# ChrisHird/ZLIB

Hardware: AMD Instinct MI355X
Metric: GiB/s raw input compressed (deflate level 6) (higher is better)
Workload: dtype u8

## Files before the change

### include/zamd_gpu.h

```cpp
#ifndef ZAMD_GPU_H
#define ZAMD_GPU_H
#include <stddef.h>
#include <stdint.h>

#ifdef __cplusplus
extern "C" {
#endif

#define ZGPU_OK 0
#define ZGPU_ERRNO (-1)
#define ZGPU_STREAM_ERROR (-2)
#define ZGPU_DATA_ERROR (-3)
#define ZGPU_MEM_ERROR (-4)
#define ZGPU_BUF_ERROR (-5)

#define ZGPU_CHUNK_MAX 65536u

#define ZGPU_F_FINAL 1u
#define ZGPU_F_ZLIB_WRAP 2u
#define ZGPU_F_POS0 4u
#define ZGPU_F_POS0_ALL 8u
#define ZGPU_F_GZIP_WRAP 16u
#define ZGPU_F_CRC32 32u

// ... 213 lines not shown
                                   uint64_t *total, uint64_t *nfailed);

int zgpu_inflate_batch_verify_device(zgpu_engine *e, const void *d_in, uint64_t in_bytes, const uint64_t *d_in_offsets, uint64_t n, int wrap,
                                     uint32_t checks, zgpu_inflate_item *d_items, uint64_t *nfailed, void *hip_stream);
int zgpu_inflate_batch_verify_host(zgpu_engine *e, const void *in, uint64_t in_bytes, const uint64_t *in_offsets, uint64_t n, int wrap,
                                   uint32_t checks, zgpu_inflate_item *items, uint64_t *nfailed);

#define ZGPU_BATCH_JOB_DECODE 0
#define ZGPU_BATCH_JOB_SIZES 1
#define ZGPU_BATCH_JOB_VERIFY 2
#define ZGPU_BATCH_JOB_PACKED 3
typedef struct {
    uint64_t nfailed, nbad_offsets, total;
    uint32_t overflow, reserved;
} zgpu_inflate_batch_summary;
uint64_t zgpu_inflate_batch_workspace_bytes(int job, uint64_t n);
int zgpu_inflate_batch_enqueue(zgpu_engine *e, const void *d_in, uint64_t in_bytes, const uint64_t *d_in_offsets, uint64_t n, int wrap,
                               uint32_t checks, void *d_out, uint64_t out_cap, const uint64_t *d_out_offsets, zgpu_inflate_item *d_items,
                               zgpu_inflate_batch_summary *d_summary, void *d_ws, uint64_t ws_bytes, void *hip_stream);
int zgpu_inflate_batch_sizes_enqueue(zgpu_engine *e, const void *d_in, uint64_t in_bytes, const uint64_t *d_in_offsets, uint64_t n, int wrap,
                                     zgpu_inflate_item *d_items, zgpu_inflate_batch_summary *d_summary, void *d_ws, uint64_t ws_bytes,
                                     void *hip_stream);
int zgpu_inflate_batch_verify_enqueue(zgpu_engine *e, const void *d_in, uint64_t in_bytes, const uint64_t *d_in_offsets, uint64_t n, int wrap,
                                      uint32_t checks, zgpu_inflate_item *d_items, zgpu_inflate_batch_summary *d_summary, void *d_ws,
                                      uint64_t ws_bytes, void *hip_stream);
int zgpu_inflate_batch_packed_enqueue(zgpu_engine *e, const void *d_in, uint64_t in_bytes, const uint64_t *d_in_offsets, uint64_t n, int wrap,
                                      uint32_t checks, uint32_t align, void *d_out, uint64_t out_cap, uint64_t *d_out_offsets,
                                      zgpu_inflate_item *d_items, zgpu_inflate_batch_summary *d_summary, void *d_ws, uint64_t ws_bytes,
                                      void *hip_stream);

int zgpu_bgzf_index_device(zgpu_engine *e, const void *d_in, uint64_t in_bytes, uint64_t *d_in_offsets, uint64_t *d_out_offsets, uint64_t cap_blocks,
                           uint64_t *nblocks, uint64_t *out_bytes, uint32_t *ends_with_eof_block, void *hip_stream);
int zgpu_bgzf_inflate_device(zgpu_engine *e, const void *d_in, uint64_t in_bytes, void *d_out, uint64_t out_cap, zgpu_inflate_item *d_items,
                             zgpu_inflate_result *res, void *hip_stream);
int zgpu_bgzf_inflate_host(zgpu_engine *e, const void *in, uint64_t in_bytes, void *out, uint64_t out_cap, zgpu_inflate_item *items, zgpu_inflate_result *res);
int zgpu_bgzf_verify_device(zgpu_engine *e, const void *d_in, uint64_t in_bytes, zgpu_inflate_item *d_items, zgpu_inflate_result *res, void *hip_stream);
int zgpu_bgzf_verify_host(zgpu_engine *e, const void *in, uint64_t in_bytes, zgpu_inflate_item *items, zgpu_inflate_result *res);

int zgpu_gzip_inflate_device(zgpu_engine *e, const void *d_in, uint64_t in_bytes, void *d_out, uint64_t out_cap, uint64_t *d_in_offsets, uint64_t *d_out_offsets,
                             zgpu_inflate_item *d_items, uint64_t cap_members, uint64_t *nmembers, zgpu_inflate_result *res, void *hip_stream);
int zgpu_gzip_inflate_host(zgpu_engine *e, const void *in, uint64_t in_bytes, void *out, uint64_t out_cap, uint64_t *in_offsets, uint64_t *out_offsets,
                           zgpu_inflate_item *items, uint64_t cap_members, uint64_t *nmembers, zgpu_inflate_result *res);
uint64_t zgpu_gzip_members_count(int which);

int zgpu_adler32_device(zgpu_engine *e, const void *d_in, uint64_t in_bytes, uint32_t *adler_out, void *hip_stream);
int zgpu_crc32_device(zgpu_engine *e, const void *d_in, uint64_t in_bytes, uint32_t *crc_out, void *hip_stream);

typedef struct {
    uint32_t adler32, crc32;
} zgpu_check_item;
int zgpu_checksum_batch_device(zgpu_engine *e, const void *d_in, uint64_t in_bytes, const uint64_t *d_offsets, uint64_t n, uint32_t checks,
                               zgpu_check_item *d_items, void *hip_stream);
int zgpu_checksum_batch_host(zgpu_engine *e, const void *in, uint64_t in_bytes, const uint64_t *offsets, uint64_t n, uint32_t checks,
                             zgpu_check_item *items);

enum {
    ZGPU_STAGE_CHAIN = 0,
    ZGPU_STAGE_MATCH,
    ZGPU_STAGE_PARSE,
    ZGPU_STAGE_LZ_SERIAL,
    ZGPU_STAGE_HUFFMAN,
    ZGPU_STAGE_STITCH,
    ZGPU_STAGE_INFLATE,
    ZGPU_STAGE_COUNT
};
void zgpu_profile_enable(zgpu_engine *e, int on);
void zgpu_profile_reset(zgpu_engine *e);
int zgpu_profile_get(zgpu_engine *e, int stage, double *ms, uint64_t *launches);
const char *zgpu_stage_name(int stage);

enum {
    ZGPU_FAST_ROUNDS = 0,
    ZGPU_FAST_TILE_PARSES,
    ZGPU_FAST_SAME_ENTRY,
    ZGPU_FAST_STOPPED_EARLY,
    ZGPU_FAST_DIFFERENT_TOKEN,
    ZGPU_FAST_REACH_TO_END,
    ZGPU_FAST_WINDOWS_TO_DIFF,
    ZGPU_FAST_WINDOWS_OF_DIFF,
    ZGPU_FAST_COUNT_N
};
uint64_t zgpu_deflate_fast_count(zgpu_engine *e, int which);

int zgpu_corpus_fill_device(zgpu_engine *e, uint32_t kind, uint64_t seed, uint64_t first_chunk, uint64_t nchunks,
                            void *d_out, void *hip_stream);

#ifdef __cplusplus
}
#endif
#endif
```

### zlib_amd/csrc/zgpu_common.h

```cpp
#pragma once
#include <hip/hip_runtime.h>
#include <stdint.h>

namespace zgpu {

constexpr uint32_t kWSize = 32768, kWMask = kWSize - 1, kHashSize = 32768, kHashMask = kHashSize - 1;
constexpr uint32_t kMinMatch = 3, kMaxMatch = 258, kMinLookahead = kMaxMatch + kMinMatch + 1;
constexpr uint32_t kMaxDist = kWSize - kMinLookahead;
constexpr uint32_t kTooFar = 4096;
constexpr uint32_t kChunkMax = 65536;
constexpr uint32_t kSPad = 8, kSStride = kChunkMax + kSPad;
constexpr uint32_t kBlockTokens = 16383;
constexpr uint32_t kSerialTableEntries = 32768 + 32768;
constexpr uint32_t kGeoTableEntries = 65536 + 32768;
constexpr uint32_t kGeoNostoreWords = 18;
constexpr uint32_t kGeoSlotStride = 65536 + 8192 + 1024 + 64 + 5 * 32 * kGeoNostoreWords + 448;
constexpr uint32_t kMaxBlocks = 6;
constexpr uint32_t kFullFinalBlock = 1u << 31;
constexpr uint32_t kHandedOn = 0xFFFFFFFFu;
constexpr int kLCodes = 286, kDCodes = 30, kBLCodes = 19, kHeapSize = 2 * kLCodes + 1, kMaxBits = 15, kMaxBLBits = 7;
constexpr int kEndBlock = 256;
constexpr uint32_t kSlotStride = 65536 + 256;

struct LevelCfg { uint32_t good, lazy, nice, chain, slow, strategy; uint32_t w_bits, hash_bits; };
constexpr uint32_t kFiltered = 1, kHuffmanOnly = 2, kRle = 3, kFixed = 4;
inline LevelCfg level_cfg(int level)
{
    static const LevelCfg t[10] = {{0, 0, 0, 0, 0, 0},      {4, 4, 8, 4, 0, 0},      {4, 5, 16, 8, 0, 0},      {4, 6, 32, 32, 0, 0},
                                   {4, 4, 16, 16, 1, 0},    {8, 16, 32, 32, 1, 0},   {8, 16, 128, 128, 1, 0},  {8, 32, 128, 256, 1, 0},
                                   {32, 128, 258, 1024, 1, 0}, {32, 258, 258, 4096, 1, 0}};
    return t[level];
}

enum InfMsg : uint32_t {
    kMsgNone = 0, kMsgBlockType, kMsgStoredLen, kMsgTooMany, kMsgCodeLens, kMsgRepeat, kMsgLitLens, kMsgDists, kMsgLitCode, kMsgDistCode,
    kMsgTooFar, kMsgTruncated, kMsgOutput, kMsgTrailing, kMsgShort, kMsgTable,
    kMsgHeaderCheck, kMsgMethod, kMsgWindow, kMsgHeaderFlags, kMsgHeaderCrc, kMsgDataCheck, kMsgLengthCheck, kMsgBgzfChain, kMsgCount
};

constexpr uint32_t kWrapRaw = 0, kWrapZlib = 1, kWrapGzip = 2, kWrapAuto = 3;
struct BatchItemState {
    uint64_t in_lo, in_hi, body_lo, out_lo;
    uint64_t piece0;
    uint32_t kind;
    int32_t code;
    uint32_t msg, used;
    uint32_t out_bytes, npieces;
};
struct InfStatus { int32_t code; uint32_t msg; uint32_t out_bytes; uint32_t used; };
constexpr uint32_t kWholeStream = 0xFFFFFFFFu;
struct SpecEnd { uint64_t end_bit; uint32_t out_bytes, flags; };
struct SpecArgs {
    uint16_t *mid;
    uint64_t *page_owner;
    uint32_t *page_count;
    uint32_t page_cap;
    uint16_t *tails;
    SpecEnd *ends;
    const struct PieceRow *rows = nullptr;
    uint32_t *need = nullptr;
    const uint8_t *windows = nullptr;
    const uint64_t *ostart = nullptr;
    struct PieceCheck *checks = nullptr;
};
struct PieceCheck { uint64_t end_bit; uint32_t out_bytes, flags, adler_a, adler_b, crc, pad; };
struct PieceTarget { uint64_t lo_bit, hi_bit, limit; };
struct PieceRow {
    uint64_t start, stop;
    uint64_t in_end;
    uint32_t item;
    uint32_t first;
};
constexpr uint32_t kPieceNoItem = 0xFFFFFFFFu;
struct PieceItem {
    uint64_t body_lo, in_hi, out_lo, out_hi;
    uint64_t total;
    uint64_t end_bit;
    uint32_t k;
    uint32_t target0, slot0;
    uint32_t ntargets, piece_cap;
    uint32_t npieces;
    uint32_t clean;
    uint32_t bad;
};
struct PiecesList { unsigned long long *hdr; PieceItem *items; uint64_t min_bytes, max_long; };
constexpr uint32_t kHdrLong = 0, kHdrTargets = 1, kHdrSlots = 2, kHdrRoom = 3, kHdrClean = 4, kHdrFell = 5, kHdrGathered = 6;

struct FrameHead { uint8_t b[18]; uint8_t n, gzip, bgzf; };
constexpr uint32_t kBgzfBlockMax = 65280;

struct ChunkMeta {
    uint32_t ntok;
    uint32_t nostore;
    uint32_t out_bytes;
    uint32_t data_type;
    uint32_t adler_a, adler_b;
    uint32_t in_bytes;
    uint32_t crc;
};

struct TileRow {
// ... 335 lines not shown
```

### zlib_amd/csrc/zgpu_deflate.hip

```cpp
#include "zgpu_engine.h"
#include "zgpu_deflate_plan.h"
#include <cstdlib>
#include <atomic>
#include <thread>

namespace zgpu {

int ensure_deflate_ws(zgpu_engine *e, uint32_t batch, bool serial, uint64_t nchunks_total, bool geo)
{
    int rc;
    bool grew;
    if (geo) {
        if ((rc = e->geo_slots.reserve(e, (size_t)batch * kGeoSlotStride))) return rc;
        if ((rc = e->geo_tables.reserve(e, (size_t)batch * kGeoTableEntries, &grew))) return rc;
        if (grew) {
            ZGPU_HIP_CHECK(hipMemsetAsync(e->geo_tables, 0, e->geo_tables.cap * sizeof(uint4), e->stream));
            ZGPU_HIP_CHECK(hipStreamSynchronize(e->stream));
        }
        if ((rc = e->geo_nostore.reserve(e, (size_t)batch * kGeoNostoreWords))) return rc;
    }
    if ((rc = e->tokens.reserve(e, (size_t)batch * kChunkMax))) return rc;
    if ((rc = e->meta.reserve(e, (size_t)batch))) return rc;
    if ((rc = e->slots.reserve(e, (size_t)batch * kSlotStride))) return rc;
    if (serial && !geo) {
// ... 155 lines not shown
    launch_seg_limit(c.d_seg, c.nseg, c.in_bytes, kBgzfBlockMax, flag, c.st);
    ZGPU_HIP_CHECK(hipMemcpyAsync(&over, flag, 4, hipMemcpyDeviceToHost, c.st));
    ZGPU_HIP_CHECK(hipStreamSynchronize(c.st));
    if (over) return fail(e, ZGPU_STREAM_ERROR, "BGZF blocks: a segment is longer than 65280 bytes (or the table leaves the input)");
    return ZGPU_OK;
}

static int reserve_deflate(zgpu_engine *e, const DeflatePlan &pl, uint32_t *hand_piece)
{
    int rc = ensure_deflate_ws(e, pl.batch, pl.serial, pl.nchunks, pl.geo);
    if (rc) return rc;
    *hand_piece = pl.hand_piece;
    if (pl.hand_on) {
        if ((rc = ensure_deflate_ws(e, pl.hand_piece, false, pl.nchunks))) return rc;
        if (e->par_cap > pl.hand_piece) *hand_piece = e->par_cap < pl.batch ? e->par_cap : pl.batch;
        if ((rc = e->hand_list.reserve(e, (size_t)pl.batch + 1))) return rc;
    }
    return ZGPU_OK;
}

static ChunkGeom chunk_geom(const zgpu_engine *e, const DeflateCall &c, const DeflatePlan &pl)
{
    const zgpu_deflate_params *p = c.p;
    ChunkGeom g{};
    g.in = c.d_in; g.in_bytes = c.in_bytes; g.seg_off = c.d_seg; g.chunk_size = pl.chunk_size;
    g.final_chunk = (!c.d_seg && (p->flags & ZGPU_F_FINAL)) ? pl.nchunks - 1 : ~0ull;
    g.all_final = (c.d_seg && (p->flags & ZGPU_F_FINAL)) ? 1u : 0u;
    g.pos0_mode = (p->flags & ZGPU_F_POS0_ALL) ? 2u : (p->flags & ZGPU_F_POS0) ? 1u : 0u;
    g.skip0 = c.skip0;
    g.block_tokens = pl.block_tokens;
    g.slot_stride = pl.geo ? kGeoSlotStride : kSlotStride;
    g.nostore_bits = pl.geo ? e->geo_nostore : nullptr;
    g.prime = (p->prime >> 16) ? ((p->prime & 0xffff0000u) | (p->prime & ((1u << (p->prime >> 16)) - 1u))) : 0u;
    return g;
}

static int copy_batch_in(zgpu_engine *e, const DeflateCall &c, const BatchSteps &s, uint32_t chunk_size)
{
    const uint64_t c1 = s.c0 + s.nb();
    const uint64_t lo = s.c0 * chunk_size, hi = c1 * (uint64_t)chunk_size < c.in_bytes ? c1 * (uint64_t)chunk_size : c.in_bytes;
    const hipEvent_t ev = engine_copy_event(e, s.k);
    ZGPU_HIP_CHECK(hipMemcpyAsync(const_cast<uint8_t *>(c.d_in) + lo, c.h_src + lo, hi - lo, hipMemcpyHostToDevice, e->copy_stream));
    ZGPU_HIP_CHECK(hipEventRecord(ev, e->copy_stream));
    ZGPU_HIP_CHECK(hipStreamWaitEvent(c.st, ev, 0));
    return ZGPU_OK;
}

static int lz_batch(zgpu_engine *e, const ChunkGeom &g, const DeflatePlan &pl, uint32_t hand_piece, hipStream_t st, bool *adler_done)
{
    *adler_done = false;
    if (!pl.serial) {
        if (pl.impl == ZGPU_LZ_PARALLEL) launch_lz_parallel(g, pl.cfg, e->par_ws, e->tokens, e->meta, st, e);
        else *adler_done = launch_lz_sorted(g, pl.cfg, e->par_ws, e->tokens, e->meta, st, e, e->exact_sort, pl.impl);
        return ZGPU_OK;
    }
    StageTimer t(e, st, ZGPU_STAGE_LZ_SERIAL);
    if (++e->serial_tag == 0) {
        if (e->tables) ZGPU_HIP_CHECK(hipMemsetAsync(e->tables, 0, e->tables.cap * sizeof(uint4), st));
        if (e->geo_tables) ZGPU_HIP_CHECK(hipMemsetAsync(e->geo_tables, 0, e->geo_tables.cap * sizeof(uint4), st));
        e->serial_tag = 1;
    }
    if (pl.geo) launch_lz_serial(g, pl.cfg, e->geo_tables, e->tokens, e->meta, st, e->geo_nostore, false, e->serial_tag);
    else launch_lz_serial(g, pl.cfg, e->tables, e->tokens, e->meta, st, nullptr, pl.hand_on, e->serial_tag);
    if (pl.hand_on) {
        launch_collect_handed_on(e->meta, g.nchunks, e->hand_list + 1, e->hand_list, st);
        uint32_t handed = 0;
        ZGPU_HIP_CHECK(hipMemcpyAsync(&handed, e->hand_list, 4, hipMemcpyDeviceToHost, st));
        ZGPU_HIP_CHECK(hipStreamSynchronize(st));
        for (uint32_t at = 0; at < handed; at += hand_piece) {
            ChunkGeom gl = g; gl.nchunks = handed - at < hand_piece ? handed - at : hand_piece; gl.chunk_map = e->hand_list + 1 + at;
            launch_lz_sorted(gl, pl.cfg, e->par_ws, e->tokens, e->meta, st, e, e->exact_sort, ZGPU_LZ_FASTWIN);
        }
        e->handed_on += handed;
    }
    return ZGPU_OK;
}

static void blocks_batch(zgpu_engine *e, const DeflateCall &c, const DeflatePlan &pl, const ChunkGeom &g, const FrameHead &fh, uint64_t body_cap, bool adler_done)
{
    const hipStream_t st = c.st;
    uint8_t *const slots = pl.geo ? e->geo_slots : e->slots;
    {
        StageTimer t(e, st, ZGPU_STAGE_HUFFMAN);
        launch_huffman(g, e->tokens, e->meta, slots, st, pl.cfg.strategy == kFixed);
    }
    StageTimer t(e, st, ZGPU_STAGE_STITCH);
    if (!adler_done) launch_adler(g, e->meta, st);
    if (pl.with_crc) launch_crc(g, e->meta, st);
    if (pl.seg_wrap) launch_frame(slots, e->meta, e->offsets, c.d_seg, g.chunk0, g.nchunks, c.d_out, body_cap, g.slot_stride, e->run, pl.with_crc, fh, st);
    else {
        launch_scan(e->meta, g.nchunks, g.chunk0, e->offsets, e->run, body_cap, st, pl.with_crc);
        launch_stitch(slots, e->meta, e->offsets, g.chunk0, g.nchunks, c.d_out, body_cap, g.slot_stride, st);
    }
    if (c.d_items) launch_seg_items(e->meta, e->offsets, c.d_seg, g.chunk0, g.nchunks, pl.with_crc, c.d_items, st);
}

static int deflate_device(zgpu_engine *e, const DeflateCall &c)
{
    if (!e) return ZGPU_STREAM_ERROR;
    const zgpu_deflate_params *const p = c.p;
    const hipStream_t st = c.st;
    PlanCall pc;
    pc.args = p && c.res && (c.d_in || !c.in_bytes) && c.d_out;
    if (p) { pc.level = p->level; pc.strategy = p->strategy; pc.lz_impl = p->lz_impl; pc.chunk_size = p->chunk_size; pc.flags = p->flags; pc.prime = p->prime; }
    pc.in_bytes = c.in_bytes; pc.seg = c.d_seg != nullptr; pc.nseg = c.nseg; pc.skip0 = c.skip0; pc.host_in = c.h_src != nullptr;
    PlanEngine pe; pe.geo_w = e->geo_w; pe.geo_m = e->geo_m;
    DeflatePlan pl = plan_deflate_args(pc, pe);
    if (pl.rc) return fail(e, pl.rc, pl.msg);
    ZGPU_HIP_CHECK(hipSetDevice(e->device));
    int rc;
    if ((p->flags & ZGPU_F_BGZF_WRAP) && c.nseg && !c.seg_checked && (rc = check_bgzf_segments(e, c))) return rc;
    const LevelCfg lc = level_cfg_for(e, p->level, p->strategy);
    pl = plan_deflate(pc, plan_engine(e, &lc), read_deflate_knobs());
    if (pl.rc) return fail(e, pl.rc, pl.msg);
    uint32_t hand_piece = 0;
    if ((rc = reserve_deflate(e, pl, &hand_piece))) return rc;
    const FrameHead fh = frame_head(p->level, p->strategy, pl.wrap, pl.gz, pl.bgzf);
    ChunkGeom g = chunk_geom(e, c, pl);
    const uint64_t body_cap = pl.tail_bytes ? (c.out_cap >= pl.head_bytes + pl.tail_bytes ? c.out_cap - pl.tail_bytes : 0) : c.out_cap;
    RunState rs{}; rs.out_total = pl.head_bytes; rs.adler_a = 1; rs.adler_b = 0; rs.data_type = 2;
    ZGPU_HIP_CHECK(hipMemcpyAsync(e->run, &rs, sizeof rs, hipMemcpyHostToDevice, st));
    uint32_t sort_fault = 0;
    if (pl.check_sort) ZGPU_HIP_CHECK(hipMemsetAsync(lz_sorted_fault_word(e->par_ws), 0, 4, st));
    if (!pl.seg_wrap && pl.head_bytes && c.out_cap >= pl.head_bytes) ZGPU_HIP_CHECK(hipMemcpyAsync(c.d_out, fh.b, pl.head_bytes, hipMemcpyHostToDevice, st));
    const size_t nbatches = plan_nbatches(pl);
    BatchHomer home;
    if (c.h_dst && c.h_src && nbatches > 1 && nbatches <= BatchHomer::kMaxBatches && (rc = home.start(e, c, nbatches))) return rc;
    for (BatchSteps s(pl); s.more(); s.next()) {
        g.chunk0 = s.c0; g.nchunks = s.nb();
        if (c.h_src && c.in_bytes && (rc = copy_batch_in(e, c, s, pl.chunk_size))) return rc;
        bool adler_done;
        if ((rc = lz_batch(e, g, pl, hand_piece, st, &adler_done))) return rc;
        blocks_batch(e, c, pl, g, fh, body_cap, adler_done);
        if (home.on() && (rc = home.queued(s.k, st))) return rc;
        const hipError_t he = hipGetLastError();
        if (he != hipSuccess) return zgpu::fail_hip(e, he, "kernel launch", __FILE__, __LINE__);
    }
    if (home.on() && (rc = home.finish(c.h_copied))) return rc;
    ZGPU_HIP_CHECK(hipMemcpyAsync(&rs, e->run, sizeof rs, hipMemcpyDeviceToHost, st));
    if (pl.check_sort) ZGPU_HIP_CHECK(hipMemcpyAsync(&sort_fault, lz_sorted_fault_word(e->par_ws), 4, hipMemcpyDeviceToHost, st));
    ZGPU_HIP_CHECK(hipStreamSynchronize(st));
    collect_spans(e);
    if (sort_fault) {
        e->exact_sort = 1;
        return deflate_device(e, c);
    }
    if (rs.overflow || (pl.tail_bytes && c.out_cap < rs.out_total + pl.tail_bytes)) return fail(e, ZGPU_BUF_ERROR, "output capacity too small");
    const uint32_t adler = rs.adler_a | (rs.adler_b << 16);
    if ((pl.wrap || pl.gz) && !pl.seg_wrap && (rc = write_trailer(e, pl.gz, adler, rs.crc, c.in_bytes, c.d_out, &rs.out_total, st))) return rc;
    if (c.d_chunk_offsets) {
        ZGPU_HIP_CHECK(hipMemcpyAsync(c.d_chunk_offsets, e->offsets, (pl.nchunks + 1) * sizeof(uint64_t), hipMemcpyDeviceToDevice, st));
        ZGPU_HIP_CHECK(hipStreamSynchronize(st));
    }
    zgpu_deflate_result *const res = c.res;
    res->out_bytes = rs.out_total; res->nchunks = pl.nchunks; res->adler32 = adler; res->data_type = rs.data_type; res->ntokens = rs.ntokens;
    res->crc32 = pl.with_crc ? rs.crc : 0;
    return ZGPU_OK;
}

}

using namespace zgpu;

extern "C" {
#pragma GCC visibility push(default)

uint64_t zgpu_deflate_bound(uint64_t in_bytes, uint32_t chunk_size)
// ... 256 lines not shown
```

### zlib_amd/csrc/zgpu_deflate_batch.hip

```cpp
#include "zgpu_engine.h"
#include "zgpu_deflate_plan.h"
#include "zgpu_deflate_batch_plan.h"

namespace zgpu {

static_assert(kDwsTokenBytes == kChunkMax * sizeof(uint32_t) && kDwsSlotBytes == kSlotStride && kDwsMetaBytes == sizeof(ChunkMeta),
              "zgpu_deflate_batch_plan.h states what a round's item costs as numbers");
static_assert(sizeof(zgpu_deflate_batch_item) == 40 && sizeof(zgpu_deflate_batch_summary) == 40, "the records of include/zamd_gpu.h");
static_assert(kDwsStageBytes == kChunkMax && kDwsLoBytes == sizeof(uint64_t) && kDwsPreBytes == sizeof(uint64_t), "the staging buffer and its tables");
static_assert(kDwsCntBytes / 8 == 32, "dbatch_head_kernel clears the counters with lanes 0..31");
static_assert(kSlotStride % 4 == 0, "dbatch_place_kernel reads the slots as words");

constexpr uint32_t kItemServed = 0, kItemFailed = 1;

__global__ void __launch_bounds__(64) dbatch_head_kernel(unsigned long long *cnt, uint32_t *fault, zgpu_deflate_batch_summary *summary)
{
    const uint32_t tid = threadIdx.x;
    if (cnt && tid < kDwsCntBytes / 8) cnt[tid] = 0;
    if (fault && tid == 32) fault[0] = 0;
    if (summary && tid == 33) *summary = zgpu_deflate_batch_summary{};
}

__global__ void __launch_bounds__(1024) dbatch_check_kernel(const uint64_t *__restrict__ in_off, uint64_t n, uint64_t in_bytes, uint32_t limit, const uint64_t *__restrict__ out_off,
                                                            uint64_t out_cap, uint32_t packed, uint64_t c0, uint32_t nb, uint64_t *__restrict__ lo_out, uint64_t *__restrict__ t,
// ... 137 lines not shown
{
    const uint64_t k = (uint64_t)blockIdx.x * 256 + threadIdx.x;
    const bool raised = fault[0] != 0;
    if (raised && k < n) items[k].code = ZGPU_ERRNO;
    if (k == 0 && summary) {
        zgpu_deflate_batch_summary s{};
        s.nfailed = raised ? n : cnt[kDcntFailed]; s.nbad_offsets = cnt[kDcntBadOffsets]; s.ntoo_long = cnt[kDcntTooLong];
        s.total = packed ? cnt[kDcntTotal] : 0; s.overflow = packed && cnt[kDcntTotal] > out_cap ? 1u : 0u; s.sort_fault = raised ? 1u : 0u;
        *summary = s;
    }
}

struct DeflateBatchWs {
    unsigned long long *cnt; uint64_t *lo, *pre; uint32_t *state; uint8_t *stage; uint8_t *sorted; uint32_t *tokens; uint8_t *slots; ChunkMeta *meta;
    uint32_t round;
};

struct DeflateBatchCfg { LevelCfg cfg; int impl; bool with_crc; FrameHead fh; uint32_t tail, limit; };
static const char *batch_params(const zgpu_engine *e, const zgpu_deflate_params *p, DeflateBatchCfg *bc)
{
    constexpr uint32_t kServed = ZGPU_F_FINAL | ZGPU_F_ZLIB_WRAP | ZGPU_F_GZIP_WRAP | ZGPU_F_CRC32 | ZGPU_F_BGZF_WRAP;
    if (p->level < 1 || p->level > 9) return "deflate batch: level must be 1..9";
    if (!(p->flags & ZGPU_F_FINAL)) return "deflate batch: every item is a stream of its own, ZGPU_F_FINAL is required";
    if (p->flags & ~kServed) return "deflate batch: ZGPU_F_POS0 / ZGPU_F_POS0_ALL / ZGPU_F_CONTINUOUS are not served";
    const uint32_t wrappers = (p->flags & ZGPU_F_ZLIB_WRAP ? 1 : 0) + (p->flags & ZGPU_F_GZIP_WRAP ? 1 : 0) + (p->flags & ZGPU_F_BGZF_WRAP ? 1 : 0);
    if (wrappers > 1) return "deflate batch: one wrapper at a time";
    if (p->prime) return "deflate batch: prime is not served";
    if (p->lz_impl != ZGPU_LZ_AUTO) return "deflate batch: lz_impl must be ZGPU_LZ_AUTO";
    if (p->strategy < 0 || p->strategy > (int)kFixed) return "strategy must be 0..4";
    if (p->strategy == (int)kHuffmanOnly || p->strategy == (int)kRle) return "deflate batch: Z_HUFFMAN_ONLY and Z_RLE are not served (the blocking segment call serves them)";
    if (e->geo_w != 15 || e->geo_m != 8) return "deflate batch: the default geometry only (windowBits 15, memLevel 8)";
    bc->cfg = level_cfg_for(e, p->level, p->strategy);
    if (bc->cfg.slow) {
        if (const char *why = records_refuse(bc->cfg, ZGPU_LZ_WALK)) return why;
        bc->impl = ZGPU_LZ_WALK;
    } else {
        if (!lz_fastwin_serves(bc->cfg)) return "deflate batch: levels 1-3 with their own parameters only (ZGPU_LZ_FASTWIN does not serve this deflateTune row)";
        if (const char *why = fast_refuse(bc->cfg)) return why;
        bc->impl = ZGPU_LZ_FASTWIN;
    }
    const bool wrap = p->flags & ZGPU_F_ZLIB_WRAP, bgzf = p->flags & ZGPU_F_BGZF_WRAP, gz = (p->flags & ZGPU_F_GZIP_WRAP) || bgzf;
    bc->with_crc = gz || (p->flags & ZGPU_F_CRC32);
    bc->fh = frame_head(p->level, p->strategy, wrap, gz, bgzf);
    bc->tail = gz ? 8u : wrap ? 4u : 0u;
    bc->limit = bgzf ? kBgzfBlockMax : kChunkMax;
    return nullptr;
}

static int deflate_batch_enqueue(zgpu_engine *e, const void *d_in, uint64_t in_bytes, const uint64_t *d_in_off, uint64_t n, const zgpu_deflate_params *p, void *d_out, uint64_t out_cap,
                                 uint64_t *d_out_off, bool packed, zgpu_deflate_batch_item *d_items, zgpu_deflate_batch_summary *d_summary, void *d_ws, uint64_t ws_bytes,
                                 uint32_t batch_items, void *hip_stream)
{
    if (!e) return ZGPU_STREAM_ERROR;
    if (!p || n >= kDwsMaxItems || (n && (!d_in_off || !d_items || !d_out_off)) || (n && in_bytes && !d_in) || (n && out_cap && !d_out))
        return fail(e, ZGPU_STREAM_ERROR, "bad deflate batch arguments");
    DeflateBatchCfg bc{};
    if (const char *why = batch_params(e, p, &bc)) return fail(e, ZGPU_STREAM_ERROR, why);
    const hipStream_t st = hip_stream ? static_cast<hipStream_t>(hip_stream) : e->stream;
    DeflateBatchWs w{};
    if (n) {
        const DeflateWsPlan pl = deflate_batch_ws_plan(n, batch_items);
        if (!d_ws || (reinterpret_cast<uintptr_t>(d_ws) & (kDwsAlign - 1)) || pl.total == 0 || ws_bytes < pl.total)
            return fail(e, ZGPU_STREAM_ERROR, "deflate batch workspace: null, not 256-byte aligned or too small");
        uint8_t *b = static_cast<uint8_t *>(d_ws);
        w.cnt = reinterpret_cast<unsigned long long *>(b + pl.cnt.off); w.lo = reinterpret_cast<uint64_t *>(b + pl.lo.off); w.pre = reinterpret_cast<uint64_t *>(b + pl.pre.off); w.stage = b + pl.stage.off;
        w.state = reinterpret_cast<uint32_t *>(b + pl.state.off); w.sorted = b + pl.sorted.off; w.tokens = reinterpret_cast<uint32_t *>(b + pl.tokens.off);
        w.slots = b + pl.slots.off; w.meta = reinterpret_cast<ChunkMeta *>(b + pl.meta.off); w.round = (uint32_t)pl.round;
    }
    int cur = -1;
    ZGPU_HIP_CHECK(hipGetDevice(&cur));
    if (cur != e->device) ZGPU_HIP_CHECK(hipSetDevice(e->device));
    if (n == 0) {
        if (d_summary) hipLaunchKernelGGL(dbatch_head_kernel, dim3(1), dim3(64), 0, st, static_cast<unsigned long long *>(nullptr), static_cast<uint32_t *>(nullptr), d_summary);
        ZGPU_HIP_CHECK(hipGetLastError());
        return ZGPU_OK;
    }
    uint32_t *const fault = lz_sorted_fault_word(w.sorted);
    hipLaunchKernelGGL(dbatch_head_kernel, dim3(1), dim3(64), 0, st, w.cnt, fault, d_summary);
    const uint32_t ngrid = (uint32_t)((n + 255) / 256);
    ChunkGeom g{};
    g.in = w.stage; g.in_bytes = (uint64_t)w.round * kDwsStageBytes; g.chunk_size = kChunkMax;
    g.final_chunk = ~0ull; g.all_final = 1; g.block_tokens = kBlockTokens; g.slot_stride = kSlotStride;
    const uint32_t frame = bc.fh.n + bc.tail;
    for (uint64_t c0 = 0; c0 < n; c0 += w.round) {
        const uint32_t nb = (uint32_t)(n - c0 < w.round ? n - c0 : w.round);
        const uint64_t *const t = w.pre;
        g.seg_off = t; g.chunk0 = 0; g.nchunks = nb;
        hipLaunchKernelGGL(dbatch_check_kernel, dim3(1), dim3(1024), 0, st, d_in_off, n, in_bytes, bc.limit, d_out_off, out_cap, packed ? 1u : 0u, c0, nb, w.lo, w.pre, w.state, w.cnt);
        hipLaunchKernelGGL(dbatch_gather_kernel, dim3(nb), dim3(256), 0, st, static_cast<const uint8_t *>(d_in), w.lo, w.state, t, nb, w.stage);
        const bool adler_done = launch_lz_sorted(g, bc.cfg, w.sorted, w.tokens, w.meta, st, nullptr, e->exact_sort, bc.impl);
        launch_huffman(g, w.tokens, w.meta, w.slots, st, bc.cfg.strategy == kFixed);
        if (!adler_done) launch_adler(g, w.meta, st);
        if (bc.with_crc) launch_crc(g, w.meta, st);
        if (packed) hipLaunchKernelGGL(dbatch_scan_kernel, dim3(1), dim3(1024), 0, st, w.meta, w.state, c0, nb, frame, d_out_off, w.cnt);
        hipLaunchKernelGGL(dbatch_place_kernel, dim3(nb), dim3(256), 0, st, w.slots, w.meta, w.state, t, d_out_off, c0, nb, static_cast<uint8_t *>(d_out), out_cap,
                           packed ? 1u : 0u, bc.with_crc ? 1u : 0u, bc.fh, bc.tail, d_items, w.cnt);
    }
    hipLaunchKernelGGL(dbatch_finish_kernel, dim3(ngrid), dim3(256), 0, st, fault, n, packed ? 1u : 0u, out_cap, w.cnt, d_items, d_summary);
    ZGPU_HIP_CHECK(hipGetLastError());
    return ZGPU_OK;
}

}

using namespace zgpu;

extern "C" {
#pragma GCC visibility push(default)

uint64_t zgpu_deflate_batch_workspace_bytes(uint64_t n, uint32_t batch_items) { return deflate_batch_ws_bytes(n, batch_items); }

int zgpu_deflate_batch_enqueue(zgpu_engine *e, const void *d_in, uint64_t in_bytes, const uint64_t *d_in_offsets, uint64_t n, const zgpu_deflate_params *p, void *d_out,
                               uint64_t out_cap, const uint64_t *d_out_offsets, zgpu_deflate_batch_item *d_items, zgpu_deflate_batch_summary *d_summary, void *d_ws,
                               uint64_t ws_bytes, uint32_t batch_items, void *hip_stream)
{
    return deflate_batch_enqueue(e, d_in, in_bytes, d_in_offsets, n, p, d_out, out_cap, const_cast<uint64_t *>(d_out_offsets), false, d_items, d_summary, d_ws, ws_bytes, batch_items,
                                 hip_stream);
}

int zgpu_deflate_batch_packed_enqueue(zgpu_engine *e, const void *d_in, uint64_t in_bytes, const uint64_t *d_in_offsets, uint64_t n, const zgpu_deflate_params *p, void *d_out,
                                      uint64_t out_cap, uint64_t *d_out_offsets, zgpu_deflate_batch_item *d_items, zgpu_deflate_batch_summary *d_summary, void *d_ws,
                                      uint64_t ws_bytes, uint32_t batch_items, void *hip_stream)
{
    return deflate_batch_enqueue(e, d_in, in_bytes, d_in_offsets, n, p, d_out, out_cap, d_out_offsets, true, d_items, d_summary, d_ws, ws_bytes, batch_items, hip_stream);
}

int zgpu_engine_set_exact_sort(zgpu_engine *e, int on)
{
    if (!e) return ZGPU_STREAM_ERROR;
    e->exact_sort = on != 0;
    return ZGPU_OK;
}

#pragma GCC visibility pop
}
```

### zlib_amd/csrc/zgpu_engine.h

```cpp
#pragma once
#include "zgpu_common.h"
#include "../../include/zamd_gpu.h"
#include <vector>

namespace zgpu {

int fail_hip(zgpu_engine *e, hipError_t err, const char *what, const char *file, int line);
int fail(zgpu_engine *e, int code, const char *msg);

template <typename T> struct DevBuf {
    T *p = nullptr;
    size_t cap = 0;
    DevBuf() = default;
    DevBuf(const DevBuf &) = delete;
    DevBuf &operator=(const DevBuf &) = delete;
    ~DevBuf() { release(); }
    operator T *() const { return p; }
    void release() { if (p) hipFree(p); p = nullptr; cap = 0; }
    int reserve(zgpu_engine *e, size_t n, bool *grew = nullptr)
    {
        if (grew) *grew = false;
        if (n <= cap) return ZGPU_OK;
        release();
        const hipError_t err = hipMalloc(reinterpret_cast<void **>(&p), n * sizeof(T));
        if (err != hipSuccess) { p = nullptr; return fail_hip(e, err, "hipMalloc of an engine buffer", __FILE__, __LINE__); }
        cap = n;
        if (grew) *grew = true;
        return ZGPU_OK;
    }
};

struct Carve {
    size_t off = 0;
    size_t operator()(size_t bytes) { const size_t at = off; off = (off + bytes + 255) & ~(size_t)255; return at; }
};

}

namespace zgpu { struct StreamsRoundPart; struct StreamsRound; }
struct StageSpan { int stage; hipEvent_t a, b; };

struct zgpu_engine {
    template <typename T> using DevBuf = zgpu::DevBuf<T>;
    int device = 0;
    hipStream_t stream = nullptr;
    hipStream_t copy_stream = nullptr;
    std::vector<hipEvent_t> copy_ev;
    hipStream_t d2h_stream = nullptr;
    std::vector<hipEvent_t> done_ev;
    uint64_t *pin_tot = nullptr;
    char err[512] = {0};
    DevBuf<uint32_t> tokens;
    DevBuf<zgpu::ChunkMeta> meta;
    DevBuf<uint8_t> slots;
    uint32_t batch_cap() const { return (uint32_t)meta.cap; }
    DevBuf<uint4> tables;
    uint32_t serial_tag = 0;
    DevBuf<uint8_t> par_ws;
    uint32_t par_cap = 0;
    int tuned = 0; uint32_t tune[4] = {0, 0, 0, 0};
    int fast_prev0 = 0, before_buf = -1;
    int last_tok_match = -1;
    uint64_t handed_on = 0;
    DevBuf<uint32_t> hand_list;
    int geo_w = 15, geo_m = 8;
    DevBuf<uint8_t> geo_slots; DevBuf<uint4> geo_tables; DevBuf<uint32_t> geo_nostore;
    int exact_sort = 0;
    DevBuf<uint64_t> offsets;
    DevBuf<zgpu::RunState> run;
    DevBuf<uint8_t> stage_in, stage_out;
    DevBuf<uint8_t> inf_status;
    DevBuf<zgpu::ChunkMeta> inf_meta;
    DevBuf<uint64_t> inf_offs;
    DevBuf<uint8_t> inf_slots;
    DevBuf<uint8_t> inf_dict; uint32_t inf_dict_len = 0;
    uint32_t inf_checks = 3;
    DevBuf<uint16_t> ct_exits, ct_entry, ct_comp, ct_gentry;
    DevBuf<uint32_t> ct_tokoff, ct_T, ct_carry, ct_carry_in;
    DevBuf<zgpu::ContBlk> ct_blk; DevBuf<uint64_t> ct_pos; DevBuf<uint8_t> ct_slots; DevBuf<zgpu::ContState> ct_st;
    uint32_t ct_tiles() const { return ct_tokoff.cap ? (uint32_t)(ct_tokoff.cap - 1) : 0; }
    DevBuf<zgpu::ChunkMeta> ct_ckmeta;
    DevBuf<uint64_t> ct_excl;
    DevBuf<zgpu::TileRow> ds_rows; DevBuf<uint16_t> ds_entry; DevBuf<zgpu::ContState> ds_st; DevBuf<zgpu_check_item> ds_check; DevBuf<unsigned long long> ds_totals;
    DevBuf<uint32_t> ds_tokoff, ds_blk_item; DevBuf<zgpu::StreamsRoundPart> ds_parts; DevBuf<zgpu::StreamsRound> ds_rounds; DevBuf<uint64_t> ds_tile0;
    DevBuf<uint64_t> ds_in_off, ds_oo, ds_po; DevBuf<zgpu_deflate_batch_item> ds_items; DevBuf<uint8_t> ds_packed;
    DevBuf<uint16_t> cf_exit_a, cf_exit_b; DevBuf<uint32_t> cf_ins0, cf_ins1, cf_prev, cf_prev2, cf_hist, cf_count;
    DevBuf<uint8_t> cf_cur, cf_act_a, cf_act_b, cf_changed, cf_kept; DevBuf<uint32_t> cf_list_a, cf_list_b, cf_used; DevBuf<uint16_t> cf_entry_used;
    DevBuf<uint32_t> cf_dbg, cf_dstat;
    hipStream_t ct_stream = nullptr; hipEvent_t ct_ev_a[2] = {nullptr, nullptr}, ct_ev_b[2] = {nullptr, nullptr};
    uint64_t cf_rounds = 0, cf_tile_parses = 0;
    uint64_t cf_stat[6] = {};
    DevBuf<uint32_t> bz_cnt, bz_isize, bz_jump_a, bz_jump_b, bz_reach, bz_res;
    DevBuf<uint64_t> bz_base, bz_pos, bz_next, bz_in_off, bz_out_off;
    DevBuf<zgpu_inflate_item> bz_items;
    DevBuf<uint64_t> gz_in_end, gz_trial, gz_next; DevBuf<uint32_t> gz_guess;
    DevBuf<zgpu_inflate_item> gz_items;
    DevBuf<uint64_t> pk_hi; DevBuf<zgpu_inflate_item> pk_items;
    DevBuf<uint64_t> ck_piece0; DevBuf<uint32_t> ck_flag, ck_part;
    bool prof = false;
    double ms[ZGPU_STAGE_COUNT] = {0};
    uint64_t launches[ZGPU_STAGE_COUNT] = {0};
    std::vector<hipEvent_t> ev_pool;
    size_t ev_used = 0;
    std::vector<StageSpan> spans;

    zgpu_engine() = default;
    zgpu_engine(const zgpu_engine &) = delete;
    zgpu_engine &operator=(const zgpu_engine &) = delete;
    ~zgpu_engine();
};

namespace zgpu {

void collect_spans(zgpu_engine *e);
int ensure_stage(zgpu_engine *e, uint64_t in_bytes, uint64_t out_bytes);
hipEvent_t engine_copy_event(zgpu_engine *e, size_t i);
void prof_span_begin(zgpu_engine *e, hipStream_t st, hipEvent_t *a);
void prof_span_end(zgpu_engine *e, hipStream_t st, int stage, hipEvent_t a);
struct StageTimer {
    zgpu_engine *e; hipStream_t st; int stage; hipEvent_t a{};
    StageTimer(zgpu_engine *e_, hipStream_t st_, int stage_) : e(e_), st(st_), stage(stage_) { prof_span_begin(e, st, &a); }
    ~StageTimer() { prof_span_end(e, st, stage, a); }
};
uint32_t env_u32(const char *name, uint32_t dflt);
int checksum_pass(zgpu_engine *e, const uint8_t *d_bytes, uint64_t nbytes, uint32_t mask, uint32_t batch_cap, DevBuf<ChunkMeta> &meta, hipStream_t st, uint32_t *adler, uint32_t *crc);

int ensure_deflate_ws(zgpu_engine *e, uint32_t batch, bool serial, uint64_t nchunks_total, bool geo = false);
LevelCfg level_cfg_for(const zgpu_engine *e, int level, int strategy);
FrameHead frame_head(int level, int strategy, bool wrap, bool gz, bool bgzf = false);
int write_trailer(zgpu_engine *e, bool gz, uint32_t adler, uint32_t crc, uint64_t in_bytes, uint8_t *d_out, uint64_t *out_total, hipStream_t st);
struct PlanEngine;
PlanEngine plan_engine(const zgpu_engine *e, const LevelCfg *cfg);

const char *streams_refuse(const zgpu_engine *e, const zgpu_deflate_params *p);
void streams_list_geom(const uint8_t *d_in, uint64_t in_bytes, uint16_t *exits, uint16_t *entry, ChunkGeom *g, TileGeom *tg);

int deflate_cont_oneshot(zgpu_engine *e, const uint8_t *d_in, uint64_t in_bytes, const zgpu_deflate_params *p, uint8_t *d_out, uint64_t out_cap, zgpu_deflate_result *res, hipStream_t st);

void launch_lz_serial(const ChunkGeom &g, LevelCfg cfg, uint4 *tables, uint32_t *tokens, ChunkMeta *meta, hipStream_t st, uint32_t *nostore_bits, bool hand_on, uint32_t tag);

void launch_huffman(const ChunkGeom &g, const uint32_t *tokens, ChunkMeta *meta, uint8_t *slots, hipStream_t st, bool fixed_trees);
void launch_huffman_cont(const ChunkGeom &g, const uint32_t *compact_tokens, uint32_t nblk, ContBlk *blk, ContState *cst, uint8_t *slots, hipStream_t st, bool fixed_trees);
void launch_huffman_streams(const ChunkGeom &g, const uint32_t *batch_tokens, uint32_t nslots, ContBlk *blk, ContState *states, const uint32_t *blk_item, uint8_t *slots, hipStream_t st,
                            bool fixed_trees);

void launch_collect_handed_on(const ChunkMeta *meta, uint32_t n, uint32_t *list, uint32_t *count, hipStream_t st);
void launch_adler(const ChunkGeom &g, ChunkMeta *meta, hipStream_t st);
void launch_crc(const ChunkGeom &g, ChunkMeta *meta, hipStream_t st);
void launch_scan(const ChunkMeta *meta, uint32_t nchunks, uint64_t chunk0, uint64_t *offsets, void *run, uint64_t out_cap, hipStream_t st, bool with_crc = false);
void launch_frame(const uint8_t *slots, const ChunkMeta *meta, uint64_t *offsets, const uint64_t *seg_off, uint64_t chunk0, uint32_t nchunks, uint8_t *out,
                  uint64_t out_cap, uint32_t slot_stride, void *run, bool with_crc, const FrameHead &h, hipStream_t st);
void launch_stitch(const uint8_t *slots, const ChunkMeta *meta, const uint64_t *offsets, uint64_t chunk0, uint32_t nchunks, uint8_t *out,
                   uint64_t out_cap, uint32_t slot_stride, hipStream_t st);
void launch_bgzf_cut(uint64_t in_bytes, uint32_t block_size, uint64_t nseg, uint64_t *seg_off, hipStream_t st);
void launch_seg_limit(const uint64_t *seg_off, uint64_t nseg, uint64_t in_bytes, uint32_t limit, uint32_t *flag, hipStream_t st);
void launch_seg_items(const ChunkMeta *meta, const uint64_t *offsets, const uint64_t *seg_off, uint64_t chunk0, uint32_t nchunks, bool with_crc, zgpu_deflate_item *items, hipStream_t st);
void launch_corpus(uint32_t kind, uint64_t seed, uint64_t first_chunk, uint64_t nchunks, uint8_t *out, hipStream_t st);
void launch_batch_finish(const BatchItemState *items, uint64_t n, const ChunkMeta *meta, const uint8_t *in, uint32_t do_adler, uint32_t do_crc,
                         zgpu_inflate_item *out_items, unsigned long long *nfailed, hipStream_t st);

bool lz_parallel_available();
size_t lz_parallel_workspace_bytes(uint32_t batch_chunks);
void launch_lz_parallel(const ChunkGeom &g, LevelCfg cfg, void *workspace, uint32_t *tokens, ChunkMeta *meta, hipStream_t st, zgpu_engine *prof);
void launch_parse(const ChunkGeom &g, LevelCfg cfg, const uint2 *recs, uint32_t *tokens, ChunkMeta *meta, hipStream_t st);

void launch_parse2(const ChunkGeom &g, LevelCfg cfg, const uint2 *recs, uint32_t *tokens, ChunkMeta *meta, hipStream_t st);
void launch_parse_tile(const ChunkGeom &g, LevelCfg cfg, const uint32_t *gm, const uint32_t *gs, uint32_t *tokens, ChunkMeta *meta, const TileGeom &tg, hipStream_t st);

size_t lz_sorted_workspace_bytes(uint32_t batch_chunks);
uint32_t *lz_sorted_fault_word(void *workspace);
bool launch_lz_sorted(const ChunkGeom &g, LevelCfg cfg, void *workspace, uint32_t *tokens, ChunkMeta *meta, hipStream_t st, zgpu_engine *prof, int exact_sort,
                      int impl);
void launch_lz_tiles(const ChunkGeom &g, const TileGeom &tg, LevelCfg cfg, void *workspace, ChunkMeta *meta, uint16_t *comp, uint16_t *gentry, hipStream_t st, zgpu_engine *prof,
                     int exact_sort);
void launch_lz_tiles_parse(const ChunkGeom &g, const TileGeom &tg, LevelCfg cfg, void *workspace, uint32_t *tokens, ChunkMeta *meta, hipStream_t st, zgpu_engine *prof);
void launch_sort_tiles(const ChunkGeom &g, void *workspace, ChunkMeta *meta, hipStream_t st, zgpu_engine *prof, int exact_sort, const uint16_t **S_out, const uint32_t **ir_out);

bool lz_fastwin_serves(const LevelCfg &cfg);
void launch_lz_fastwin(const ChunkGeom &g, LevelCfg cfg, const uint16_t *S, const uint32_t *ir, uint32_t *tokens, ChunkMeta *meta, hipStream_t st);
void launch_lz_fastwin_tiles(const ChunkGeom &g, const TileGeom &tg, const FastTiles &ft, LevelCfg cfg, const uint16_t *S, const uint32_t *ir, uint32_t *tokens, ChunkMeta *meta, uint32_t ngrid,
                             hipStream_t st);
void launch_fast_init(uint8_t *cur, uint8_t *active, uint16_t *exit_cur, uint32_t n, hipStream_t st);
void launch_fast_flip_list(uint8_t *cur, uint16_t *exit_cur, const uint16_t *exit_new, const uint32_t *list, uint32_t n, hipStream_t st);
void launch_fast_flip(uint8_t *cur, const uint8_t *active, uint8_t *active_next, const uint8_t *changed, uint16_t *exit_cur, const uint16_t *exit_new, uint32_t n, uint32_t round,
                      uint32_t *count, uint32_t *list, const uint8_t *kept, hipStream_t st);
void launch_fast_finish(const uint8_t *cur, const uint16_t *exit_cur, const uint32_t *ins0, const uint32_t *ins1, uint32_t n, uint16_t *entry_after, uint32_t *prev_ins, uint32_t *prev_prev_ins,
                        const uint32_t *low, hipStream_t st);
void launch_fast_hist(const uint32_t *before, const uint32_t *last, uint32_t x0, uint32_t count, uint32_t *out, hipStream_t st);

uint32_t chain_groups(uint32_t ntiles);
uint64_t cont_special_pos(uint64_t n);
void launch_chain(const uint16_t *exits, uint32_t ntiles, uint16_t *comp, uint16_t *gentry, uint16_t *entry, hipStream_t st);
void launch_cont_tokens(const ChunkGeom &g, const TileGeom &tg, const uint32_t *tokens, const ChunkMeta *tmeta, ContState *st, uint32_t *tokoff, const uint32_t *carry, uint32_t *T,
                        ContBlk *blk, uint64_t seg_end, bool final_block, uint64_t sp, uint32_t nblk_cap, bool slow, hipStream_t s);
void launch_cont_stitch(const ContBlk *blk, ContState *st, uint64_t *pos, const uint8_t *slots, uint32_t slot_stride, const uint8_t *in, uint64_t abs0, uint8_t *out, uint64_t out_cap,
                        uint32_t nblk_cap, const uint32_t *T, uint32_t *carry, uint64_t seg_end, hipStream_t s);

struct ContBatch {
    const StreamsRoundPart *parts; const StreamsRound *round;
    const uint64_t *in_off, *oo, *tile0; uint64_t t0;
    const uint8_t *in; uint8_t *out; uint32_t flags, slow, nslots_max;
    ContState *st; const uint16_t *entry;
    const uint32_t *tokens; const ChunkMeta *tmeta;
    uint32_t *tokoff, *carry, *T; ContBlk *blk; uint64_t *pos; const uint8_t *slots; uint32_t *blk_item;
};
void launch_cont_batch_tokens(const ContBatch &q, uint32_t nparts_max, uint32_t ntiles_max, hipStream_t s);
void launch_cont_batch_stitch(const ContBatch &q, uint32_t nparts_max, hipStream_t s);

void launch_streams_head(const uint64_t *in_off, const uint64_t *oo, const uint32_t *state, uint64_t n, const FrameHead &fh, uint32_t flags, ContState *st, uint8_t *out, uint16_t *entry0,
                         unsigned long long *totals, hipStream_t s);
void launch_streams_entry(const TileRow *rows, uint32_t ntiles, uint16_t *entry, hipStream_t s);
void launch_streams_finish(const uint64_t *in_off, const uint64_t *oo, const uint32_t *state, uint64_t n, const FrameHead &fh, uint32_t flags, const ContState *st,
                           const zgpu_check_item *chk, bool want_crc, uint8_t *out, zgpu_deflate_batch_item *items, unsigned long long *totals, hipStream_t s);
void launch_streams_pack(const uint8_t *rooms, const uint64_t *oo, const uint64_t *po, uint64_t n, uint64_t total, uint8_t *packed, hipStream_t s);

void launch_senq_clear(unsigned long long *cnt, uint32_t *fault, zgpu_deflate_batch_summary *summary, hipStream_t s);
void launch_senq_scan(const uint64_t *in_off, const uint64_t *oo, uint64_t n, uint64_t in_bytes, uint64_t out_cap, uint32_t *state, uint64_t *tile0, uint64_t *piece0,
                      unsigned long long *cnt, hipStream_t s);
void launch_senq_rows(const uint64_t *in_off, const uint64_t *tile0, uint64_t n, uint64_t nrows, TileRow *rows, hipStream_t s);
void launch_senq_round(const uint64_t *tile0, uint64_t n, uint64_t t0, uint32_t batch, const TileRow *rows, StreamsRoundPart *parts, StreamsRound *round, uint16_t *exits, ChunkMeta *meta,
                       hipStream_t s);
void launch_senq_layout(const uint64_t *in_off, uint64_t n, uint64_t in_bytes, uint32_t flags, uint64_t *oo, hipStream_t s);
void launch_senq_summary(const uint32_t *fault, uint64_t n, const unsigned long long *cnt, zgpu_deflate_batch_item *items, zgpu_deflate_batch_summary *summary, hipStream_t s);

struct InfLaunch {
    const uint8_t *in; uint64_t in_bytes; const uint64_t *offsets; uint64_t chunk0; uint32_t nchunks;
    uint8_t *out; uint64_t out_cap; InfStatus *status;
    uint64_t last_chunk = ~0ull; uint32_t chunk_size = kWholeStream; ChunkMeta *meta = nullptr;
    const uint8_t *dict = nullptr; uint32_t dict_len = 0; uint32_t stream_mode = 1;
    uint32_t checks = 0;
};
enum InfKind { kInfChunks, kInfBatch, kInfSizes, kInfPieces, kInfVerify, kInfBatchFold, kInfPieceSizes, kInfPieceVerify };
constexpr int kInfNoRing = 0;
int inflate_ring_kb();
void launch_inflate_decode(InfKind kind, int ring_kb, const InfLaunch &a, const SpecArgs &sp, hipStream_t st);
int output_checksums(zgpu_engine *e, const uint8_t *d_out, uint64_t nbytes, uint64_t out_cap, zgpu_inflate_result *res, hipStream_t st);
int inflate_run(zgpu_engine *e, const uint8_t *d_in, uint64_t in_bytes, const uint64_t *d_offsets, uint64_t nchunks, uint32_t chunk_size, uint8_t *d_out, uint64_t out_cap,
                zgpu_inflate_result *res, hipStream_t st, uint32_t stream_mode = 0, const uint64_t *h_offsets = nullptr, bool open_end = false, uint8_t *h_dst = nullptr, uint64_t h_cap = 0);

void launch_spec_find_table(const uint8_t *d_in, uint64_t in_bytes, const PieceTarget *table, uint32_t ntargets, uint64_t *found, hipStream_t st);
void launch_spec_resolve_items(const SpecArgs &sp, uint32_t nslots, uint32_t nitems, const uint2 *ranges, const uint8_t *entry, uint8_t *windows, const uint64_t *out_start,
                               PieceItem *items, uint8_t *d_out, hipStream_t st);
void launch_spec_windows_items(uint16_t *tails, uint32_t nslots, uint32_t nitems, const uint2 *ranges, const uint8_t *entry, uint8_t *windows, hipStream_t st);

struct BatchPiecesKnobs { uint64_t min_bytes, round_bytes; };
BatchPiecesKnobs batch_pieces_knobs();
uint64_t batch_pieces_count(int which);
size_t batch_pieces_scratch_bytes(uint64_t max_long);
PieceItem *batch_pieces_items(uint8_t *scr);
int batch_pieces_run(zgpu_engine *e, const uint8_t *d_in, uint64_t in_bytes, uint8_t *d_out, uint64_t out_cap, uint64_t max_long, uint8_t *scr, unsigned long long *d_hdr,
                     const unsigned long long *hdr, BatchItemState *states, InfStatus *status, uint64_t round_bytes, int ring_kb, hipStream_t st);
struct BatchPiecesSizesKnobs { uint64_t min_bytes, round_slots; };
BatchPiecesSizesKnobs batch_pieces_sizes_knobs();
// ... 29 lines not shown
```

### zlib_amd/csrc/zgpu_engine.hip

```cpp
#include "zgpu_engine.h"
#include <cstdio>
#include <cstdlib>
#include <cstring>

namespace zgpu {

int fail_hip(zgpu_engine *e, hipError_t err, const char *what, const char *file, int line)
{
    if (e) snprintf(e->err, sizeof e->err, "HIP error %d (%s) at %s:%d: %s", (int)err, hipGetErrorString(err), file, line, what);
    if (err == hipErrorOutOfMemory) return ZGPU_MEM_ERROR;
    return ZGPU_ERRNO;
}

int fail(zgpu_engine *e, int code, const char *msg)
{
    if (e) snprintf(e->err, sizeof e->err, "%s", msg);
    return code;
}

static hipEvent_t next_event(zgpu_engine *e)
{
    if (e->ev_used == e->ev_pool.size()) { hipEvent_t ev; hipEventCreate(&ev); e->ev_pool.push_back(ev); }
    return e->ev_pool[e->ev_used++];
}

void prof_span_begin(zgpu_engine *e, hipStream_t st, hipEvent_t *a)
{
    if (e && e->prof) { *a = next_event(e); hipEventRecord(*a, st); }
}
void prof_span_end(zgpu_engine *e, hipStream_t st, int stage, hipEvent_t a)
{
    if (e && e->prof) { hipEvent_t b = next_event(e); hipEventRecord(b, st); e->spans.push_back({stage, a, b}); }
}

void collect_spans(zgpu_engine *e)
{
    for (auto &s : e->spans) { float ms = 0; if (hipEventElapsedTime(&ms, s.a, s.b) == hipSuccess) { e->ms[s.stage] += ms; e->launches[s.stage]++; } }
    e->spans.clear(); e->ev_used = 0;
}

uint32_t env_u32(const char *name, uint32_t dflt)
{
    const char *v = getenv(name);
    if (!v || !*v) return dflt;
    long x = strtol(v, nullptr, 10);
    return x > 0 ? (uint32_t)x : dflt;
}

int ensure_stage(zgpu_engine *e, uint64_t in_bytes, uint64_t out_bytes)
{
    int rc;
    if (in_bytes > e->stage_in.cap && (rc = e->stage_in.reserve(e, in_bytes + (in_bytes >> 3) + 4096))) return rc;
    if (out_bytes > e->stage_out.cap && (rc = e->stage_out.reserve(e, out_bytes + (out_bytes >> 3) + 4096))) return rc;
    return ZGPU_OK;
}

int checksum_pass(zgpu_engine *e, const uint8_t *d_bytes, uint64_t nbytes, uint32_t mask, uint32_t batch_cap, DevBuf<ChunkMeta> &meta, hipStream_t st, uint32_t *adler, uint32_t *crc)
{
    const uint64_t npieces = nbytes ? (nbytes + kChunkMax - 1) / kChunkMax : 1;
    const uint32_t batch = (uint32_t)(npieces < batch_cap ? npieces : batch_cap);
    if (meta.reserve(e, batch) || e->inf_offs.reserve(e, npieces + 1)) return ZGPU_MEM_ERROR;
    RunState rs{}; rs.adler_a = 1;
    ZGPU_HIP_CHECK(hipMemcpyAsync(e->run, &rs, sizeof rs, hipMemcpyHostToDevice, st));
    for (uint64_t c0 = 0; c0 < npieces; c0 += batch) {
        const uint32_t nb = (uint32_t)(npieces - c0 < batch ? npieces - c0 : batch);
        ZGPU_HIP_CHECK(hipMemsetAsync(meta, 0, (size_t)nb * sizeof(ChunkMeta), st));
        ChunkGeom g{}; g.in = d_bytes; g.in_bytes = nbytes; g.chunk_size = kChunkMax; g.chunk0 = c0; g.nchunks = nb; g.final_chunk = ~0ull;
        if (mask & 1u) launch_adler(g, meta, st);
        if (mask & 2u) launch_crc(g, meta, st);
        launch_scan(meta, nb, c0, e->inf_offs, e->run, ~0ull, st, (mask & 2u) != 0);
    }
    ZGPU_HIP_CHECK(hipMemcpyAsync(&rs, e->run, sizeof rs, hipMemcpyDeviceToHost, st));
    ZGPU_HIP_CHECK(hipStreamSynchronize(st));
    *adler = (mask & 1u) ? rs.adler_a | (rs.adler_b << 16) : 1u;
    *crc = (mask & 2u) ? rs.crc : 0u;
    return ZGPU_OK;
}

hipEvent_t engine_copy_event(zgpu_engine *e, size_t i)
{
    while (e->copy_ev.size() <= i) { hipEvent_t ev; if (hipEventCreateWithFlags(&ev, hipEventDisableTiming) != hipSuccess) return nullptr; e->copy_ev.push_back(ev); }
    return e->copy_ev[i];
}

}

zgpu_engine::~zgpu_engine()
{
    hipSetDevice(device);
    if (stream) hipStreamSynchronize(stream);
    for (auto ev : ev_pool) hipEventDestroy(ev);
    for (auto ev : copy_ev) hipEventDestroy(ev);
    for (auto ev : done_ev) hipEventDestroy(ev);
    if (ct_stream) hipStreamDestroy(ct_stream);
    for (int i = 0; i < 2; i++) { if (ct_ev_a[i]) hipEventDestroy(ct_ev_a[i]); if (ct_ev_b[i]) hipEventDestroy(ct_ev_b[i]); }
    if (d2h_stream) hipStreamDestroy(d2h_stream);
    if (pin_tot) hipHostFree(pin_tot);
    if (copy_stream) hipStreamDestroy(copy_stream);
    if (stream) hipStreamDestroy(stream);
}

using namespace zgpu;

extern "C" {
#pragma GCC visibility push(default)

int zgpu_device_count(void)
{
    int n = 0;
    if (hipGetDeviceCount(&n) != hipSuccess) return 0;
    return n;
}

const char *zgpu_version(void) { return "zamd-gpu 0.1 (gfx950; zlib 1.2.3 bit-exact, 64 KiB independent chunks)"; }

int zgpu_engine_create(int device, zgpu_engine **out)
{
    if (!out) return ZGPU_STREAM_ERROR;
    *out = nullptr;
    int n = zgpu_device_count();
    if (device < 0 || device >= n) return ZGPU_ERRNO;
    zgpu_engine *e = new zgpu_engine();
    e->device = device;
    if (hipSetDevice(device) != hipSuccess || hipStreamCreateWithFlags(&e->stream, hipStreamNonBlocking) != hipSuccess || hipStreamCreateWithFlags(&e->copy_stream, hipStreamNonBlocking) != hipSuccess ||
        e->run.reserve(e, 1) != ZGPU_OK) {
        delete e;
        return ZGPU_ERRNO;
    }
    *out = e;
    return ZGPU_OK;
}

void zgpu_engine_destroy(zgpu_engine *e)
{
    if (e) delete e;
}

const char *zgpu_engine_error(const zgpu_engine *e) { return e ? e->err : "no engine"; }
uint64_t zgpu_debug_handed_on(const zgpu_engine *e) { return e ? e->handed_on : 0; }
int zgpu_debug_sort_fallback(const zgpu_engine *e) { return e ? e->exact_sort : 0; }

int zgpu_adler32_device(zgpu_engine *e, const void *d_in, uint64_t in_bytes, uint32_t *adler_out, void *hip_stream)
{
    if (!e || !adler_out || (!d_in && in_bytes)) return fail(e, ZGPU_STREAM_ERROR, "null argument");
    ZGPU_HIP_CHECK(hipSetDevice(e->device));
    hipStream_t st = hip_stream ? static_cast<hipStream_t>(hip_stream) : e->stream;
    int rc = ensure_deflate_ws(e, 1, false, 1);
    if (rc) return rc;
    uint32_t crc;
    return checksum_pass(e, static_cast<const uint8_t *>(d_in), in_bytes, 1u, 65536, e->inf_meta, st, adler_out, &crc);
}

int zgpu_crc32_device(zgpu_engine *e, const void *d_in, uint64_t in_bytes, uint32_t *crc_out, void *hip_stream)
{
    if (!e || !crc_out || (!d_in && in_bytes)) return fail(e, ZGPU_STREAM_ERROR, "null argument");
    ZGPU_HIP_CHECK(hipSetDevice(e->device));
    hipStream_t st = hip_stream ? static_cast<hipStream_t>(hip_stream) : e->stream;
    int rc = ensure_deflate_ws(e, 1, false, 1);
    if (rc) return rc;
    uint32_t adler;
    return checksum_pass(e, static_cast<const uint8_t *>(d_in), in_bytes, 2u, 65536, e->inf_meta, st, &adler, crc_out);
}

void zgpu_profile_enable(zgpu_engine *e, int on) { if (e) e->prof = on != 0; }
void zgpu_profile_reset(zgpu_engine *e) { if (e) { memset(e->ms, 0, sizeof e->ms); memset(e->launches, 0, sizeof e->launches); } }
int zgpu_profile_get(zgpu_engine *e, int stage, double *ms, uint64_t *launches)
{
    if (!e || stage < 0 || stage >= ZGPU_STAGE_COUNT) return ZGPU_STREAM_ERROR;
    if (ms) *ms = e->ms[stage];
    if (launches) *launches = e->launches[stage];
    return ZGPU_OK;
}
const char *zgpu_stage_name(int stage)
{
    static const char *names[ZGPU_STAGE_COUNT] = {"chain", "match", "parse", "lz_serial", "huffman", "stitch", "inflate"};
    return stage >= 0 && stage < ZGPU_STAGE_COUNT ? names[stage] : "?";
}

uint64_t zgpu_deflate_fast_count(zgpu_engine *e, int which)
{
    if (!e || which < 0 || which >= ZGPU_FAST_COUNT_N) return 0;
    return which == ZGPU_FAST_ROUNDS ? e->cf_rounds : which == ZGPU_FAST_TILE_PARSES ? e->cf_tile_parses : e->cf_stat[which - ZGPU_FAST_SAME_ENTRY];
}

int zgpu_corpus_fill_device(zgpu_engine *e, uint32_t kind, uint64_t seed, uint64_t first_chunk, uint64_t nchunks, void *d_out, void *hip_stream)
{
    if (!e || !d_out) return fail(e, ZGPU_STREAM_ERROR, "null argument");
    ZGPU_HIP_CHECK(hipSetDevice(e->device));
    hipStream_t st = hip_stream ? static_cast<hipStream_t>(hip_stream) : e->stream;
    launch_corpus(kind, seed, first_chunk, nchunks, static_cast<uint8_t *>(d_out), st);
    ZGPU_HIP_CHECK(hipGetLastError());
    ZGPU_HIP_CHECK(hipStreamSynchronize(st));
    return ZGPU_OK;
}

#pragma GCC visibility pop
}
```

### zlib_amd/csrc/zgpu_huffman.hip

```cpp
#include "zgpu_common.h"
#include "zgpu_engine.h"

namespace zgpu {

#ifndef ZGPU_HUFF_THREADS
#define ZGPU_HUFF_THREADS 128
#endif
constexpr int kThreads = ZGPU_HUFF_THREADS;
constexpr uint32_t kEmitPer = 4, kEmitRound = kThreads * kEmitPer;

template <int kNodes>
struct TreeWorkT {
    static constexpr int kCap = kNodes;
    uint16_t freq[kNodes];
    uint16_t dad[kNodes];
    uint16_t len[kNodes];
    __attribute__((aligned(16))) uint32_t heap[kNodes + 5];
    uint16_t bl_count[kMaxBits + 1];
    uint16_t next_code[kMaxBits + 1];
};
using TreeWork = TreeWorkT<kHeapSize>;
using TreeWorkD = TreeWorkT<2 * kDCodes + 1>;
__device__ inline uint32_t heap_entry(uint32_t freq, uint32_t depth, uint32_t node) { return (freq << 16) | (depth << 10) | node; }

struct BitWriter {
    uint32_t *words;
    uint32_t wi;
    uint64_t acc;
    uint32_t nacc;
    __device__ void begin(uint32_t *base, uint64_t bitpos, uint32_t carry) { words = base; wi = (uint32_t)(bitpos >> 5); nacc = (uint32_t)(bitpos & 31); acc = carry; }
    __device__ uint64_t pos() const { return ((uint64_t)wi << 5) + nacc; }
    __device__ void put(uint32_t v, uint32_t nb)
    {
        acc |= (uint64_t)v << nacc; nacc += nb;
        if (nacc >= 32) { words[wi] = (uint32_t)acc; wi++; acc >>= 32; nacc -= 32; }
    }
    __device__ void put64(uint64_t v, uint32_t nb)
    {
        if (nb > 32) { put((uint32_t)v, 32); put((uint32_t)(v >> 32), nb - 32); } else put((uint32_t)v, nb);
    }
    __device__ void align_byte() { uint32_t k = (8 - (nacc & 7)) & 7; if (k) put(0, k); }
    __device__ uint32_t carry() const { return (uint32_t)acc; }
    __device__ void store_tail() { if (nacc) words[wi] = (uint32_t)acc; }
};

template <class TW>
__device__ inline void sift_down(TW &t, int heap_len, int k)
{
    const uint32_t v = t.heap[k];
    int j = k << 1;
    while (j <= heap_len) {
        const uint2 ch = *reinterpret_cast<const uint2 *>(&t.heap[j]);
        const uint4 gc = *reinterpret_cast<const uint4 *>(&t.heap[2 * j]);
        uint32_t c = ch.x; int j1 = j;
        if (j < heap_len && (ch.y >> 10) <= (ch.x >> 10)) { c = ch.y; j1 = j + 1; }
        if ((v >> 10) <= (c >> 10)) break;
        t.heap[k] = c; k = j1;
        const int j2 = j1 << 1;
        if (j2 > heap_len) break;
        const uint32_t g0 = j1 == j ? gc.x : gc.z, g1 = j1 == j ? gc.y : gc.w;
        uint32_t c2 = g0; int j3 = j2;
        if (j2 < heap_len && (g1 >> 10) <= (g0 >> 10)) { c2 = g1; j3 = j2 + 1; }
        if ((v >> 10) <= (c2 >> 10)) break;
        t.heap[k] = c2; k = j3; j = j3 << 1;
    }
    t.heap[k] = v;
}

__device__ inline uint32_t extra_bits_of(int kind, int n)
{
    if (kind == 0) { const int k = n - 257; return (k < 8 || k == 28) ? 0u : (uint32_t)((k >> 2) - 1); }
    if (kind == 1) return n < 4 ? 0u : (uint32_t)((n >> 1) - 1);
    return n == 16 ? 2u : n == 17 ? 3u : n == 18 ? 7u : 0u;
}
__device__ inline uint32_t static_len_of(int kind, int n) { return kind == 0 ? (n < 144 ? 8u : n < 256 ? 9u : n < 280 ? 7u : 8u) : 5u; }

template <class TW>
__device__ int build_tree(TW &t, int elems, int kind, int max_length,
                          uint16_t *out_code, uint8_t *out_len, uint32_t &opt_len, uint32_t &static_len)
{
    const bool has_static = kind != 2;
    int heap_len = 0, heap_max = TW::kCap, max_code = -1, n, m, node;
    for (n = 0; n < elems; n++) {
        if (t.freq[n] != 0) t.heap[++heap_len] = heap_entry(t.freq[n], 0, (uint32_t)(max_code = n));
// ... 215 lines not shown
        count = 0; prevlen = curlen;
        if (nextlen == 0) { max_count = 138; min_count = 3; }
        else if (curlen == nextlen) { max_count = 6; min_count = 3; }
        else { max_count = 7; min_count = 4; }
    }
}

template <int MODE>
__device__ __forceinline__ uint32_t run_items(uint32_t L, uint32_t N, uint32_t *blf, const uint16_t *blcode, const uint8_t *bllen, uint32_t *obuf, uint32_t at)
{
    uint32_t bits = 0, rem = N;
    bool first = true;
    auto item = [&](uint32_t sym, uint32_t xv, uint32_t xb) {
        if (MODE == 0) atomicAdd(&blf[sym], 1u);
        else {
            const uint32_t cl = bllen[sym], nb = cl + xb;
            if (MODE == 2) {
                const uint32_t v = (uint32_t)blcode[sym] | (xv << cl), w = at >> 5, sh = at & 31;
                atomicOr(&obuf[w], v << sh);
                if (sh + nb > 32) atomicOr(&obuf[w + 1], v >> (32 - sh));
                at += nb;
            }
            bits += nb;
        }
    };
    while (rem) {
        if (L == 0) {
            const uint32_t take = rem < 138 ? rem : 138;
            if (take < 3) { for (uint32_t k = 0; k < take; k++) item(0, 0, 0); }
            else if (take <= 10) item(17, take - 3, 3);
            else item(18, take - 11, 7);
            rem -= take;
        } else {
            const uint32_t maxc = first ? 7 : 6, minc = first ? 4 : 3, take = rem < maxc ? rem : maxc;
            if (take < minc) { for (uint32_t k = 0; k < take; k++) item(L, 0, 0); }
            else if (first) { item(L, 0, 0); item(16, take - 4, 2); }
            else item(16, take - 3, 2);
            rem -= take; first = false;
        }
    }
    return bits;
}

__device__ __forceinline__ uint32_t find_runs(const uint8_t *len, int max_code, uint16_t *spos, uint32_t lane)
{
    uint32_t nruns = 0;
    for (int g = 0; g * 64 <= max_code; g++) {
        const int n = g * 64 + (int)lane;
        const bool valid = n <= max_code;
        const uint32_t cur = valid ? len[n] : 0u, prv = (valid && n > 0) ? len[n - 1] : 0u;
        const bool st = valid && (n == 0 || cur != prv);
        const uint64_t m = __ballot(st);
        if (st) spos[nruns + __builtin_amdgcn_mbcnt_hi((uint32_t)(m >> 32), __builtin_amdgcn_mbcnt_lo((uint32_t)m, 0u))] = (uint16_t)n;
        nruns += (uint32_t)__builtin_popcountll(m);
    }
    if (lane == 0) spos[nruns] = (uint16_t)(max_code + 1);
    __builtin_amdgcn_wave_barrier(); asm volatile("s_waitcnt lgkmcnt(0)" ::: "memory");
    return nruns;
}

template <int MODE>
__device__ __forceinline__ uint32_t walk_lengths_wave(const uint8_t *len, int max_code, uint16_t *spos, uint32_t *blf, const uint16_t *blcode, const uint8_t *bllen,
                                                      uint32_t *obuf, uint32_t at0, uint32_t lane)
{
    const uint32_t nruns = find_runs(len, max_code, spos, lane);
    uint32_t done = 0;
    for (uint32_t r0 = 0; r0 < nruns; r0 += 64) {
        const uint32_t r = r0 + lane;
        uint32_t L = 0, N = 0;
        if (r < nruns) { const uint32_t p = spos[r]; N = (uint32_t)spos[r + 1] - p; L = len[p]; }
        if (MODE == 0) run_items<0>(L, N, blf, blcode, bllen, obuf, 0);
        else {
            const uint32_t mybits = run_items<1>(L, N, blf, blcode, bllen, obuf, 0);
            uint32_t x = mybits;
            for (int o = 1; o < 64; o <<= 1) { const uint32_t y = __shfl_up(x, o); if ((int)lane >= o) x += y; }
            run_items<2>(L, N, blf, blcode, bllen, obuf, at0 + done + x - mybits);
            done += __shfl(x, 63);
        }
    }
    __builtin_amdgcn_wave_barrier(); asm volatile("s_waitcnt lgkmcnt(0)" ::: "memory");
    return done;
}

__device__ inline void len_code_of(uint32_t lc, uint32_t &code, uint32_t &extra)
{
    const uint32_t e = (31u - (uint32_t)__clz((int)(lc | 8u))) - 2u;
    const bool small = lc < 8, top = lc == 255;
    code = small ? lc : top ? 28u : 4u * e + 4u + ((lc >> e) & 3u);
    extra = (small || top) ? 0u : e;
}
__device__ inline void dist_code_bits(uint32_t d, uint32_t &code, uint32_t &extra)
{
    const uint32_t msb = 31u - (uint32_t)__clz((int)(d | 2u));
    const bool small = d < 4;
    code = small ? d : 2u * msb + ((d >> (msb - 1u)) & 1u);
    extra = small ? 0u : msb - 1u;
}

__device__ inline void token_bits(uint32_t t, const uint16_t *lcode, const uint8_t *llen, const uint16_t *dcode, const uint8_t *dlen,
                                  uint64_t &bits, uint32_t &nb)
{
    uint32_t dist = t >> 8, lc = t & 255;
    if (dist == 0) { bits = lcode[lc]; nb = llen[lc]; return; }
    uint32_t c, xl, dc, xd;
    len_code_of(lc, c, xl);
    const uint32_t s = 257 + c;
    bits = lcode[s]; nb = llen[s];
    bits |= (uint64_t)(lc & ((1u << xl) - 1u)) << nb; nb += xl;
    dist--;
    dist_code_bits(dist, dc, xd);
    bits |= (uint64_t)dcode[dc] << nb; nb += dlen[dc];
    bits |= (uint64_t)(dist & ((1u << xd) - 1u)) << nb; nb += xd;
}

__device__ inline uint32_t block_reduce_add(uint32_t v, uint32_t *tmp)
{
    for (int o = 32; o > 0; o >>= 1) v += __shfl_down(v, o);
    __syncthreads();
    if ((threadIdx.x & 63) == 0) tmp[threadIdx.x >> 6] = v;
    __syncthreads();
    uint32_t s = 0;
    for (int w = 0; w < kThreads / 64; w++) s += tmp[w];
    return s;
}

__device__ inline uint32_t block_exclusive_scan(uint32_t v, uint32_t *tmp, uint32_t *total)
{
    uint32_t lane = threadIdx.x & 63, wave = threadIdx.x >> 6, x = v;
    for (int o = 1; o < 64; o <<= 1) { uint32_t y = __shfl_up(x, o); if (lane >= (uint32_t)o) x += y; }
    __syncthreads();
    if (lane == 63) tmp[wave] = x;
    __syncthreads();
    uint32_t base = 0;
    for (uint32_t w = 0; w < wave; w++) base += tmp[w];
    uint32_t s = 0;
    for (int w = 0; w < kThreads / 64; w++) s += tmp[w];
    *total = s;
    return base + x - v;
}

#ifdef ZGPU_HUF_TIME
__device__ unsigned long long huf_time[8];
extern "C" __attribute__((visibility("default"))) void zgpu_debug_huf_time(unsigned long long *out, int reset)
{
    unsigned long long z[8] = {};
    (void)hipMemcpyFromSymbol(out, HIP_SYMBOL(huf_time), sizeof z);
    if (reset) (void)hipMemcpyToSymbol(HIP_SYMBOL(huf_time), z, sizeof z);
}
#define HUF_T(i) do { if (tid == 0) { const unsigned long long t_ = wall_clock64(); t_acc[i] += t_ - t_prev; t_prev = t_; } } while (0)
#define HUF_T0() unsigned long long t_prev = wall_clock64(), t_acc[8] = {}
#define HUF_TEND() do { if (tid == 0) for (int i_ = 0; i_ < 8; i_++) atomicAdd(&huf_time[i_], t_acc[i_]); } while (0)
#else
#define HUF_T(i) do { } while (0)
#define HUF_T0() do { } while (0)
#define HUF_TEND() do { } while (0)
#endif

#ifndef ZGPU_HUF_WAVES
#define ZGPU_HUF_WAVES 8
#endif
template <bool CONT, bool MULTI = false>
__global__ void __launch_bounds__(kThreads, ZGPU_HUF_WAVES) huffman_kernel(ChunkGeom g, const uint32_t *__restrict__ tokens, ChunkMeta *meta, uint8_t *slots, uint32_t fixed_trees,
                                                                            ContBlk *blk, ContState *cst, const uint32_t *__restrict__ blk_item)
{
    static_assert(CONT || !MULTI, "many streams' blocks are continuous streams' blocks");
    __shared__ __attribute__((aligned(16))) TreeWork work0;
    __shared__ TreeWorkD work1;
    __shared__ uint32_t hist[kLCodes + kDCodes + 2];
    __shared__ uint16_t lcode[kLCodes + 2], dcode[kDCodes + 2], blcode[kBLCodes + 1];
    __shared__ uint8_t llen[kLCodes + 2], dlen[kDCodes + 2], bllen[kBLCodes + 1];
    __shared__ uint32_t tmp[4];
    constexpr uint32_t kObufWords = (kEmitRound * 48 + 31 + 31) / 32 + 1;
    static_assert(sizeof(TreeWork) >= (kEmitRound + kObufWords) * 4 && alignof(TreeWork) >= 8, "emit buffers live in the tree workspace");
    uint32_t *tokbuf = reinterpret_cast<uint32_t *>(&work0), *obuf = tokbuf + kEmitRound;
    __shared__ uint32_t sh_optl, sh_statl, sh_optd, sh_statd, sh_btype, sh_lmax, sh_dmax;
    __shared__ uint64_t sh_bitpos;
    __shared__ uint32_t sh_carry;

    const uint32_t c = blockIdx.x, tid = threadIdx.x;
    if (!CONT && c >= g.nchunks) return;
    if constexpr (MULTI) { const uint32_t item = blk_item[c]; if (item == 0xFFFFFFFFu) return; cst += item; }
    else if (CONT && c >= cst->nblk) return;
    uint64_t lo = 0; uint32_t nbytes = 0;
    if (!CONT) chunk_span(g, c, lo, nbytes);
    const uint8_t *src = g.in + lo;
    const uint32_t *tok = CONT ? tokens + blk[c].tok0 : tokens + (size_t)c * kChunkMax;
    uint32_t *out = reinterpret_cast<uint32_t *>(slots + (size_t)c * g.slot_stride);
    const uint32_t ntok = CONT ? blk[c].nt : meta[c].ntok, nostore = CONT ? blk[c].nostore : meta[c].nostore;
    const bool final_chunk_here = CONT ? blk[c].eof != 0 : chunk_is_final(g, c);
    const uint32_t btok = g.block_tokens, nblocks = CONT ? 1u : ntok / btok + ((nostore & kFullFinalBlock) ? 0u : 1u);
    const uint32_t *nostore_bits = (!CONT && g.nostore_bits) ? g.nostore_bits + (size_t)c * kGeoNostoreWords : nullptr;
    uint32_t block_start = CONT ? 0u : chunk_skip(g, c), data_type = 2;
    if (tid == 0) { const uint32_t pr = CONT ? 0u : chunk_prime(g, c); sh_bitpos = pr >> 16; sh_carry = pr & 0xffffu; }
    HUF_T0();

    for (uint32_t b = 0; b < nblocks; b++) {
        const uint32_t t0 = b * btok, t1 = (b + 1 == nblocks) ? ntok : t0 + btok, nt = t1 - t0;
        const uint32_t eof = (final_chunk_here && b + 1 == nblocks) ? 1u : 0u;
        for (uint32_t i = tid; i < kLCodes + kDCodes + 2; i += kThreads) hist[i] = 0;
        __syncthreads();
        uint32_t bytes = 0;
        for (uint32_t i0 = t0 + tid; i0 < t1; i0 += 4 * kThreads) {
            uint32_t tv[4];
#pragma unroll
            for (uint32_t k = 0; k < 4; k++) tv[k] = i0 + k * kThreads < t1 ? tok[i0 + k * kThreads] : 0xFFFFFFFFu;
#pragma unroll
            for (uint32_t k = 0; k < 4; k++) {
                if (i0 + k * kThreads >= t1) continue;
                const uint32_t t = tv[k], dist = t >> 8, lc = t & 255;
                if (dist == 0) { atomicAdd(&hist[lc], 1u); bytes += 1; }
                else { uint32_t c, xl, dc, xd; len_code_of(lc, c, xl); dist_code_bits(dist - 1, dc, xd); atomicAdd(&hist[257 + c], 1u); atomicAdd(&hist[kLCodes + dc], 1u); bytes += lc + 3; }
            }
        }
        const uint32_t stored_len = block_reduce_add(bytes, tmp);
        __syncthreads();
        if (tid == 0) hist[kEndBlock] = 1;
        __syncthreads();
        if ((CONT ? blk[c].first != 0 : b == 0) && stored_len > 0) {
            bool bin = false;
            if (tid < 32 && (tid < 9 || tid >= 14)) bin = hist[tid] != 0;
            data_type = __syncthreads_or(bin) ? 0u : 1u;
        }
        for (uint32_t i = tid; i < kLCodes; i += kThreads) work0.freq[i] = (uint16_t)hist[i];
        if (tid < kDCodes) work1.freq[tid] = (uint16_t)hist[kLCodes + tid];
        __syncthreads();
        HUF_T(0);
        if (tid < 64) {
            uint32_t o = 0, s = 0;
            const int mc = build_tree_wave(work0, kLCodes, 0, kMaxBits, lcode, llen, o, s, tid);
            if (tid == 0) { sh_lmax = (uint32_t)mc; sh_optl = o; sh_statl = s; }
        } else {
            uint32_t o = 0, s = 0;
            const int mc = build_tree_wave(work1, kDCodes, 1, kMaxBits, dcode, dlen, o, s, tid - 64);
            if (tid == 64) { sh_dmax = (uint32_t)mc; sh_optd = o; sh_statd = s; }
        }
        __syncthreads();
        HUF_T(1);
        if (tid < 64) {
            const uint32_t lane = tid;
            auto wsync = [&]() { __builtin_amdgcn_wave_barrier(); asm volatile("s_waitcnt lgkmcnt(0)" ::: "memory"); };
            const int lmax = (int)sh_lmax, dmax = (int)sh_dmax;
            uint32_t *blf = hist;
            uint16_t *spos = reinterpret_cast<uint16_t *>(hist + 32);
            static_assert((kLCodes + kDCodes + 2 - 32) * 2 >= kLCodes + 2, "run starts fit behind the counts");
            if (lane < kBLCodes) blf[lane] = 0;
            wsync();
            walk_lengths_wave<0>(llen, lmax, spos, blf, nullptr, nullptr, nullptr, 0, lane);
            walk_lengths_wave<0>(dlen, dmax, spos, blf, nullptr, nullptr, nullptr, 0, lane);
            TreeWork &w = work0;
            if (lane < kBLCodes) w.freq[lane] = (uint16_t)blf[lane];
            wsync();
            if (lane == 0) {
                uint32_t opt_len = sh_optl + sh_optd, static_len = sh_statl + sh_statd;
                uint32_t dummy = 0;
                build_tree(w, kBLCodes, 2, kMaxBLBits, blcode, bllen, opt_len, dummy);
                int max_blindex;
                for (max_blindex = kBLCodes - 1; max_blindex >= 3; max_blindex--) if (bllen[kTables.bl_order[max_blindex]] != 0) break;
                opt_len += 3 * (uint32_t)(max_blindex + 1) + 5 + 5 + 4;
                uint32_t opt_lenb = (opt_len + 3 + 7) >> 3, static_lenb = (static_len + 3 + 7) >> 3;
                if (static_lenb <= opt_lenb) opt_lenb = static_lenb;
                uint32_t btype;
                if (stored_len + 4 <= opt_lenb && !(nostore_bits ? (nostore_bits[b >> 5] >> (b & 31u)) & 1u : (nostore >> b) & 1u)) btype = 0;
                else if (fixed_trees || static_lenb == opt_lenb) btype = 1;
                else btype = 2;
                sh_btype = btype;
                HUF_T(2);
                BitWriter bw; bw.begin(out, sh_bitpos, sh_carry);
                bw.put((btype << 1) + eof, 3);
                if (btype == 0) {
                    bw.align_byte(); bw.put(stored_len & 0xffff, 16); bw.put(~stored_len & 0xffff, 16);
                } else if (btype == 2) {
                    bw.put((uint32_t)(lmax + 1 - 257), 5); bw.put((uint32_t)(dmax + 1 - 1), 5); bw.put((uint32_t)(max_blindex + 1 - 4), 4);
                    for (int r = 0; r <= max_blindex; r++) bw.put(bllen[kTables.bl_order[r]], 3);
                }
                sh_bitpos = bw.pos();
                sh_carry = bw.carry();
            }
            wsync();
            if (sh_btype == 2) {
                constexpr uint32_t kHdrWords = (31 + (kLCodes + kDCodes) * 14 + 31) / 32 + 2;
                static_assert(kHdrWords <= kObufWords, "the header's bits fit the round buffer");
                const uint64_t pos0 = sh_bitpos;
                const uint32_t sh0 = (uint32_t)(pos0 & 31);
                for (uint32_t i = lane; i < kHdrWords; i += 64) obuf[i] = 0;
                wsync();
                if (lane == 0) obuf[0] = sh_carry;
                wsync();
                uint32_t nbits = walk_lengths_wave<2>(llen, lmax, spos, blf, blcode, bllen, obuf, sh0, lane);
                nbits += walk_lengths_wave<2>(dlen, dmax, spos, blf, blcode, bllen, obuf, sh0 + nbits, lane);
                const uint32_t nfull = (sh0 + nbits) >> 5, nwords = (sh0 + nbits + 31) >> 5;
                uint32_t *dstw = out + (pos0 >> 5);
                for (uint32_t wd = lane; wd < nwords; wd += 64) { const uint32_t x = obuf[wd]; if (wd < nfull) dstw[wd] = x; else sh_carry = x; }
                if (lane == 0) { if (nfull == nwords) sh_carry = 0; sh_bitpos = pos0 + nbits; }
            }
        }
        __syncthreads();
        HUF_T(3);
// ... 12 lines not shown
            if (tid == 0) {
                const uint32_t k = (uint32_t)(bitpos >> 3) & 3u, cw = sh_carry;
                for (uint32_t j = 0; j < k; j++) dst[(int)j - (int)k] = (uint8_t)(cw >> (8 * j));
            }
            for (uint32_t i = tid; i < stored_len; i += kThreads) dst[i] = src[block_start + i];
            bitpos += (uint64_t)stored_len * 8;
        } else {
            if (btype == 1) {
                for (uint32_t i = tid; i < kLCodes; i += kThreads) { lcode[i] = kTables.sl_code[i]; llen[i] = kTables.sl_len[i]; }
                if (tid < kDCodes) { dcode[tid] = kTables.sd_code[tid]; dlen[tid] = 5; }
                __syncthreads();
            }
            for (uint32_t i = tid; i < kObufWords; i += kThreads) obuf[i] = 0;
            for (uint32_t r0 = 0; r0 <= nt; r0 += kEmitRound) {
                uint32_t tv[kEmitPer];
#pragma unroll
                for (uint32_t k = 0; k < kEmitPer; k++) { const uint32_t j = r0 + k * kThreads + tid; tv[k] = j < nt ? tok[t0 + j] : 0u; }
#pragma unroll
                for (uint32_t k = 0; k < kEmitPer; k++) tokbuf[k * kThreads + tid] = tv[k];
                __syncthreads();
                if (tid == 0) obuf[0] = sh_carry;
                const uint4 mine = reinterpret_cast<const uint4 *>(tokbuf)[tid];
                const uint32_t mt[4] = {mine.x, mine.y, mine.z, mine.w};
                uint64_t v[kEmitPer]; uint32_t nb[kEmitPer], mybits = 0;
#pragma unroll
                for (uint32_t k = 0; k < kEmitPer; k++) {
                    const uint32_t j = r0 + tid * kEmitPer + k;
                    v[k] = 0; nb[k] = 0;
                    if (j < nt) token_bits(mt[k], lcode, llen, dcode, dlen, v[k], nb[k]);
                    else if (j == nt) { v[k] = lcode[kEndBlock]; nb[k] = llen[kEndBlock]; }
                    mybits += nb[k];
                }
                uint32_t total, off = block_exclusive_scan(mybits, tmp, &total);
                const uint32_t sh0 = (uint32_t)(bitpos & 31);
                uint32_t at = sh0 + off;
#pragma unroll
                for (uint32_t k = 0; k < kEmitPer; k++) {
                    if (nb[k]) {
                        const uint32_t w = at >> 5, sh = at & 31;
                        atomicOr(&obuf[w], (uint32_t)(v[k] << sh));
                        if (sh + nb[k] > 32) atomicOr(&obuf[w + 1], (uint32_t)(v[k] >> (32 - sh)));
                        if (sh + nb[k] > 64) atomicOr(&obuf[w + 2], (uint32_t)(v[k] >> (64 - sh)));
                    }
                    at += nb[k];
                }
                __syncthreads();
                const uint32_t nfull = (sh0 + total) >> 5, nwords = (sh0 + total + 31) >> 5;
                uint32_t *dstw = out + (bitpos >> 5);
                for (uint32_t w = tid; w < nwords; w += kThreads) {
                    const uint32_t x = obuf[w];
                    obuf[w] = 0;
                    if (w < nfull) dstw[w] = x; else sh_carry = x;
                }
                if (tid == 0 && nfull == nwords) sh_carry = 0;
                bitpos += total;
            }
        }
        block_start += stored_len;
        __syncthreads();
        HUF_T(4);
        if (tid == 0) {
            sh_bitpos = bitpos;
            if (btype == 0) {
                const uint32_t k = (uint32_t)(bitpos >> 3) & 3u;
                sh_carry = k ? *reinterpret_cast<volatile uint32_t *>(out + (bitpos >> 5)) & ((1u << (8 * k)) - 1u) : 0u;
            }
        }
        __syncthreads();
    }
    if (CONT) {
        if (tid == 0) { BitWriter bw; bw.begin(out, sh_bitpos, sh_carry); bw.store_tail(); blk[c].nbits = (uint32_t)sh_bitpos; }
    } else if (tid == 0) {
        BitWriter bw; bw.begin(out, sh_bitpos, sh_carry);
        if (!final_chunk_here) { bw.put(0, 3); bw.align_byte(); bw.put(0, 16); bw.put(0xffff, 16); }
        else bw.align_byte();
        uint64_t endpos = bw.pos();
        bw.store_tail();
        meta[c].out_bytes = (uint32_t)(endpos >> 3);
        meta[c].data_type = data_type;
    }
    HUF_TEND();
}

void launch_huffman(const ChunkGeom &g, const uint32_t *tokens, ChunkMeta *meta, uint8_t *slots, hipStream_t st, bool fixed_trees)
{
    hipLaunchKernelGGL(huffman_kernel<false>, dim3(g.nchunks), dim3(kThreads), 0, st, g, tokens, meta, slots, fixed_trees ? 1u : 0u, nullptr, nullptr, nullptr);
}
void launch_huffman_cont(const ChunkGeom &g, const uint32_t *compact_tokens, uint32_t nblk, ContBlk *blk, ContState *cst, uint8_t *slots, hipStream_t st, bool fixed_trees)
{
    if (nblk) hipLaunchKernelGGL(huffman_kernel<true>, dim3(nblk), dim3(kThreads), 0, st, g, compact_tokens, nullptr, slots, fixed_trees ? 1u : 0u, blk, cst, nullptr);
}
void launch_huffman_streams(const ChunkGeom &g, const uint32_t *batch_tokens, uint32_t nslots, ContBlk *blk, ContState *states, const uint32_t *blk_item, uint8_t *slots, hipStream_t st,
                            bool fixed_trees)
{
    if (nslots) hipLaunchKernelGGL((huffman_kernel<true, true>), dim3(nslots), dim3(kThreads), 0, st, g, batch_tokens, nullptr, slots, fixed_trees ? 1u : 0u, blk, states, blk_item);
}

}
```

### zlib_amd/csrc/zgpu_lz_parse.h

```cpp
#pragma once
#include "zgpu_common.h"

namespace zgpu {

#ifndef ZGPU_P2WIN
#define ZGPU_P2WIN 8192
#endif
constexpr uint32_t kP2Win = ZGPU_P2WIN, kP2Blk = kP2Win / 64;
constexpr uint32_t kP2Words = kChunkMax / 32, kP2Batch = 8, kP2Pair = 4, kP2Over = 8;
constexpr uint32_t kNone = 0xffffffffu;

struct ParseCtx {
    const uint2 *rec;
    uint32_t n, base, good, lazy, strategy;
    int slide_at;
    __device__ bool slid(uint32_t p) const { return (int)p >= slide_at; }
    __device__ uint32_t take(uint32_t p, uint32_t prev_len, uint2 r, uint32_t &dist) const
    {
        const uint32_t pick = (prev_len >= good && strategy != kRle) ? r.y : r.x;
        const uint32_t d = (pick >> 9) & 32767u;
        const bool nil = ((r.y >> 24) & 1u) && slid(p);
        const uint32_t len = nil ? 0u : (pick & 511u);
        const bool weak = len <= 5 && (strategy == kFiltered || (len == kMinMatch && d > kTooFar));
        const bool ok = prev_len < lazy && len > prev_len && !weak;
        dist = ok ? d : dist;
        return ok ? len : kMinMatch - 1;
    }
    __device__ void game(uint32_t r, uint2 rr, uint2 rn, uint32_t &m, uint32_t &len, uint32_t &dist) const
    {
        uint32_t L, D = 0;
        L = take(r, kMinMatch - 1, rr, D);
        uint32_t q = r + 1;
        for (;;) {
            uint32_t D2 = 0;
            const uint32_t L2 = take(q, L, rn, D2);
            if (L2 <= L) break;
            L = L2; D = D2; q++;
            rn = rec[q];
        }
        m = q - 1; len = L; dist = D;
    }
};

__device__ inline uint32_t wave_rol1(uint32_t v) { return (uint32_t)__builtin_amdgcn_update_dpp(0, (int)v, 0x134, 0xf, 0xf, false); }

__device__ inline uint32_t next_bit(const uint32_t *bits, uint32_t x, uint32_t nwords)
{
    uint32_t w = x >> 5;
    if (w >= nwords) return kNone;
    uint32_t v = bits[w] & (~0u << (x & 31u));
    while (v == 0) { if (++w >= nwords) return kNone; v = bits[w]; }
    return (w << 5) + (uint32_t)__builtin_ctz(v);
}

__device__ inline void parse_block_cuts(int slide_at, uint32_t base, const uint32_t *TOK, const uint32_t *MAT, const uint32_t *wbase, uint32_t n, uint32_t nwords, uint32_t nw_done,
                                        uint32_t ntok, ChunkMeta &out)
{
    uint32_t nostore = 0, nblk = 0, block_start = 0;
    for (uint32_t b = 0;; b++) {
        const uint32_t e = (b + 1) * kBlockTokens - 1;
        if (e >= ntok) break;
        uint32_t lo_w = 0, hi_w = nw_done;
        while (hi_w - lo_w > 1) { const uint32_t mid = (lo_w + hi_w) >> 1; if (wbase[mid] <= e) lo_w = mid; else hi_w = mid; }
        uint32_t v = TOK[lo_w];
        for (uint32_t s2 = e - wbase[lo_w]; s2; s2--) v &= v - 1;
        const uint32_t pe = (lo_w << 5) + (uint32_t)__builtin_ctz(v);
        const bool is_mat = (MAT[pe >> 5] >> (pe & 31u)) & 1u;
        if (!is_mat && pe == n - 1) { nostore |= kFullFinalBlock; break; }
        uint32_t ns = pe + 1;
        if (is_mat) { ns = next_bit(TOK, pe + 1, nwords); if (ns == kNone) ns = n; }
        if ((int)(pe + 1) >= slide_at && block_start + base < kWSize) nostore |= 1u << nblk;
        nblk++; block_start = ns;
    }
    if ((int)n >= (int)(kWSize + kMaxDist) - (int)base && block_start + base < kWSize) nostore |= 1u << nblk;
    out.ntok = ntok; out.nostore = nostore; out.in_bytes = n;
}

#ifdef ZGPU_P2_TIME
#ifndef ZGPU_PARSE_HEADER_ONLY
#define P2_TIME_ARR p2_time
__device__ unsigned long long p2_time[8];
extern "C" __attribute__((visibility("default"))) void zgpu_debug_p2_time(unsigned long long *out, int reset)
{
    unsigned long long z[8] = {};
    hipMemcpyFromSymbol(out, HIP_SYMBOL(p2_time), sizeof z);
    if (reset) hipMemcpyToSymbol(HIP_SYMBOL(p2_time), z, sizeof z);
}
#endif
#define P2_T(i) do { if (tid == 0) { const unsigned long long t_ = wall_clock64(); t_acc[i] += t_ - t_prev; t_prev = t_; } } while (0)
#define P2_T0() unsigned long long t_prev = wall_clock64(), t_acc[8] = {0, 0, 0, 0, 0, 0, 0, 0}
#define P2_TEND() do { if (tid == 0) for (int i_ = 0; i_ < 7; i_++) atomicAdd(&P2_TIME_ARR[i_], t_acc[i_]); } while (0)
#else
#define P2_T(i) do { } while (0)
#define P2_T0() do { } while (0)
#define P2_TEND() do { } while (0)
#endif

template <bool FUSED> __device__ inline uint32_t p2_ld(const uint32_t *p) { return FUSED ? __hip_atomic_load(p, __ATOMIC_RELAXED, __HIP_MEMORY_SCOPE_AGENT) : *p; }
constexpr uint32_t kP2OffJ = 0, kP2OffHAS = kP2Win * 2, kP2OffMARK = kP2OffHAS + kP2Words * 4, kP2OffCOV = kP2OffMARK + kP2Words * 4, kP2OffMAT = kP2OffCOV + kP2Words * 4,
                   kP2OffWbase = kP2OffMAT + kP2Words * 4, kP2OffVIS = kP2OffWbase + (kP2Words + 4) * 4, kP2OffEXITS = kP2OffVIS + kP2Win / 32 * 4, kP2OffWtot = kP2OffEXITS + 256,
                   kP2OffEntry = kP2OffWtot + 64, kP2LdsBytes = kP2OffEntry + 16;
constexpr uint32_t kP2Wins = kChunkMax / kP2Win, kP2OffEND = kP2LdsBytes, kP2LogLdsBytes = kP2OffEND + kP2Win * 2;
static_assert(kChunkMax % kP2Win == 0 && kP2Win - 1 + 255 + 258 <= 0xffffu, "whole windows; a game's end fits END");

}
```

### zlib_amd/csrc/zgpu_lz_sorted.h

```cpp
#pragma once
#include "zgpu_common.h"
#include "zgpu_engine.h"
#include "zgpu_deflate_batch_plan.h"

namespace zgpu {

constexpr uint32_t kHeadWords = kChunkMax / 32;
constexpr uint32_t kHeadStride = kHeadWords + kChunkMax / 64 / 2;
constexpr uint32_t kGPad = 32, kGStride = kChunkMax + 2 * kGPad;

struct SortedWs {
    static constexpr size_t kHeaderBytes = 256, kSBytes = kSStride * 2, kRkBytes = kChunkMax * 2, kHeadBytes = kHeadStride * 4, kRecBytes = kChunkMax * 8, kIrBytes = kChunkMax * 4;
    static constexpr size_t kSlack = 1024;
    static_assert(kChunkMax * 4 + kChunkMax / 8 <= kRecBytes && kGStride <= kRecBytes, "gm + gs, and G, lie in the records' memory");
    static_assert(kChunkMax * (4 + 2) <= kRecBytes, "and so do the logs: the workspace, and with it the batch a device holds, is what it was");
    static constexpr size_t bytes(size_t nchunks) { return kHeaderBytes + nchunks * (kSBytes + kRkBytes + kHeadBytes + kRecBytes + kIrBytes) + kSlack; }

    size_t nch;
    uint32_t *fault; uint16_t *S, *rk; uint32_t *heads; uint2 *recs; uint32_t *ir;
    SortedWs(void *workspace, size_t nchunks) : nch(nchunks)
    {
        uint8_t *p = static_cast<uint8_t *>(workspace);
        auto take = [&p](size_t n) { uint8_t *at = p; p += n; return at; };
        fault = reinterpret_cast<uint32_t *>(take(kHeaderBytes));
        S = reinterpret_cast<uint16_t *>(take((nch * kSBytes + 255) & ~(size_t)255));
        rk = reinterpret_cast<uint16_t *>(take(nch * kRkBytes));
        heads = reinterpret_cast<uint32_t *>(take(nch * kHeadBytes));
        recs = reinterpret_cast<uint2 *>(take(nch * kRecBytes));
        ir = reinterpret_cast<uint32_t *>(take(nch * kIrBytes));
    }
    uint32_t *gm() const { return reinterpret_cast<uint32_t *>(recs); }
    uint32_t *gs() const { return gm() + nch * kChunkMax; }
    uint32_t *lrec() const { return reinterpret_cast<uint32_t *>(recs); }
    uint16_t *lpos() const { return reinterpret_cast<uint16_t *>(lrec() + nch * kChunkMax); }
    uint8_t *G() const { return reinterpret_cast<uint8_t *>(recs); }
};

static_assert(SortedWs::kHeaderBytes == kDwsSortedHeader && SortedWs::kSlack == kDwsSortedSlack && SortedWs::bytes(1) == kDwsSortedHeader + kDwsSortedChunk + kDwsSortedSlack &&
              SortedWs::bytes(3) - SortedWs::bytes(2) == kDwsSortedChunk, "zgpu_deflate_batch_plan.h states the workspace of a chunk as numbers");

bool launch_sort(const ChunkGeom &g, const SortedWs &ws, ChunkMeta *meta, hipStream_t st, zgpu_engine *prof, int exact_sort);
void launch_match3(const ChunkGeom &g, LevelCfg cfg, const SortedWs &ws, hipStream_t st);
void launch_walk_chunks(const ChunkGeom &g, LevelCfg cfg, const SortedWs &ws, uint32_t *tokens, ChunkMeta *meta, hipStream_t st);
void launch_walk_tiles(const ChunkGeom &g, const TileGeom &tg, LevelCfg cfg, const SortedWs &ws, ChunkMeta *meta, hipStream_t st);
void launch_fast(const ChunkGeom &g, LevelCfg cfg, const SortedWs &ws, uint32_t *tokens, ChunkMeta *meta, hipStream_t st);

__device__ inline uint32_t lds_off(const void *p) { return (uint32_t)(uintptr_t)(const __attribute__((address_space(3))) void *)p; }
__device__ inline void lds_st32(uint32_t a, uint32_t v) { asm volatile("ds_write_b32 %0, %1" ::"v"(a), "v"(v) : "memory"); }
__device__ inline void lds_st16(uint32_t a, uint32_t v) { asm volatile("ds_write_b16 %0, %1" ::"v"(a), "v"(v) : "memory"); }
__device__ inline void lds_max32(uint32_t a, uint32_t v) { asm volatile("ds_max_u32 %0, %1" ::"v"(a), "v"(v) : "memory"); }
__device__ inline uint32_t lds_ld32(uint32_t a) { uint32_t v; asm volatile("ds_read_b32 %0, %1\n\ts_waitcnt lgkmcnt(0)" : "=v"(v) : "v"(a) : "memory"); return v; }
__device__ inline uint32_t lds_ld16(uint32_t a) { uint32_t v; asm volatile("ds_read_u16 %0, %1\n\ts_waitcnt lgkmcnt(0)" : "=v"(v) : "v"(a) : "memory"); return v; }

__device__ inline void lds_st8(uint32_t a, uint32_t v) { asm volatile("ds_write_b8 %0, %1" ::"v"(a), "v"(v) : "memory"); }
__device__ inline uint32_t lds_ld8(uint32_t a) { uint32_t v; asm volatile("ds_read_u8 %0, %1\n\ts_waitcnt lgkmcnt(0)" : "=v"(v) : "v"(a) : "memory"); return v; }

__device__ inline uint32_t lds_ld32u(uint32_t a)
{
    uint64_t v; const uint32_t al = a & ~3u;
    asm volatile("ds_read2_b32 %0, %1 offset1:1\n\ts_waitcnt lgkmcnt(0)" : "=v"(v) : "v"(al) : "memory");
    return __builtin_amdgcn_alignbyte((uint32_t)(v >> 32), (uint32_t)v, a & 3);
}
__device__ inline void lds_cmp8(uint32_t a, uint32_t b, uint32_t &xa, uint32_t &xb)
{
    uint64_t va, vb; uint32_t va2, vb2;
    const uint32_t aa = a & ~3u, ba = b & ~3u;
    asm volatile("ds_read2_b32 %0, %4 offset1:1\n\tds_read_b32 %1, %4 offset:8\n\tds_read2_b32 %2, %5 offset1:1\n\tds_read_b32 %3, %5 offset:8\n\ts_waitcnt lgkmcnt(0)"
                 : "=&v"(va), "=&v"(va2), "=&v"(vb), "=&v"(vb2) : "v"(aa), "v"(ba) : "memory");
    const uint32_t a0 = __builtin_amdgcn_alignbyte((uint32_t)(va >> 32), (uint32_t)va, a & 3), a1 = __builtin_amdgcn_alignbyte(va2, (uint32_t)(va >> 32), a & 3);
    const uint32_t b0 = __builtin_amdgcn_alignbyte((uint32_t)(vb >> 32), (uint32_t)vb, b & 3), b1 = __builtin_amdgcn_alignbyte(vb2, (uint32_t)(vb >> 32), b & 3);
    xa = a0 ^ b0; xb = a1 ^ b1;
}
__device__ inline void lds_ld2bytes(uint32_t a, uint32_t &b0, uint32_t &b1)
{
    asm volatile("ds_read_u8 %0, %2\n\tds_read_u8 %1, %2 offset:1\n\ts_waitcnt lgkmcnt(0)" : "=&v"(b0), "=&v"(b1) : "v"(a) : "memory");
}
struct __attribute__((packed, aligned(2))) U64u { uint64_t v; };
struct __attribute__((packed, aligned(2))) U128u { uint4 v; };

template <uint32_t T> __device__ inline void stage_chunk(const uint8_t *src, uint32_t n, uint32_t *d32, uint32_t tid)
{
    if ((reinterpret_cast<uintptr_t>(src) & 15) == 0) {
        const uint4 *s128 = reinterpret_cast<const uint4 *>(src);
        uint4 *d128 = reinterpret_cast<uint4 *>(d32);
        const uint32_t nv = n >> 4;
        for (uint32_t i = tid; i < (kChunkMax + 64) / 16; i += T) {
            uint4 v = make_uint4(0, 0, 0, 0);
            if (i < nv) v = s128[i];
            else if (i == nv) {
                uint32_t w[4] = {0, 0, 0, 0};
                for (uint32_t k = 0; k < (n & 15); k++) w[k >> 2] |= (uint32_t)src[(nv << 4) + k] << (8 * (k & 3));
                v = make_uint4(w[0], w[1], w[2], w[3]);
            }
            d128[i] = v;
        }
    } else {
        for (uint32_t i = tid; i < (kChunkMax + 64) / 4; i += T) {
            uint32_t v = 0;
            for (uint32_t k = 0; k < 4; k++) { uint32_t a = (i << 2) + k; if (a < n) v |= (uint32_t)src[a] << (8 * (k & 3)); }
            d32[i] = v;
        }
    }
}

__device__ inline unsigned long long mask_eq_u32(uint32_t a, uint32_t b) { unsigned long long m; asm volatile("v_cmp_eq_u32_e64 %0, %1, %2" : "=s"(m) : "v"(a), "v"(b)); return m; }
__device__ inline unsigned long long mask_le_i32(int a, int b) { unsigned long long m; asm volatile("v_cmp_le_i32_e64 %0, %1, %2" : "=s"(m) : "v"(a), "v"(b)); return m; }
__device__ inline unsigned long long mask_gt_u32(uint32_t a, uint32_t b) { unsigned long long m; asm volatile("v_cmp_gt_u32_e64 %0, %1, %2" : "=s"(m) : "v"(a), "v"(b)); return m; }
__device__ inline unsigned long long mask_lt_i32(int a, int b) { unsigned long long m; asm volatile("v_cmp_lt_i32_e64 %0, %1, %2" : "=s"(m) : "v"(a), "v"(b)); return m; }
__device__ inline void stack_push(unsigned long long m, uint32_t rt, uint32_t dummy, uint32_t entry)
{
    uint32_t t;
    asm volatile("v_mbcnt_lo_u32_b32 %0, %2, 0\n\tv_mbcnt_hi_u32_b32 %0, %3, %0\n\tv_lshl_add_u32 %0, %0, 2, %4\n\t"
                 "v_cndmask_b32_e64 %0, %5, %0, %1\n\tds_write_b32 %0, %6"
                 : "=&v"(t) : "s"(m), "s"((uint32_t)m), "s"((uint32_t)(m >> 32)), "s"(rt), "v"(dummy), "v"(entry) : "memory");
}

__device__ inline uint32_t stack_slot(unsigned long long m, uint32_t rt)
{
    uint32_t t;
// ... 10 lines not shown
```

### zlib_amd/csrc/zgpu_lz_sorted.hip

```cpp
#include "zgpu_lz_sorted.h"

namespace zgpu {

size_t lz_sorted_workspace_bytes(uint32_t batch) { return SortedWs::bytes(batch); }
uint32_t *lz_sorted_fault_word(void *workspace) { return SortedWs(workspace, 0).fault; }

bool launch_lz_sorted(const ChunkGeom &g, LevelCfg cfg, void *workspace, uint32_t *tokens, ChunkMeta *meta, hipStream_t st, zgpu_engine *prof, int exact_sort, int impl)
{
    const SortedWs ws(workspace, g.nchunks);
    const bool adler_done = launch_sort(g, ws, meta, st, prof, exact_sort);
    hipEvent_t ev{};
    prof_span_begin(prof, st, &ev);
    if (impl == ZGPU_LZ_FASTWIN) launch_lz_fastwin(g, cfg, ws.S, ws.ir, tokens, meta, st);
    else if (impl == ZGPU_LZ_FAST) launch_fast(g, cfg, ws, tokens, meta, st);
    else if (impl == ZGPU_LZ_WALK) launch_walk_chunks(g, cfg, ws, tokens, meta, st);
    else {
        launch_match3(g, cfg, ws, st);
        prof_span_end(prof, st, ZGPU_STAGE_MATCH, ev);
        prof_span_begin(prof, st, &ev);
        launch_parse(g, cfg, ws.recs, tokens, meta, st);
        prof_span_end(prof, st, ZGPU_STAGE_PARSE, ev);
        return adler_done;
    }
    prof_span_end(prof, st, ZGPU_STAGE_MATCH, ev);
    return adler_done;
}


void launch_sort_tiles(const ChunkGeom &g, void *workspace, ChunkMeta *meta, hipStream_t st, zgpu_engine *prof, int exact_sort, const uint16_t **S_out, const uint32_t **ir_out)
{
    const SortedWs ws(workspace, g.nchunks);
    launch_sort(g, ws, meta, st, prof, exact_sort);
    *S_out = ws.S; *ir_out = ws.ir;
}
void launch_lz_tiles(const ChunkGeom &g, const TileGeom &tg, LevelCfg cfg, void *workspace, ChunkMeta *meta, uint16_t *comp, uint16_t *gentry, hipStream_t st, zgpu_engine *prof,
                     int exact_sort)
{
    const SortedWs ws(workspace, g.nchunks);
    launch_sort(g, ws, meta, st, prof, exact_sort);
    hipEvent_t ev{};
    prof_span_begin(prof, st, &ev);
    launch_walk_tiles(g, tg, cfg, ws, meta, st);
    prof_span_end(prof, st, ZGPU_STAGE_MATCH, ev);
    prof_span_begin(prof, st, &ev);
    launch_chain(tg.exits, g.nchunks, comp, gentry, tg.entry + g.chunk0, st);
    prof_span_end(prof, st, ZGPU_STAGE_PARSE, ev);
}
void launch_lz_tiles_parse(const ChunkGeom &g, const TileGeom &tg, LevelCfg cfg, void *workspace, uint32_t *tokens, ChunkMeta *meta, hipStream_t st, zgpu_engine *prof)
{
    const SortedWs ws(workspace, g.nchunks);
    hipEvent_t ev{};
    prof_span_begin(prof, st, &ev);
    launch_parse_tile(g, cfg, ws.gm(), ws.gs(), tokens, meta, tg, st);
    prof_span_end(prof, st, ZGPU_STAGE_PARSE, ev);
}

}
```

### zlib_amd/csrc/zgpu_lz_tail.h

```cpp
#pragma once

namespace zgpu {

constexpr uint32_t kWtRounds = 24, kWtBlk = 64, kWtNone = 0xffffu;
template <uint32_t T> struct TailLds {
    static constexpr uint32_t kCap = kWtRounds * T;
    static constexpr uint32_t kBlocks = kCap / kWtBlk;
    static constexpr uint32_t kHAS = 0, kCOV = kHAS + kP2Words * 4, kMAT = kCOV + kP2Words * 4, kWbase = kMAT + kP2Words * 4, kRC = kWbase + (kP2Words + 4) * 4,
                              kN = kRC + kP2Words * 2, kMARK = kN + kCap * 2, kEX = kMARK + kCap / 8, kENT = kEX + kBlocks * 2, kWtot = kENT + kBlocks * 2,
                              kFlag = kWtot + 64, kBytes = kFlag + 16;
    static_assert(kCap < kWtNone && kCap % kWtBlk == 0 && kBlocks % 64 == 0 && kBlocks <= T && kP2Words % T == 0 && T % 64 == 0 && T / 64 <= 16, "workgroup size");
};

#ifdef ZGPU_P2_TIME
__device__ unsigned long long p2_tail_time[12];
extern "C" __attribute__((visibility("default"))) void zgpu_debug_p2_tail_time(unsigned long long *out, int reset)
{
    unsigned long long z[12] = {};
    hipMemcpyFromSymbol(out, HIP_SYMBOL(p2_tail_time), sizeof z);
    if (reset) hipMemcpyToSymbol(HIP_SYMBOL(p2_tail_time), z, sizeof z);
}
#define WT_T0() unsigned long long wt_prev_ = wall_clock64(), wt_acc_[10] = {0, 0, 0, 0, 0, 0, 0, 0, 0, 0}
#define WT_T(i) do { if (tid == 0) { const unsigned long long t_ = wall_clock64(); wt_acc_[i] += t_ - wt_prev_; wt_prev_ = t_; } } while (0)
#define WT_TEND(failed) do { if (tid == 0) { for (int i_ = 0; i_ < 10; i_++) atomicAdd(&p2_tail_time[i_], wt_acc_[i_]); atomicAdd(&p2_tail_time[10], 1ull); \
                                              if (failed) atomicAdd(&p2_tail_time[11], 1ull); } } while (0)
#else
#define WT_T0() do { } while (0)
#define WT_T(i) do { } while (0)
#define WT_TEND(failed) do { } while (0)
#endif

template <uint32_t T> __device__ __forceinline__ uint32_t tail_scan(uint32_t v, uint32_t *wtot, uint32_t tid, uint32_t &total)
{
    const uint32_t lane = tid & 63, wave = tid >> 6;
    uint32_t x = v;
#pragma unroll
    for (int d = 1; d < 64; d <<= 1) { const uint32_t y = __shfl_up(x, d); if ((int)lane >= d) x += y; }
    if (lane == 63) wtot[wave] = x;
    __syncthreads();
    uint32_t b = x - v, tot = 0;
    for (uint32_t w = 0; w < T / 64; w++) { const uint32_t t = wtot[w]; tot += t; if (w < wave) b += t; }
    total = tot;
    return b;
}

template <uint32_t T>
__device__ __forceinline__ bool tail_chunk(uint8_t *pl, const uint32_t *lcnt, const uint16_t *lpos, const uint32_t *lrec, const uint8_t *src, uint32_t n, uint32_t base,
                                           int slide_at, uint32_t *tok, ChunkMeta &out, uint32_t tid_all)
{
    using L = TailLds<T>;
    constexpr uint32_t kOwn = kP2Batch, kRun = 4 * kOwn * T;
    static_assert(kWtRounds % kP2Batch == 0 && kP2Wins == 8, "whole batches");
    uint32_t *const HAS = reinterpret_cast<uint32_t *>(pl + L::kHAS), *const COV = reinterpret_cast<uint32_t *>(pl + L::kCOV), *const MAT = reinterpret_cast<uint32_t *>(pl + L::kMAT),
             *const wbase = reinterpret_cast<uint32_t *>(pl + L::kWbase), *const MARK = reinterpret_cast<uint32_t *>(pl + L::kMARK), *const wtot = reinterpret_cast<uint32_t *>(pl + L::kWtot),
             *const flag = reinterpret_cast<uint32_t *>(pl + L::kFlag);
    uint16_t *const RC = reinterpret_cast<uint16_t *>(pl + L::kRC), *const N = reinterpret_cast<uint16_t *>(pl + L::kN), *const EX = reinterpret_cast<uint16_t *>(pl + L::kEX),
             *const ENT = reinterpret_cast<uint16_t *>(pl + L::kENT);
    uint32_t tid = tid_all;
#define WT_TID() do { tid = tid_all; asm volatile("" : "+v"(tid)); } while (0)
    WT_TID();
    const uint32_t lane = tid_all & 63, wave = tid_all >> 6;
    const uint32_t nwords = (n + 31) >> 5;
    const uint32_t *lpos2 = reinterpret_cast<const uint32_t *>(lpos);
    WT_T0();

    uint32_t cum[kP2Wins + 1];
    cum[0] = 0;
#pragma unroll
    for (uint32_t a = 0; a < kP2Wins; a++) cum[a + 1] = cum[a] + (uint32_t)__builtin_amdgcn_readfirstlane((int)lcnt[a]);
    const uint32_t nlog = cum[kP2Wins];
    for (uint32_t i = tid; i < kP2Words; i += T) { HAS[i] = 0; COV[i] = 0; MAT[i] = 0; }
    if (tid < L::kBlocks) ENT[tid] = (uint16_t)kWtNone;
    if (tid == 0) *flag = 0;
    auto slot_of = [&](uint32_t i) {
        const uint32_t f = i * T + tid;
        uint32_t at = f;
#pragma unroll
        for (uint32_t a = 1; a < kP2Wins; a++) at = f >= cum[a] ? a * kP2Win + (f - cum[a]) : at;
        return f < nlog ? at : 0u;
    };
    uint32_t gq[kWtRounds], gm[kWtRounds];
#pragma unroll
    for (uint32_t i = 0; i < kWtRounds; i++) {
        gq[i] = 0; gm[i] = 0;
        if (i * T < nlog) {
            const uint32_t at = slot_of(i);
            gq[i] = p2_ld<true>(lpos2 + (at >> 1));
            gm[i] = p2_ld<true>(lrec + at);
        }
    }
    __syncthreads();
    WT_TID();
    uint32_t gp[kWtRounds / 2];
    auto is_game = [&](uint32_t i) { return i * T + tid < nlog; };
    auto pos_of = [&](uint32_t i) { return (gp[i >> 1] >> ((i & 1u) << 4)) & 0xffffu; };
#pragma unroll
    for (uint32_t i = 0; i < kWtRounds; i += 2)
        gp[i >> 1] = ((gq[i] >> ((slot_of(i) & 1u) << 4)) & 0xffffu) | ((gq[i + 1] >> ((slot_of(i + 1) & 1u) << 4)) << 16);
#pragma unroll
    for (uint32_t i = 0; i < kWtRounds; i++) {
        if (!is_game(i)) gm[i] = 0;
        if (is_game(i)) { const uint32_t p = pos_of(i); atomicOr(&HAS[p >> 5], 1u << (p & 31u)); }
    }
    WT_T(0);

    WT_TID();
    constexpr uint32_t kPer = kP2Words / T;
    uint32_t nn;
    {
        uint32_t cnt[kPer], sum = 0;
        __syncthreads();
#pragma unroll
        for (uint32_t i = 0; i < kPer; i++) { cnt[i] = (uint32_t)__builtin_popcount(HAS[tid * kPer + i]); sum += cnt[i]; }
        uint32_t b = tail_scan<T>(sum, wtot, tid, nn);
#pragma unroll
        for (uint32_t i = 0; i < kPer; i++) { RC[tid * kPer + i] = (uint16_t)b; b += cnt[i]; }
        __syncthreads();
    }
#ifdef ZGPU_WALK_STATS
    if (tid == 0 && nn != nlog) atomicAdd(&walk_log_stats[5], 1ull);
#endif
    auto rank_of = [&](uint32_t p) { return (uint32_t)RC[p >> 5] + (uint32_t)__builtin_popcount(HAS[p >> 5] & ~(~0u << (p & 31u))); };
    WT_T(1);

    WT_TID();
#pragma unroll
    for (uint32_t i = 0; i < kWtRounds; i++) {
        if (is_game(i)) {
            const uint32_t p = pos_of(i), x = p + (gm[i] >> 24) + ((gm[i] >> 15) & 511u);
            uint32_t w = x >> 5, s = kWtNone;
            if (w < nwords) {
                uint32_t hv = HAS[w], v = hv & (~0u << (x & 31u));
                while (v == 0 && ++w < nwords) { hv = HAS[w]; v = hv; }
                if (v) s = (uint32_t)RC[w] + (uint32_t)__builtin_popcount(hv & ~(~0u << (uint32_t)__builtin_ctz(v)));
            }
            N[rank_of(p)] = (uint16_t)s;
        }
    }
    __syncthreads();
    WT_T(2);

    WT_TID();
    const uint32_t nblk = (nn + kWtBlk - 1) / kWtBlk, r0 = tid * kWtBlk, r1 = r0 + kWtBlk < nn ? r0 + kWtBlk : nn;
    uint64_t vis = 0;
    uint32_t myexit = kWtNone;
    if (tid < nblk) {
        uint32_t x = r0;
        while (x < r1) { vis |= 1ull << (x - r0); const uint32_t s = N[x]; x = s > x ? s : x + 1; }
        myexit = x;
        EX[tid] = (uint16_t)x;
    }
    __syncthreads();
    WT_T(3);

    WT_TID();
    if (wave == 0 && nn != 0) {
        uint32_t ex[L::kBlocks / 64];
#pragma unroll
        for (uint32_t j = 0; j < L::kBlocks / 64; j++) ex[j] = EX[j * 64 + lane];
        uint32_t cb = 0, ce = 0;
        for (uint32_t step = 0; step < L::kBlocks; step++) {
            if (lane == 0) ENT[cb] = (uint16_t)ce;
            uint32_t e = 0;
            const uint32_t hi = (uint32_t)__builtin_amdgcn_readfirstlane((int)(cb >> 6));
#pragma unroll
            for (uint32_t j = 0; j < L::kBlocks / 64; j++) if (hi == j) e = (uint32_t)__builtin_amdgcn_readlane((int)ex[j], (int)(cb & 63u));
            if (e == kWtNone) break;
            ce = e; cb = e / kWtBlk;
            if (cb >= L::kBlocks) break;
        }
    }
    __syncthreads();
    WT_T(4);

    WT_TID();
    if (tid < nblk) {
        uint32_t x = ENT[tid];
        uint64_t m = 0;
        bool met = false;
        const bool on = x != kWtNone;
        while (x < r1) {
            const uint64_t below = ~0ull << (x - r0);
            if ((vis >> (x - r0)) & 1ull) { m |= vis & below; met = true; break; }
            m |= below & ~(below << 1);
            const uint32_t s = N[x];
            x = s > x ? s : x + 1;
        }
        MARK[2 * tid] = (uint32_t)m; MARK[2 * tid + 1] = (uint32_t)(m >> 32);
        if (on && !met && x != myexit) *flag = 1;
    }
    __syncthreads();
    const bool ok = *flag == 0;
    WT_T(5);
    if (!ok) { WT_TEND(1); __syncthreads(); return false; }

    WT_TID();
    uint32_t onp = 0;
#pragma unroll
    for (uint32_t i = 0; i < kWtRounds; i++) {
        bool on_path = false;
        if (is_game(i)) { const uint32_t r = rank_of(pos_of(i)); on_path = (MARK[r >> 5] >> (r & 31u)) & 1u; }
        onp |= on_path ? 1u << i : 0u;
        if (on_path) {
            const uint32_t m = pos_of(i) + (gm[i] >> 24), Lm = (gm[i] >> 15) & 511u;
            atomicOr(&MAT[m >> 5], 1u << (m & 31u));
            const uint32_t a = m + 1, z = m + Lm;
            for (uint32_t wd = a >> 5; wd <= (z - 1) >> 5; wd++) {
                const uint32_t lo_b = wd == (a >> 5) ? (a & 31u) : 0u, hi_b = wd == ((z - 1) >> 5) ? ((z - 1) & 31u) : 31u;
                atomicOr(&COV[wd], (~0u << lo_b) & (~0u >> (31u - hi_b)));
            }
        }
    }
    __syncthreads();
    WT_T(6);

    WT_TID();
    uint32_t ntok;
    {
        uint32_t tw[kPer], sum = 0;
#pragma unroll
        for (uint32_t i = 0; i < kPer; i++) {
            const uint32_t wd = tid * kPer + i;
            tw[i] = wd < nwords ? ~COV[wd] : 0u;
            if (wd == nwords - 1 && (n & 31u)) tw[i] &= ~0u >> (32u - (n & 31u));
            sum += (uint32_t)__builtin_popcount(tw[i]);
        }
        uint32_t b = tail_scan<T>(sum, wtot, tid, ntok);
#pragma unroll
        for (uint32_t i = 0; i < kPer; i++) { const uint32_t wd = tid * kPer + i; wbase[wd] = b; COV[wd] = tw[i]; b += (uint32_t)__builtin_popcount(tw[i]); }
        __syncthreads();
    }
    const uint32_t *TOK = COV;
    auto index_of = [&](uint32_t p) { return wbase[p >> 5] + (uint32_t)__builtin_popcount(TOK[p >> 5] & ~(~0u << (p & 31u))); };
    WT_T(7);

    auto tok_put = [&](uint32_t idx, uint32_t v) { *reinterpret_cast<uint32_t *>(reinterpret_cast<uint8_t *>(tok) + (idx << 2)) = v; };
    WT_TID();
#pragma unroll
    for (uint32_t ib = 0; ib < kWtRounds; ib += kP2Batch) {
        if (ib * T < nlog) {
            uint32_t mx[kP2Batch], mt[kP2Batch];
#pragma unroll
            for (uint32_t u = 0; u < kP2Batch; u++) {
                const uint32_t gv = ((onp >> (ib + u)) & 1u) ? gm[ib + u] : 0u, m = pos_of(ib + u) + (gv >> 24);
                mt[u] = gv ? tok_match(gv & 32767u, ((gv >> 15) & 511u) - kMinMatch) : 0u;
                mx[u] = gv ? index_of(m) : kNone;
            }
#pragma unroll
            for (uint32_t u = 0; u < kP2Batch; u++) asm volatile("" : "+v"(mx[u]), "+v"(mt[u]));
#pragma unroll
            for (uint32_t u = 0; u < kP2Batch; u++) if (mx[u] != kNone) tok_put(mx[u], mt[u]);
        }
    }
    const uint32_t sa = (uint32_t)(reinterpret_cast<uintptr_t>(src) & 3u), dlast = (sa + n - 1) >> 2;
    const uint32_t *src4 = reinterpret_cast<const uint32_t *>(src - sa);
    auto run_fetch = [&](uint32_t w0, uint32_t (&lit)[kOwn]) {
        WT_TID();
#pragma unroll
        for (uint32_t i = 0; i < kOwn; i++) {
            const uint32_t d = w0 / 4 + i * T + tid;
            uint32_t v = 0;
            if (w0 < n) v = __builtin_amdgcn_alignbyte(src4[d + 1 < dlast ? d + 1 : dlast], src4[d < dlast ? d : dlast], sa);
            lit[i] = v;
        }
    };
    auto run_store = [&](uint32_t w0, uint32_t (&lit)[kOwn]) {
        WT_TID();
#pragma unroll
        for (uint32_t i = 0; i < kOwn; i++) {
            const uint32_t p = w0 + 4 * (i * T + tid), sh = p & 31u;
            const uint32_t tw = TOK[p >> 5], lw = ((tw & ~MAT[p >> 5]) >> sh) & 15u;
            uint32_t ix = wbase[p >> 5] + (uint32_t)__builtin_popcount(tw & ~(~0u << sh));
            asm volatile("" : "+v"(lit[i]), "+v"(ix));
#pragma unroll
            for (uint32_t j = 0; j < 4; j++) {
                if ((lw >> j) & 1u) tok_put(ix, tok_lit((lit[i] >> (8 * j)) & 255u));
                ix += (tw >> (sh + j)) & 1u;
            }
        }
    };
    {
        uint32_t la[kOwn], lb[kOwn];
        run_fetch(0, la);
        for (uint32_t w0 = 0; w0 < n; w0 += 2 * kRun) {
            run_fetch(w0 + kRun, lb);
            run_store(w0, la);
            run_fetch(w0 + 2 * kRun, la);
            if (w0 + kRun < n) run_store(w0 + kRun, lb);
        }
    }
    WT_T(8);

    WT_TID();
    if (tid == 0) parse_block_cuts(slide_at, base, TOK, MAT, wbase, n, nwords, kP2Words, ntok, out);
    WT_T(9);
    WT_TEND(0);
#undef WT_TID
    return true;
}

}
```

### zlib_amd/csrc/zgpu_lz_walk.hip

```cpp
#include "zgpu_lz_sorted.h"
#define ZGPU_PARSE_HEADER_ONLY
#include "zgpu_lz_parse.h"
#include <cstdlib>

namespace zgpu {

#ifndef ZGPU_WTRIG
#define ZGPU_WTRIG 48
#endif
#ifndef ZGPU_WBLK
#define ZGPU_WBLK 64
#endif
#ifndef ZGPU_WTAPER32
#define ZGPU_WTAPER32 16384
#endif
#ifndef ZGPU_WTAPER16
#define ZGPU_WTAPER16 4096
#endif
#ifndef ZGPU_WNEU_SHIFT
#define ZGPU_WNEU_SHIFT 0
#endif
#ifndef ZGPU_WFOLD_AT
#define ZGPU_WFOLD_AT 64
#endif
// ... 105 lines not shown
    constexpr uint32_t kCapNodes = (kM3DataLds - (kWords * 6 + 64)) / 2;
    static_assert(kCapNodes < 0x8000u && kCapNodes > kTileH1 / 3, "a path's game starts are three positions apart at least; different paths' need not be");
    const uint32_t lane = tid & 63, wave = tid >> 6;
    constexpr uint32_t per = kWords / T;
    uint32_t sum = 0, cnt[per];
#pragma unroll
    for (uint32_t i = 0; i < per; i++) {
        const uint32_t w = tid * per + i, v = __hip_atomic_load(gs + w, __ATOMIC_RELAXED, __HIP_MEMORY_SCOPE_AGENT);
        HAS[w] = v; cnt[i] = (uint32_t)__builtin_popcount(v); sum += cnt[i];
    }
    uint32_t x = sum;
#pragma unroll
    for (int d = 1; d < 64; d <<= 1) { const uint32_t y = __shfl_up(x, d); if ((int)lane >= d) x += y; }
    if (lane == 63) wtot[wave] = x;
    __syncthreads();
    uint32_t b = x - sum;
    for (uint32_t w = 0; w < wave; w++) b += wtot[w];
#pragma unroll
    for (uint32_t i = 0; i < per; i++) { wcnt[tid * per + i] = (uint16_t)b; b += cnt[i]; }
    __syncthreads();
    uint32_t nn = 0;
    for (uint32_t w = 0; w < T / 64; w++) nn += wtot[w];
    auto rank_of = [&](uint32_t p) { return (uint32_t)wcnt[p >> 5] + (uint32_t)__builtin_popcount(HAS[p >> 5] & ~(~0u << (p & 31u))); };
    if (nn > kCapNodes) {
        for (uint32_t k = tid; k < kTileExitStride; k += T) {
            uint32_t v = 0;
            if (k < nent) {
                const uint32_t e = h0 + k;
                uint32_t p = e < h1 ? next_bit(HAS, e, kWords) : kNone, x = e > h1 ? e : h1;
                while (p != kNone && p < h1) {
                    const uint32_t gv = __hip_atomic_load(gm + p, __ATOMIC_RELAXED, __HIP_MEMORY_SCOPE_AGENT), q = p + (gv >> 24) + ((gv >> 15) & 511u);
                    x = q > h1 ? q : h1;
                    p = q < h1 ? next_bit(HAS, q, kWords) : kNone;
                }
                v = x - h1;
            }
            exits[k] = (uint16_t)v;
        }
        return;
    }
    constexpr uint32_t kExit = 0x8000u;
    for (uint32_t p0 = h0 & ~31u; p0 < h1; p0 += T * 8) {
        uint32_t gv[8];
#pragma unroll
        for (uint32_t u = 0; u < 8; u++) { const uint32_t p = p0 + u * T + tid; gv[u] = p < h1 ? __hip_atomic_load(gm + p, __ATOMIC_RELAXED, __HIP_MEMORY_SCOPE_AGENT) : 0u; }
#pragma unroll
        for (uint32_t u = 0; u < 8; u++) {
            const uint32_t p = p0 + u * T + tid;
            if (p < h1 && ((HAS[p >> 5] >> (p & 31u)) & 1u)) {
                const uint32_t q = p + (gv[u] >> 24) + ((gv[u] >> 15) & 511u);
                uint32_t v = kExit | (q > h1 ? q - h1 : 0u);
                if (q < h1) { const uint32_t t = next_bit(HAS, q, kWords); if (t != kNone && t < h1) v = rank_of(t); }
                N[rank_of(p)] = (uint16_t)v;
            }
        }
    }
    __syncthreads();
    for (;;) {
        bool more = false;
        for (uint32_t i = tid; i < nn; i += T) {
            const uint32_t v = N[i];
            if (!(v & kExit)) { const uint32_t w = N[v]; N[i] = (uint16_t)w; more = more || !(w & kExit); }
        }
        if (!__syncthreads_or(more)) break;
    }
    for (uint32_t k = tid; k < kTileExitStride; k += T) {
        uint32_t v = 0;
        if (k < nent) {
            const uint32_t e = h0 + k, t = e < h1 ? next_bit(HAS, e, kWords) : kNone;
            v = (t == kNone || t >= h1) ? (e > h1 ? e - h1 : 0u) : ((uint32_t)N[rank_of(t)] & 0x7fffu);
        }
        exits[k] = (uint16_t)v;
    }
}

static_assert(kP2LogLdsBytes <= kWOffLcnt, "the parse works in the memory of the chunk bytes, the neutral bitmap and the rings");
}
#include "zgpu_lz_tail.h"
namespace zgpu {
constexpr uint32_t kWTailCap = TailLds<kWThreads>::kCap;
static_assert(TailLds<kWThreads>::kBytes <= kWOffLcnt && kWTailCap >= 12288, "the whole-chunk tail works in the same memory; every chunk of the bench corpora at levels 4-9 fits it (profiles/r07_walk_log_summary.txt)");
template <int MODE>
__global__ void __launch_bounds__(kWThreads, kWThreads / 128) walk_kernel(ChunkGeom g, LevelCfg cfg, const uint16_t *__restrict__ S_all, const uint32_t *__restrict__ ir_all,
                                                            uint32_t *__restrict__ gm_all, uint32_t *__restrict__ gs_all, uint32_t *__restrict__ tokens, ChunkMeta *meta, TileGeom tg, uint32_t tail_cap)
{
    static_assert(MODE == 1 || MODE == 2 || MODE == 3, "a chunk, a tile, a tile of a launch over many streams");
    constexpr bool FUSE = MODE == 1, TILE = MODE >= 2, ROWS = MODE == 3;
    static_assert(!FUSE || kWNeuShift == 0, "a log holds kP2Win games: a position must start one game at most, so every neutral position is claimed");
    extern __shared__ __attribute__((aligned(16))) uint32_t lds[];
    if constexpr (ROWS) { if (g.rows[blockIdx.x].n == 0) return; }
    uint32_t *d32 = lds;
    uint32_t *ctrl = lds + kM3DataLds / 4;
    uint32_t *NEU = ctrl + 4;
    uint32_t *lcnt = lds + kWOffLcnt / 4;
    const uint32_t c = blockIdx.x, tid = threadIdx.x, lane = tid & 63, wave = tid >> 6;
    const uint32_t ring = (uint32_t)__builtin_amdgcn_readfirstlane(lds_off(lds) + kM3DataLds + 16 + kWNeuBytes + wave * kM3WaveLds), slot = ring + kRing * 4;
    uint64_t lo; uint32_t n;
    chunk_span<ROWS>(g, c, lo, n);
    const uint8_t *src = g.in + lo;
    const uint16_t *S = S_all + (size_t)c * kSStride + kSPad;
    const uint32_t *ir = ir_all + (size_t)c * kChunkMax;
    uint32_t *gm = gm_all + (size_t)c * kChunkMax, *gs = gs_all + (size_t)c * (kChunkMax / 32);
    uint32_t *lrec = gm; uint16_t *lpos = reinterpret_cast<uint16_t *>(gs_all) + (size_t)c * kChunkMax;
    uint32_t th0 = 0, th1 = n, tnent = 0, tnent_all = 0, nil_local = ~0u;
    uint32_t base = chunk_base(g, c);
    if (TILE) {
        uint64_t wb; uint32_t nl;
        tile_span<ROWS>(g, tg, c, wb, nl, th0, th1, tnent);
        tnent_all = tnent;
        if (tnent > th1 - th0) tnent = th1 - th0;
        if constexpr (ROWS) { base = g.rows[c].base; nil_local = g.rows[c].nil_local; }
        else {
        base = (tg.abs0_nil && tg.abs0 + wb == 0) ? 0u : 1u;
        if (tg.nil_pos >= wb && tg.nil_pos - wb < kChunkMax) nil_local = (uint32_t)(tg.nil_pos - wb);
        }
    }
    const uint32_t npos = n >= 3 ? n - 2 : 0;
#ifdef ZGPU_P2_TIME
    const unsigned long long p2_t_in = wall_clock64();
#endif
    stage_chunk<kWThreads>(src, n, d32, tid);
    for (uint32_t i = tid; i < kChunkMax / 32; i += kWThreads) { if (i < kWNeuBytes / 4) NEU[i] = 0; if (!FUSE) gs[i] = 0; }
    if (tid < 8) d32[(kChunkMax + 64) / 4 + tid] = 0xffffffffu;
    if (tid == 0) ctrl[0] = 0;
    if (FUSE && tid < kP2Wins) lcnt[tid] = 0;
    __syncthreads();
    int slide_at;
    {
        const int room = (int)(2 * kWSize - base), b0 = (int)n < room ? (int)n : room;
        const int a = b0 - (int)kMinLookahead + 1, b = (int)(kWSize + kMaxDist) - (int)base;
        slide_at = a > b ? a : b;
    }
    const WalkTaper taper(n);
    const uint32_t chainF = cfg.chain, chainQ = cfg.chain >> 2, dbase = lds_off(d32), nblk = TILE ? tnent + (th1 - th0 - tnent + kWBlk - 1) / kWBlk : taper.nblk;
    const uint32_t wlim = TILE ? th1 : n;
    const bool vexact = (chainF & 7u) != 0 || (chainQ & 7u) != 0 || cfg.strategy == kRle;
    uint32_t lanebits = lane << 16;
    const uint32_t dummy = ring + (kRing - 1) * 4;
    uint32_t st = W_NEED, x = 0, handL = kMinMatch - 1, handM = 0, handD = 0, gstart = 0;
    uint32_t irx = 0, irn = 0, irE = 0, irl = 0;
    bool haveE = false;
    uint32_t rem = 0, best = kMinMatch - 1, key_seen = 0, sentinel = 0, boff = dbase + 1;
    uint32_t sw0 = 0, sw1 = 0;
    int gi = -(int)kSPad;
    uint32_t firstb = 0;
    uint4 G0 = make_uint4(0, 0, 0, 0), G1 = G0, G2 = G0, G3 = G0, F0 = G0, F1 = G0, F2 = G0, F3 = G0;
    uint32_t left = 0;
    bool cont = false;
    unsigned long long amask = 0, jmask = 0;
    uint32_t tail = 0;

    auto fold = [&]() {
        const uint32_t cnt = tail < 64 ? tail : 64;
        W_STAT(5, 1); W_STAT(6, cnt);
        tail = (uint32_t)__builtin_amdgcn_readfirstlane(tail - cnt);
        const uint32_t e = lds_ld32(ring + ((tail + lane) << 2));
        const uint32_t q = e & 0xffffu, o = (e >> 16) & 63u, qa = dbase + q;
        uint32_t po, xa, xb;
        {
            uint64_t va; uint32_t va2, ow0, ow1;
            asm volatile("ds_bpermute_b32 %0, %5, %6\n\tds_bpermute_b32 %1, %5, %7\n\tds_bpermute_b32 %2, %5, %8\n\t"
                         "ds_read2_b32 %3, %9 offset1:1\n\tds_read_b32 %4, %9 offset:8\n\ts_waitcnt lgkmcnt(0)"
                         : "=&v"(po), "=&v"(ow0), "=&v"(ow1), "=&v"(va), "=&v"(va2) : "v"(o << 2), "v"(x), "v"(sw0), "v"(sw1), "v"(qa & ~3u) : "memory");
            xa = __builtin_amdgcn_alignbyte((uint32_t)(va >> 32), (uint32_t)va, qa & 3) ^ ow0;
            xb = __builtin_amdgcn_alignbyte(va2, (uint32_t)(va >> 32), qa & 3) ^ ow1;
        }
        if (lane < cnt) {
// ... 180 lines not shown
#pragma unroll
                for (uint32_t j = 0; j < 8; j++) total += (uint32_t)__popcll(mm[j]);
                auto entry_of = [&](uint32_t j) -> uint32_t {
                    const uint32_t wd = j < 2 ? G0.w : j < 4 ? G0.z : j < 6 ? G0.y : G0.x, lb = j == 0 ? lf : lanebits;
                    return (j & 1) ? and_or(wd, 0xffffu, lb) : or_w1(lb, wd);
                };
                if (total) {
                    if (tail + total > kRing - 1) { while (tail) W_TF(fold()); }
                    if (total <= kRing - 1) {
                        uint32_t ta[8], te[8];
#pragma unroll
                        for (uint32_t j = 0; j < 8; j++) {
                            ta[j] = stack_slot(mm[j], ring + (tail << 2)); te[j] = entry_of(j);
                            tail += (uint32_t)__popcll(mm[j]);
                        }
                        tail = (uint32_t)__builtin_amdgcn_readfirstlane(tail);
                        unsigned long long sv;
                        asm volatile("s_mov_b64 %0, exec\n\t"
                                     "s_mov_b64 exec, %17\n\tds_write_b32 %1, %9\n\ts_mov_b64 exec, %18\n\tds_write_b32 %2, %10\n\t"
                                     "s_mov_b64 exec, %19\n\tds_write_b32 %3, %11\n\ts_mov_b64 exec, %20\n\tds_write_b32 %4, %12\n\t"
                                     "s_mov_b64 exec, %21\n\tds_write_b32 %5, %13\n\ts_mov_b64 exec, %22\n\tds_write_b32 %6, %14\n\t"
                                     "s_mov_b64 exec, %23\n\tds_write_b32 %7, %15\n\ts_mov_b64 exec, %24\n\tds_write_b32 %8, %16\n\t"
                                     "s_mov_b64 exec, %0"
                                     : "=&s"(sv)
                                     : "v"(ta[0]), "v"(ta[1]), "v"(ta[2]), "v"(ta[3]), "v"(ta[4]), "v"(ta[5]), "v"(ta[6]), "v"(ta[7]),
                                       "v"(te[0]), "v"(te[1]), "v"(te[2]), "v"(te[3]), "v"(te[4]), "v"(te[5]), "v"(te[6]), "v"(te[7]),
                                       "s"(mm[0]), "s"(mm[1]), "s"(mm[2]), "s"(mm[3]), "s"(mm[4]), "s"(mm[5]), "s"(mm[6]), "s"(mm[7]) : "memory");
                    } else {
#pragma unroll
                        for (uint32_t j = 0; j < 8; j++) {
                            if (mm[j]) {
                                stack_push(mm[j], (uint32_t)__builtin_amdgcn_readfirstlane(ring + (tail << 2)), dummy, entry_of(j));
                                tail = (uint32_t)__builtin_amdgcn_readfirstlane(tail + (uint32_t)__popcll(mm[j]));
                                if (tail >= kWFoldAt) W_TF(fold());
                            }
                        }
                    }
                    while (tail >= kWFoldAt) W_TF(fold());
                }
                amask &= mask_gt_u32(rem, 8u);
                firstb = sel_mask(amask0, 0u, firstb);
            }
            G0 = G1; G1 = G2; G2 = G3;
            left = left ? left - 1 : 0;
            if (first && jmask) {
                W_TK(if ((jmask >> lane) & 1ull) { G0 = F0; G1 = F1; G2 = F2; G3 = F3; left = 4; });
            }
            rem = sel_mask(amask0, rem > 8 ? rem - 8 : 0, rem);
            {
                const unsigned long long cm = amask & mask_eq_u32(left, 0u);
                cont = cont || ((cm >> lane) & 1ull);
                amask &= ~cm;
            }
            amask |= jmask; jmask = 0;
            if (amask == 0 || (uint32_t)__popcll(smask & ~amask) + idle >= kWTrig) break;
        }
        W_T(1);
    }
    if (TILE) {
        __syncthreads();
        W_TEND();
        tile_exits<kWThreads>(reinterpret_cast<uint8_t *>(lds), gm, gs, th0, th1, tnent_all, tg.exits + (size_t)c * kTileExitStride, tid);
        if (ROWS && tnent_all == 1) {
            __syncthreads();
            uint16_t *ex = tg.exits + (size_t)c * kTileExitStride;
            const uint16_t v = __hip_atomic_load(ex, __ATOMIC_RELAXED, __HIP_MEMORY_SCOPE_AGENT);
            for (uint32_t k = 1 + tid; k < kTileEntries; k += kWThreads) ex[k] = v;
        }
    }
    if (FUSE) {
        __syncthreads();
        W_TEND();
#ifdef ZGPU_P2_TIME
        if (tid == 0) atomicAdd(&p2_fused_time[7], wall_clock64() - p2_t_in);
#endif
#ifdef ZGPU_WALK_STATS
        if (tid < kP2Wins) { atomicAdd(&walk_log_stats[0], (unsigned long long)lcnt[tid]); atomicMax(&walk_log_stats[1], (unsigned long long)lcnt[tid]); }
#endif
        uint32_t nlog = 0;
#pragma unroll
        for (uint32_t a = 0; a < kP2Wins; a++) nlog += (uint32_t)__builtin_amdgcn_readfirstlane((int)lcnt[a]);
        const bool whole = tail_cap != 0 && nlog <= tail_cap;
        bool done = false;
        if (whole) done = tail_chunk<kWThreads>(reinterpret_cast<uint8_t *>(lds), lcnt, lpos, lrec, src, n, base, slide_at, tokens + (size_t)c * kChunkMax, meta[c], tid);
#ifdef ZGPU_WALK_STATS
        if (tid == 0) atomicAdd(&walk_log_stats[done ? 2 : whole ? 4 : 3], 1ull);
#endif
        if (!done) {
            constexpr uint32_t kP2Threads = kWThreads;
            constexpr bool LITE = true, FUSED = true, TILE = false, ROWS = false, LOG = true;
            const uint2 *recs = nullptr;
            const uint32_t *gmv_all = nullptr, *gsv_all = nullptr;
            uint8_t *pl = reinterpret_cast<uint8_t *>(lds);
            uint16_t *const J = reinterpret_cast<uint16_t *>(pl + kP2OffJ);
            uint32_t *const HAS = reinterpret_cast<uint32_t *>(pl + kP2OffHAS), *const MARK = reinterpret_cast<uint32_t *>(pl + kP2OffMARK), *const COV = reinterpret_cast<uint32_t *>(pl + kP2OffCOV),
                     *const MAT = reinterpret_cast<uint32_t *>(pl + kP2OffMAT), *const wbase = reinterpret_cast<uint32_t *>(pl + kP2OffWbase), *const VIS = reinterpret_cast<uint32_t *>(pl + kP2OffVIS),
                     *const EXITS = reinterpret_cast<uint32_t *>(pl + kP2OffEXITS), *const wave_tot = reinterpret_cast<uint32_t *>(pl + kP2OffWtot);
            uint32_t &sh_entry = *reinterpret_cast<uint32_t *>(pl + kP2OffEntry), &sh_exit = *reinterpret_cast<uint32_t *>(pl + kP2OffEntry + 4);
            uint16_t *const END = reinterpret_cast<uint16_t *>(pl + kP2OffEND);
#include "zgpu_lz_parse_body.inc"
        }
    }
}

template <int MODE> static void launch_walk(const ChunkGeom &g, LevelCfg cfg, const SortedWs &ws, uint32_t *tokens, ChunkMeta *meta, const TileGeom &tg, hipStream_t st)
{
    static bool opt_in = false;
    if (!opt_in) { hipFuncSetAttribute(reinterpret_cast<const void *>(walk_kernel<MODE>), hipFuncAttributeMaxDynamicSharedMemorySize, (int)kWLds); opt_in = true; }
    uint32_t *games = MODE == 1 ? ws.lrec() : ws.gm(), *starts = MODE == 1 ? reinterpret_cast<uint32_t *>(ws.lpos()) : ws.gs();
    uint32_t tail_cap = kWTailCap;
    if (MODE == 1) { const char *v = getenv("ZGPU_WALK_TAIL_CAP"); char *end = nullptr; const unsigned long x = v ? strtoul(v, &end, 10) : 0; if (v && end != v) tail_cap = x < kWTailCap ? (uint32_t)x : kWTailCap; }
    hipLaunchKernelGGL(walk_kernel<MODE>, dim3(g.nchunks), dim3(kWThreads), kWLds, st, g, cfg, ws.S, ws.ir, games, starts, tokens, meta, tg, tail_cap);
}
void launch_walk_chunks(const ChunkGeom &g, LevelCfg cfg, const SortedWs &ws, uint32_t *tokens, ChunkMeta *meta, hipStream_t st) { launch_walk<1>(g, cfg, ws, tokens, meta, TileGeom{}, st); }
void launch_walk_tiles(const ChunkGeom &g, const TileGeom &tg, LevelCfg cfg, const SortedWs &ws, ChunkMeta *meta, hipStream_t st)
{
    if (geom_rows(g)) launch_walk<3>(g, cfg, ws, nullptr, meta, tg, st);
    else launch_walk<2>(g, cfg, ws, nullptr, meta, tg, st);
}

}
```

### zlib_amd/gpu.py

```python
import ctypes as C
import os

_HERE = os.path.dirname(os.path.abspath(__file__))
_lib = None

F_FINAL, F_ZLIB_WRAP, F_POS0, F_POS0_ALL, F_GZIP_WRAP, F_CRC32, F_CONTINUOUS, F_BGZF_WRAP = 1, 2, 4, 8, 16, 32, 64, 128
BGZF_BLOCK = 65280
CONT_MORE, CONT_FLUSH, CONT_FINISH = 0, 1, 2
WHOLE_STREAM = 0xFFFFFFFF
LZ_AUTO, LZ_SERIAL, LZ_PARALLEL, LZ_SORTED, LZ_WALK, LZ_FAST, LZ_FASTWIN = 0, 1, 2, 3, 4, 5, 6
CHECK_ADLER32, CHECK_CRC32 = 1, 2
WRAP_RAW, WRAP_ZLIB, WRAP_GZIP, WRAP_AUTO = 0, 1, 2, 3
_WRAPS = {"raw": WRAP_RAW, "zlib": WRAP_ZLIB, "gzip": WRAP_GZIP, "auto": WRAP_AUTO}
JOB_DECODE, JOB_SIZES, JOB_VERIFY, JOB_PACKED = 0, 1, 2, 3
BUF_ERROR = -5
STAGES = ["chain", "match", "parse", "lz_serial", "huffman", "stitch", "inflate"]
CHUNK = 65536


class EngineError(RuntimeError):
    def __init__(self, code, msg):
        super().__init__("zgpu error %d: %s" % (code, msg))
        self.code = code

# ... 83 lines not shown
    L.zgpu_deflate_segments_device.argtypes = [vp, vp, u64, vp, u64, C.POINTER(_Params), vp, u64, vp, C.POINTER(DeflateResult), vp]
    L.zgpu_deflate_segments_items_host.argtypes = [vp, vp, vp, u64, C.POINTER(_Params), vp, u64, vp, C.POINTER(DeflateResult), vp]
    L.zgpu_deflate_segments_items_device.argtypes = [vp, vp, u64, vp, u64, C.POINTER(_Params), vp, u64, vp, C.POINTER(DeflateResult), vp, vp]
    L.zgpu_deflate_batch_workspace_bytes.argtypes = [u64, u32]
    L.zgpu_deflate_batch_workspace_bytes.restype = u64
    L.zgpu_deflate_batch_enqueue.argtypes = [vp, vp, u64, vp, u64, C.POINTER(_Params), vp, u64, vp, vp, vp, vp, u64, u32, vp]
    L.zgpu_deflate_batch_packed_enqueue.argtypes = [vp, vp, u64, vp, u64, C.POINTER(_Params), vp, u64, vp, vp, vp, vp, u64, u32, vp]
    L.zgpu_deflate_streams_bound.argtypes = [u64, u32]
    L.zgpu_deflate_streams_bound.restype = u64
    L.zgpu_deflate_streams_layout.argtypes = [vp, u64, u32, vp, C.POINTER(u64)]
    L.zgpu_deflate_streams_device.argtypes = [vp, vp, u64, vp, u64, C.POINTER(_Params), vp, u64, vp, vp, C.POINTER(DeflateResult), vp]
    L.zgpu_deflate_streams_host.argtypes = [vp, vp, vp, u64, C.POINTER(_Params), vp, u64, vp, vp, C.POINTER(DeflateResult)]
    L.zgpu_deflate_streams_workspace_bytes.argtypes = [u64, u64, u32]
    L.zgpu_deflate_streams_workspace_bytes.restype = u64
    L.zgpu_deflate_streams_rooms_bound.argtypes = [u64, u64, u32]
    L.zgpu_deflate_streams_rooms_bound.restype = u64
    L.zgpu_deflate_streams_layout_enqueue.argtypes = [vp, vp, u64, u64, u32, vp, vp]
    L.zgpu_deflate_streams_enqueue.argtypes = [vp, vp, u64, vp, u64, C.POINTER(_Params), vp, u64, vp, vp, vp, vp, u64, u32, vp]
    L.zgpu_engine_set_exact_sort.argtypes = [vp, C.c_int]
    L.zgpu_debug_sort_fallback.argtypes = [vp]
    L.zgpu_checksum_batch_host.argtypes = [vp, vp, u64, vp, u64, u32, vp]
    L.zgpu_checksum_batch_device.argtypes = [vp, vp, u64, vp, u64, u32, vp, vp]
    L.zgpu_inflate_device.argtypes = [vp, vp, u64, vp, u64, u32, vp, u64, C.POINTER(InflateResult), vp]
    L.zgpu_inflate_host.argtypes = [vp, vp, u64, vp, u64, u32, vp, u64, C.POINTER(InflateResult)]
    L.zgpu_deflate_segments_bound.argtypes = [u64, u64, u32]
    L.zgpu_deflate_segments_bound.restype = u64
    L.zgpu_inflate_batch_device.argtypes = [vp, vp, u64, vp, u64, C.c_int, u32, vp, u64, vp, vp, C.POINTER(u64), vp]
    L.zgpu_inflate_batch_host.argtypes = [vp, vp, u64, vp, u64, C.c_int, u32, vp, u64, vp, vp, C.POINTER(u64)]
    L.zgpu_inflate_batch_sizes_device.argtypes = [vp, vp, u64, vp, u64, C.c_int, vp, C.POINTER(u64), vp]
    L.zgpu_inflate_batch_sizes_host.argtypes = [vp, vp, u64, vp, u64, C.c_int, vp, C.POINTER(u64)]
    L.zgpu_inflate_batch_packed_device.argtypes = [vp, vp, u64, vp, u64, C.c_int, u32, u32, vp, u64, vp, vp, C.POINTER(u64), C.POINTER(u64), vp]
    L.zgpu_inflate_batch_packed_host.argtypes = [vp, vp, u64, vp, u64, C.c_int, u32, u32, vp, u64, vp, vp, C.POINTER(u64), C.POINTER(u64)]
    L.zgpu_inflate_batch_verify_device.argtypes = [vp, vp, u64, vp, u64, C.c_int, u32, vp, C.POINTER(u64), vp]
    L.zgpu_inflate_batch_verify_host.argtypes = [vp, vp, u64, vp, u64, C.c_int, u32, vp, C.POINTER(u64)]
    L.zgpu_inflate_batch_workspace_bytes.argtypes = [C.c_int, u64]
    L.zgpu_inflate_batch_workspace_bytes.restype = u64
    L.zgpu_inflate_batch_enqueue.argtypes = [vp, vp, u64, vp, u64, C.c_int, u32, vp, u64, vp, vp, vp, vp, u64, vp]
    L.zgpu_inflate_batch_sizes_enqueue.argtypes = [vp, vp, u64, vp, u64, C.c_int, vp, vp, vp, u64, vp]
    L.zgpu_inflate_batch_verify_enqueue.argtypes = [vp, vp, u64, vp, u64, C.c_int, u32, vp, vp, vp, u64, vp]
    L.zgpu_inflate_batch_packed_enqueue.argtypes = [vp, vp, u64, vp, u64, C.c_int, u32, u32, vp, u64, vp, vp, vp, vp, u64, vp]
    L.zgpu_bgzf_verify_device.argtypes = [vp, vp, u64, vp, C.POINTER(InflateResult), vp]
    L.zgpu_bgzf_verify_host.argtypes = [vp, vp, u64, vp, C.POINTER(InflateResult)]
    L.zgpu_bgzf_bound.argtypes = [u64, u32]
    L.zgpu_bgzf_bound.restype = u64
    L.zgpu_bgzf_deflate_device.argtypes = [vp, vp, u64, C.c_int, C.c_int, u32, vp, u64, vp, C.POINTER(DeflateResult), vp]
    L.zgpu_bgzf_deflate_host.argtypes = [vp, vp, u64, C.c_int, C.c_int, u32, vp, u64, vp, C.POINTER(DeflateResult)]
    L.zgpu_bgzf_index_device.argtypes = [vp, vp, u64, vp, vp, u64, C.POINTER(u64), C.POINTER(u64), C.POINTER(u32), vp]
    L.zgpu_bgzf_inflate_device.argtypes = [vp, vp, u64, vp, u64, vp, C.POINTER(InflateResult), vp]
    L.zgpu_bgzf_inflate_host.argtypes = [vp, vp, u64, vp, u64, vp, C.POINTER(InflateResult)]
    L.zgpu_gzip_inflate_device.argtypes = [vp, vp, u64, vp, u64, vp, vp, vp, u64, C.POINTER(u64), C.POINTER(InflateResult), vp]
    L.zgpu_gzip_inflate_host.argtypes = [vp, vp, u64, vp, u64, vp, vp, vp, u64, C.POINTER(u64), C.POINTER(InflateResult)]
    L.zgpu_gzip_members_count.argtypes = [C.c_int]
    L.zgpu_gzip_members_count.restype = u64
    L.zgpu_inflate_find_chunks_host.argtypes = [vp, vp, u64, u32, vp, u64, C.POINTER(u64)]
    L.zgpu_inflate_stream_host2.argtypes = [vp, vp, u64, u32, vp, u64, C.POINTER(InflateResult)]
    L.zgpu_inflate_stream_host3.argtypes = [vp, vp, u64, u32, u32, vp, u64, C.POINTER(InflateResult)]
    L.zgpu_comm_unique_id.argtypes = [vp]
    L.zgpu_comm_create.argtypes = [C.c_int, C.c_int, C.c_int, vp, C.POINTER(vp)]
    L.zgpu_comm_destroy.argtypes = [vp]
    L.zgpu_comm_destroy.restype = None
    L.zgpu_comm_error.restype = C.c_char_p
    L.zgpu_gather_layout.argtypes = [C.c_int, vp, vp, C.POINTER(u64)]
    L.zgpu_gather_layout.restype = None
    L.zgpu_deflate_gather_sizes.argtypes = [vp, u64, u32, u64, vp, C.POINTER(u64), vp]
    L.zgpu_deflate_gather.argtypes = [vp, vp, vp, C.c_int, vp, u64, C.POINTER(u32), vp]
    L.zgpu_inflate_spec_count.argtypes = [C.c_int]
    L.zgpu_inflate_spec_count.restype = u64
    L.zgpu_inflate_message.argtypes = [u32]
    L.zgpu_inflate_message.restype = C.c_char_p
    L.zgpu_adler32_device.argtypes = [vp, vp, u64, C.POINTER(u32), vp]
    L.zgpu_crc32_device.argtypes = [vp, vp, u64, C.POINTER(u32), vp]
    L.zgpu_deflate_dict_chunk_host.argtypes = [vp, vp, u32, u32, vp, vp, u64, vp]
    L.zgpu_inflate_set_dictionary.argtypes = [vp, vp, u32]
    L.zgpu_inflate_set_checks.argtypes = [vp, u32]
    L.zgpu_profile_enable.argtypes = [vp, C.c_int]
    L.zgpu_profile_enable.restype = None
    L.zgpu_profile_reset.argtypes = [vp]
    L.zgpu_profile_reset.restype = None
    L.zgpu_profile_get.argtypes = [vp, C.c_int, C.POINTER(C.c_double), C.POINTER(u64)]
    L.zgpu_stage_name.argtypes = [C.c_int]
    L.zgpu_stage_name.restype = C.c_char_p
    L.zgpu_deflate_fast_count.argtypes = [vp, C.c_int]
    L.zgpu_deflate_fast_count.restype = u64
    L.zgpu_corpus_fill_device.argtypes = [vp, u32, u64, u64, u64, vp, vp]
    _lib = L
    return L


class Engine:

    def __init__(self, device=0):
        self.L = load_library()
        h = C.c_void_p()
        rc = self.L.zgpu_engine_create(device, C.byref(h))
        if rc != 0:
            raise EngineError(rc, "cannot create engine on device %d (%d visible)" % (device, self.L.zgpu_device_count()))
        self.h = h

    def close(self):
        if self.h:
            self.L.zgpu_engine_destroy(self.h)
            self.h = None

    def __del__(self):
        try:
            self.close()
        except Exception:
            pass

    def _check(self, rc):
        if rc != 0:
            raise EngineError(rc, self.L.zgpu_engine_error(self.h).decode())

    def inflate_set_dictionary(self, dictionary):
        d = bytes(dictionary) if dictionary else b""
        self._check(self.L.zgpu_inflate_set_dictionary(self.h, d if d else None, len(d)))

    def inflate_set_checks(self, mask):
        self._check(self.L.zgpu_inflate_set_checks(self.h, mask))

    def deflate_dict_chunk_host(self, dictionary, chunk, level, final, strategy=0, flags=0):
        import numpy as np
        d = bytes(dictionary)[-32506:]
        buf = np.frombuffer(d + bytes(chunk) + b"\0", dtype=np.uint8)
        n = len(d) + len(chunk)
        cap = self.L.zgpu_deflate_bound(n, CHUNK)
        out = np.empty(cap, dtype=np.uint8)
        p = _Params(level, CHUNK, flags | (F_FINAL if final else 0), LZ_AUTO, strategy, 0)
        res = DeflateResult()
        self._check(self.L.zgpu_deflate_dict_chunk_host(self.h, buf.ctypes.data, n, len(d), C.byref(p), out.ctypes.data, cap, C.byref(res)))
        self.last = res
        return out[: res.out_bytes].tobytes()

    def deflate_host(self, data, level, flags=F_FINAL | F_ZLIB_WRAP, chunk_size=CHUNK, lz_impl=LZ_AUTO, want_offsets=False, strategy=0, prime=(0, 0)):
        import numpy as np
        arr = np.frombuffer(data, dtype=np.uint8) if not hasattr(data, "ctypes") else data
        n = int(arr.size)
        cap = self.L.zgpu_deflate_bound_geometry(n, chunk_size, *getattr(self, "geometry", (15, 8)))
        if flags & F_CONTINUOUS:
            cap = self.L.zgpu_deflate_cont_bound(n) + 32
        out = np.empty(cap, dtype=np.uint8)
        nchunks = max(1, (n + chunk_size - 1) // chunk_size)
        offs = np.zeros(nchunks + 1, dtype=np.uint64)
        p = _Params(level, chunk_size, flags, lz_impl, strategy, (prime[0] << 16) | (prime[1] & 0xffff))
        res = DeflateResult()
        src = arr.ctypes.data if n else None
        self._check(self.L.zgpu_deflate_host(self.h, src, n, C.byref(p), out.ctypes.data, cap,
                                             offs.ctypes.data if want_offsets else None, C.byref(res)))
        self.last = res
        z = out[: res.out_bytes].tobytes()
        return (z, offs) if want_offsets else z

    def cont_new(self):
        import numpy as np
        cs = ContState(0, 0, 0, 0, 0, 0, 2, 1, 8)
        return cs, (np.zeros(16384, dtype=np.uint32), np.zeros(1040, dtype=np.uint32))

    def deflate_cont_host(self, buf, check_from, level, mode, cs, carry, strategy=0, flags=0, excl=(), split=None):
        import numpy as np
        arr = np.frombuffer(bytes(buf) + b"\0", dtype=np.uint8)
        n = int(arr.size) - 1
        split = 0 if split is None else min(max(split, 0), n)
        cap = self.L.zgpu_deflate_cont_bound(n) + 64
        out = np.empty(cap, dtype=np.uint8)
        p = _Params(level, 0, flags, LZ_AUTO, strategy, 0)
        res = DeflateResult()
        ex = np.ascontiguousarray(list(excl) + [0], dtype=np.uint64)
        self._check(self.L.zgpu_deflate_cont_host(self.h, arr.ctypes.data, split, arr.ctypes.data + split, n - split, check_from, C.byref(p), mode, C.byref(cs), carry[0].ctypes.data,
                                                  carry[1].ctypes.data, ex.ctypes.data, len(excl), out.ctypes.data, cap, C.byref(res)))
        self.last = res
        return out[: res.out_bytes].tobytes()

    def set_geometry(self, window_bits=15, mem_level=8):
        self._check(self.L.zgpu_deflate_set_geometry(self.h, window_bits, mem_level))
        self.geometry = (window_bits, mem_level)

    FAST_COUNTS = ("rounds", "tile_parses", "same_entry", "stopped_early", "different_token", "reach_to_end", "windows_to_diff", "windows_of_diff")

    def fast_round_counts(self):
        return {k: int(self.L.zgpu_deflate_fast_count(self.h, i)) for i, k in enumerate(self.FAST_COUNTS)}

    def set_tuning(self, tune=None):
        g, l, n, c = tune if tune else (0, 0, 0, 0)
        self._check(self.L.zgpu_deflate_set_tuning(self.h, 1 if tune else 0, g, l, n, c))

    def deflate_segments_host(self, buffers, level, flags=0, lz_impl=LZ_AUTO, want_items=False, strategy=0):
        import numpy as np
        sizes = [len(b) for b in buffers]
        offs = np.zeros(len(buffers) + 1, dtype=np.uint64)
        offs[1:] = np.cumsum(sizes)
        blob = np.frombuffer(b"".join(buffers) + b"\0", dtype=np.uint8)
        cap = int(offs[-1]) + 40 * len(buffers) + 64
        if getattr(self, "geometry", (15, 8)) != (15, 8):
            cap = int(offs[-1]) + len(buffers) * (12288 + 5 * 520)
        out = np.empty(cap, dtype=np.uint8)
        ooffs = np.zeros(len(buffers) + 1, dtype=np.uint64)
        p = _Params(level, 0, flags, lz_impl, strategy, 0)
        res = DeflateResult()
        if want_items:
            cap += 26 * len(buffers)
            out = np.empty(cap, dtype=np.uint8)
            items = (DeflateItem * max(len(buffers), 1))()
            self._check(self.L.zgpu_deflate_segments_items_host(self.h, blob.ctypes.data, offs.ctypes.data, len(buffers), C.byref(p),
                                                                out.ctypes.data, cap, ooffs.ctypes.data, C.byref(res), items))
        else:
            self._check(self.L.zgpu_deflate_segments_host(self.h, blob.ctypes.data, offs.ctypes.data, len(buffers), C.byref(p),
                                                          out.ctypes.data, cap, ooffs.ctypes.data, C.byref(res)))
        self.last = res
        raw = out[: res.out_bytes].tobytes()
        segs = [raw[int(ooffs[i]): int(ooffs[i + 1])] for i in range(len(buffers))]
        if want_items:
            return segs, [(it.out_lo, it.out_bytes, it.in_bytes, it.data_type, it.adler32, it.crc32) for it in items[: len(buffers)]]
        return segs

    def checksum_batch_host(self, data, offsets, checks=CHECK_ADLER32 | CHECK_CRC32, items=None):
        import numpy as np
        arr = data if hasattr(data, "ctypes") else np.frombuffer(bytes(data) + b"\0", dtype=np.uint8)[:-1]
        offs = np.ascontiguousarray(offsets, dtype=np.uint64)
        n = len(offs) - 1
        given = items is not None
        if not given:
            items = (CheckItem * max(n, 1))()
        self._check(self.L.zgpu_checksum_batch_host(self.h, arr.ctypes.data if arr.size else None, arr.size, offs.ctypes.data, n, checks, items))
        return items if given else [(items[k].adler32, items[k].crc32) for k in range(n)]

    def checksum_batch_device(self, d_in, in_bytes, d_offsets, n, d_items, checks=CHECK_ADLER32 | CHECK_CRC32, stream=None):
        self._check(self.L.zgpu_checksum_batch_device(self.h, d_in, in_bytes, d_offsets, n, checks, d_items, stream))

    def deflate_batch_host(self, buffers, level, wrap="zlib", strategy=0):
        import numpy as np
        flags = F_FINAL | {"raw": 0, "zlib": F_ZLIB_WRAP, "gzip": F_GZIP_WRAP}[wrap]
        sizes = [len(b) for b in buffers]
        offs = np.zeros(len(buffers) + 1, dtype=np.uint64)
        offs[1:] = np.cumsum(sizes)
        blob = np.frombuffer(b"".join(bytes(b) for b in buffers) + b"\0", dtype=np.uint8)
        cap = int(self.L.zgpu_deflate_segments_bound(len(buffers), int(offs[-1]), flags))
        out = np.empty(cap, dtype=np.uint8)
        ooffs = np.zeros(len(buffers) + 1, dtype=np.uint64)
        p = _Params(level, 0, flags, LZ_AUTO, strategy, 0)
        res = DeflateResult()
        self._check(self.L.zgpu_deflate_segments_host(self.h, blob.ctypes.data, offs.ctypes.data, len(buffers), C.byref(p),
                                                      out.ctypes.data, cap, ooffs.ctypes.data, C.byref(res)))
        self.last = res
        raw = out[: res.out_bytes].tobytes()
        return [raw[int(ooffs[i]): int(ooffs[i + 1])] for i in range(len(buffers))]

    def deflate_streams_host(self, items, level, wrap="zlib", strategy=0, flags=0, want_items=False):
        import numpy as np
        flags = flags | F_FINAL | {"raw": 0, "zlib": F_ZLIB_WRAP, "gzip": F_GZIP_WRAP}[wrap]
        n = len(items)
        offs = np.zeros(n + 1, dtype=np.uint64)
        offs[1:] = np.cumsum([len(b) for b in items])
        blob = np.frombuffer(b"".join(bytes(b) for b in items) + b"\0", dtype=np.uint8)
        ooffs = np.zeros(n + 1, dtype=np.uint64)
        total = C.c_uint64(0)
        self._check(self.L.zgpu_deflate_streams_layout(offs.ctypes.data, n, flags, ooffs.ctypes.data, C.byref(total)))
        cap = int(total.value)
        out = np.empty(cap + 1, dtype=np.uint8)
        recs = (DeflateBatchItem * max(n, 1))()
        p = _Params(level, 0, flags, LZ_AUTO, strategy, 0)
        res = DeflateResult()
        self._check(self.L.zgpu_deflate_streams_host(self.h, blob.ctypes.data, offs.ctypes.data, n, C.byref(p), out.ctypes.data, cap, ooffs.ctypes.data, recs, C.byref(res)))
        self.last = res
# ... 416 lines not shown
```

Baseline: 32.22.

## Build block symbol histograms in the LZ tail and reuse them in Huffman

The whole-chunk LZ tail now counts literal/length and distance symbols per deflate block in LDS while it writes tokens. It stores these counts, plus each block's byte length, into the sorted workspace, and flags the chunk with a bit in nostore. When that bit is set, the Huffman kernel loads the precomputed histogram instead of re-reading all tokens and running LDS atomics per block. The cost is extra LDS atomics and a global write inside the LZ stage, and a dependency on the workspace keeping the counts until the Huffman stage reads them.

Result: no change. 32.24, median of 6 (+0.1%).

```diff
diff --git a/include/zamd_gpu.h b/include/zamd_gpu.h
--- a/include/zamd_gpu.h
+++ b/include/zamd_gpu.h
@@ -319,6 +319,13 @@
 };
 uint64_t zgpu_deflate_fast_count(zgpu_engine *e, int which);
 
+enum {
+    ZGPU_TAIL_BLOCKS_FROM_COUNTS = 0,
+    ZGPU_TAIL_BLOCKS_FROM_TOKENS,
+    ZGPU_TAIL_COUNT_N
+};
+uint64_t zgpu_deflate_tail_count(zgpu_engine *e, int which);
+
 int zgpu_corpus_fill_device(zgpu_engine *e, uint32_t kind, uint64_t seed, uint64_t first_chunk, uint64_t nchunks,
                             void *d_out, void *hip_stream);
 
diff --git a/zlib_amd/csrc/zgpu_codes.h b/zlib_amd/csrc/zgpu_codes.h
--- /dev/null
+++ b/zlib_amd/csrc/zgpu_codes.h
@@ -0,0 +1,28 @@
+#pragma once
+#include <stdint.h>
+#ifndef __host__
+#define __host__
+#define __device__
+#endif
+
+namespace zgpu {
+
+__host__ __device__ inline void len_code_of(uint32_t lc, uint32_t &code, uint32_t &extra)
+{
+    const uint32_t e = (31u - (uint32_t)__builtin_clz(lc | 8u)) - 2u;
+    const bool small = lc < 8, top = lc == 255;
+    code = small ? lc : top ? 28u : 4u * e + 4u + ((lc >> e) & 3u);
+    extra = (small || top) ? 0u : e;
+}
+__host__ __device__ inline void dist_code_bits(uint32_t d, uint32_t &code, uint32_t &extra)
+{
+    const uint32_t msb = 31u - (uint32_t)__builtin_clz(d | 2u);
+    const bool small = d < 4;
+    code = small ? d : 2u * msb + ((d >> (msb - 1u)) & 1u);
+    extra = small ? 0u : msb - 1u;
+}
+
+constexpr uint32_t kCntBlocks = 5, kCntSyms = 320, kCntDist = 286, kCntBlockBytes = kCntSyms * 2, kCntStoredWord = (286 + 30) / 2, kCntChunkBytes = kCntBlocks * kCntBlockBytes;
+static_assert(kCntStoredWord * 2 + 2 <= kCntSyms, "the block's byte count lies behind its last count");
+
+}
diff --git a/zlib_amd/csrc/zgpu_common.h b/zlib_amd/csrc/zgpu_common.h
--- a/zlib_amd/csrc/zgpu_common.h
+++ b/zlib_amd/csrc/zgpu_common.h
@@ -17,6 +17,7 @@
 constexpr uint32_t kGeoSlotStride = 65536 + 8192 + 1024 + 64 + 5 * 32 * kGeoNostoreWords + 448;
 constexpr uint32_t kMaxBlocks = 6;
 constexpr uint32_t kFullFinalBlock = 1u << 31;
+constexpr uint32_t kTailCounts = 1u << 30, kTailCountsStride = kChunkMax;
 constexpr uint32_t kHandedOn = 0xFFFFFFFFu;
 constexpr int kLCodes = 286, kDCodes = 30, kBLCodes = 19, kHeapSize = 2 * kLCodes + 1, kMaxBits = 15, kMaxBLBits = 7;
 constexpr int kEndBlock = 256;
diff --git a/zlib_amd/csrc/zgpu_deflate.hip b/zlib_amd/csrc/zgpu_deflate.hip
--- a/zlib_amd/csrc/zgpu_deflate.hip
+++ b/zlib_amd/csrc/zgpu_deflate.hip
@@ -261,7 +261,7 @@
     uint8_t *const slots = pl.geo ? e->geo_slots : e->slots;
     {
         StageTimer t(e, st, ZGPU_STAGE_HUFFMAN);
-        launch_huffman(g, e->tokens, e->meta, slots, st, pl.cfg.strategy == kFixed);
+        launch_huffman(g, e->tokens, e->meta, slots, st, pl.cfg.strategy == kFixed, pl.serial ? nullptr : lz_sorted_tail_counts(e->par_ws, g.nchunks, pl.impl), tail_stat_buf(e));
     }
     StageTimer t(e, st, ZGPU_STAGE_STITCH);
     if (!adler_done) launch_adler(g, e->meta, st);
diff --git a/zlib_amd/csrc/zgpu_deflate_batch.hip b/zlib_amd/csrc/zgpu_deflate_batch.hip
--- a/zlib_amd/csrc/zgpu_deflate_batch.hip
+++ b/zlib_amd/csrc/zgpu_deflate_batch.hip
@@ -243,6 +243,7 @@
     g.in = w.stage; g.in_bytes = (uint64_t)w.round * kDwsStageBytes; g.chunk_size = kChunkMax;
     g.final_chunk = ~0ull; g.all_final = 1; g.block_tokens = kBlockTokens; g.slot_stride = kSlotStride;
     const uint32_t frame = bc.fh.n + bc.tail;
+    unsigned long long *const stat = tail_stat_buf(e);
     for (uint64_t c0 = 0; c0 < n; c0 += w.round) {
         const uint32_t nb = (uint32_t)(n - c0 < w.round ? n - c0 : w.round);
         const uint64_t *const t = w.pre;
@@ -250,7 +251,7 @@
         hipLaunchKernelGGL(dbatch_check_kernel, dim3(1), dim3(1024), 0, st, d_in_off, n, in_bytes, bc.limit, d_out_off, out_cap, packed ? 1u : 0u, c0, nb, w.lo, w.pre, w.state, w.cnt);
         hipLaunchKernelGGL(dbatch_gather_kernel, dim3(nb), dim3(256), 0, st, static_cast<const uint8_t *>(d_in), w.lo, w.state, t, nb, w.stage);
         const bool adler_done = launch_lz_sorted(g, bc.cfg, w.sorted, w.tokens, w.meta, st, nullptr, e->exact_sort, bc.impl);
-        launch_huffman(g, w.tokens, w.meta, w.slots, st, bc.cfg.strategy == kFixed);
+        launch_huffman(g, w.tokens, w.meta, w.slots, st, bc.cfg.strategy == kFixed, lz_sorted_tail_counts(w.sorted, g.nchunks, bc.impl), stat);
         if (!adler_done) launch_adler(g, w.meta, st);
         if (bc.with_crc) launch_crc(g, w.meta, st);
         if (packed) hipLaunchKernelGGL(dbatch_scan_kernel, dim3(1), dim3(1024), 0, st, w.meta, w.state, c0, nb, frame, d_out_off, w.cnt);
diff --git a/zlib_amd/csrc/zgpu_engine.h b/zlib_amd/csrc/zgpu_engine.h
--- a/zlib_amd/csrc/zgpu_engine.h
+++ b/zlib_amd/csrc/zgpu_engine.h
@@ -90,6 +90,7 @@
     hipStream_t ct_stream = nullptr; hipEvent_t ct_ev_a[2] = {nullptr, nullptr}, ct_ev_b[2] = {nullptr, nullptr};
     uint64_t cf_rounds = 0, cf_tile_parses = 0;
     uint64_t cf_stat[6] = {};
+    DevBuf<unsigned long long> tail_stat;
     DevBuf<uint32_t> bz_cnt, bz_isize, bz_jump_a, bz_jump_b, bz_reach, bz_res;
     DevBuf<uint64_t> bz_base, bz_pos, bz_next, bz_in_off, bz_out_off;
     DevBuf<zgpu_inflate_item> bz_items;
@@ -123,6 +124,7 @@
     ~StageTimer() { prof_span_end(e, st, stage, a); }
 };
 uint32_t env_u32(const char *name, uint32_t dflt);
+unsigned long long *tail_stat_buf(zgpu_engine *e);
 int checksum_pass(zgpu_engine *e, const uint8_t *d_bytes, uint64_t nbytes, uint32_t mask, uint32_t batch_cap, DevBuf<ChunkMeta> &meta, hipStream_t st, uint32_t *adler, uint32_t *crc);
 
 int ensure_deflate_ws(zgpu_engine *e, uint32_t batch, bool serial, uint64_t nchunks_total, bool geo = false);
@@ -139,7 +141,7 @@
 
 void launch_lz_serial(const ChunkGeom &g, LevelCfg cfg, uint4 *tables, uint32_t *tokens, ChunkMeta *meta, hipStream_t st, uint32_t *nostore_bits, bool hand_on, uint32_t tag);
 
-void launch_huffman(const ChunkGeom &g, const uint32_t *tokens, ChunkMeta *meta, uint8_t *slots, hipStream_t st, bool fixed_trees);
+void launch_huffman(const ChunkGeom &g, const uint32_t *tokens, ChunkMeta *meta, uint8_t *slots, hipStream_t st, bool fixed_trees, const uint32_t *counts, unsigned long long *path_stat);
 void launch_huffman_cont(const ChunkGeom &g, const uint32_t *compact_tokens, uint32_t nblk, ContBlk *blk, ContState *cst, uint8_t *slots, hipStream_t st, bool fixed_trees);
 void launch_huffman_streams(const ChunkGeom &g, const uint32_t *batch_tokens, uint32_t nslots, ContBlk *blk, ContState *states, const uint32_t *blk_item, uint8_t *slots, hipStream_t st,
                             bool fixed_trees);
@@ -169,6 +171,7 @@
 
 size_t lz_sorted_workspace_bytes(uint32_t batch_chunks);
 uint32_t *lz_sorted_fault_word(void *workspace);
+const uint32_t *lz_sorted_tail_counts(void *workspace, uint32_t nchunks, int impl);
 bool launch_lz_sorted(const ChunkGeom &g, LevelCfg cfg, void *workspace, uint32_t *tokens, ChunkMeta *meta, hipStream_t st, zgpu_engine *prof, int exact_sort,
                       int impl);
 void launch_lz_tiles(const ChunkGeom &g, const TileGeom &tg, LevelCfg cfg, void *workspace, ChunkMeta *meta, uint16_t *comp, uint16_t *gentry, hipStream_t st, zgpu_engine *prof,
diff --git a/zlib_amd/csrc/zgpu_engine.hip b/zlib_amd/csrc/zgpu_engine.hip
--- a/zlib_amd/csrc/zgpu_engine.hip
+++ b/zlib_amd/csrc/zgpu_engine.hip
@@ -45,6 +45,15 @@
     if (!v || !*v) return dflt;
     long x = strtol(v, nullptr, 10);
     return x > 0 ? (uint32_t)x : dflt;
+}
+
+unsigned long long *tail_stat_buf(zgpu_engine *e)
+{
+    if (!e || !getenv("ZGPU_TAIL_STATS")) return nullptr;
+    bool grew = false;
+    if (e->tail_stat.reserve(nullptr, ZGPU_TAIL_COUNT_N, &grew) != ZGPU_OK) return nullptr;
+    if (grew && (hipMemset(e->tail_stat, 0, ZGPU_TAIL_COUNT_N * sizeof(unsigned long long)) != hipSuccess || hipDeviceSynchronize() != hipSuccess)) { e->tail_stat.release(); return nullptr; }
+    return e->tail_stat;
 }
 
 int ensure_stage(zgpu_engine *e, uint64_t in_bytes, uint64_t out_bytes)
@@ -183,6 +192,15 @@
     return which == ZGPU_FAST_ROUNDS ? e->cf_rounds : which == ZGPU_FAST_TILE_PARSES ? e->cf_tile_parses : e->cf_stat[which - ZGPU_FAST_SAME_ENTRY];
 }
 
+uint64_t zgpu_deflate_tail_count(zgpu_engine *e, int which)
+{
+    if (!e || which < 0 || which >= ZGPU_TAIL_COUNT_N || !e->tail_stat) return 0;
+    unsigned long long v[ZGPU_TAIL_COUNT_N] = {};
+    if (hipSetDevice(e->device) != hipSuccess || hipDeviceSynchronize() != hipSuccess) return 0;
+    if (hipMemcpy(v, e->tail_stat, sizeof v, hipMemcpyDeviceToHost) != hipSuccess) return 0;
+    return v[which];
+}
+
 int zgpu_corpus_fill_device(zgpu_engine *e, uint32_t kind, uint64_t seed, uint64_t first_chunk, uint64_t nchunks, void *d_out, void *hip_stream)
 {
     if (!e || !d_out) return fail(e, ZGPU_STREAM_ERROR, "null argument");
diff --git a/zlib_amd/csrc/zgpu_huffman.hip b/zlib_amd/csrc/zgpu_huffman.hip
--- a/zlib_amd/csrc/zgpu_huffman.hip
+++ b/zlib_amd/csrc/zgpu_huffman.hip
@@ -1,5 +1,6 @@
 #include "zgpu_common.h"
 #include "zgpu_engine.h"
+#include "zgpu_codes.h"
 
 namespace zgpu {
 
@@ -381,21 +382,6 @@
     return done;
 }
 
-__device__ inline void len_code_of(uint32_t lc, uint32_t &code, uint32_t &extra)
-{
-    const uint32_t e = (31u - (uint32_t)__clz((int)(lc | 8u))) - 2u;
-    const bool small = lc < 8, top = lc == 255;
-    code = small ? lc : top ? 28u : 4u * e + 4u + ((lc >> e) & 3u);
-    extra = (small || top) ? 0u : e;
-}
-__device__ inline void dist_code_bits(uint32_t d, uint32_t &code, uint32_t &extra)
-{
-    const uint32_t msb = 31u - (uint32_t)__clz((int)(d | 2u));
-    const bool small = d < 4;
-    code = small ? d : 2u * msb + ((d >> (msb - 1u)) & 1u);
-    extra = small ? 0u : msb - 1u;
-}
-
 __device__ inline void token_bits(uint32_t t, const uint16_t *lcode, const uint8_t *llen, const uint16_t *dcode, const uint8_t *dlen,
                                   uint64_t &bits, uint32_t &nb)
 {
@@ -460,12 +446,13 @@
 #endif
 template <bool CONT, bool MULTI = false>
 __global__ void __launch_bounds__(kThreads, ZGPU_HUF_WAVES) huffman_kernel(ChunkGeom g, const uint32_t *__restrict__ tokens, ChunkMeta *meta, uint8_t *slots, uint32_t fixed_trees,
-                                                                            ContBlk *blk, ContState *cst, const uint32_t *__restrict__ blk_item)
+                                                                            ContBlk *blk, ContState *cst, const uint32_t *__restrict__ blk_item,
+                                                                            const uint32_t *__restrict__ counts, unsigned long long *path_stat)
 {
     static_assert(CONT || !MULTI, "many streams' blocks are continuous streams' blocks");
     __shared__ __attribute__((aligned(16))) TreeWork work0;
     __shared__ TreeWorkD work1;
-    __shared__ uint32_t hist[kLCodes + kDCodes + 2];
+    __shared__ __attribute__((aligned(16))) uint32_t hist[kLCodes + kDCodes + 2];
     __shared__ uint16_t lcode[kLCodes + 2], dcode[kDCodes + 2], blcode[kBLCodes + 1];
     __shared__ uint8_t llen[kLCodes + 2], dlen[kDCodes + 2], bllen[kBLCodes + 1];
     __shared__ uint32_t tmp[4];
@@ -489,6 +476,8 @@
     const bool final_chunk_here = CONT ? blk[c].eof != 0 : chunk_is_final(g, c);
     const uint32_t btok = g.block_tokens, nblocks = CONT ? 1u : ntok / btok + ((nostore & kFullFinalBlock) ? 0u : 1u);
     const uint32_t *nostore_bits = (!CONT && g.nostore_bits) ? g.nostore_bits + (size_t)c * kGeoNostoreWords : nullptr;
+    const bool counted = !CONT && counts != nullptr && (nostore & kTailCounts) != 0 && btok == kBlockTokens;
+    const uint32_t *crec = counts + (size_t)c * kTailCountsStride;
     uint32_t block_start = CONT ? 0u : chunk_skip(g, c), data_type = 2;
     if (tid == 0) { const uint32_t pr = CONT ? 0u : chunk_prime(g, c); sh_bitpos = pr >> 16; sh_carry = pr & 0xffffu; }
     HUF_T0();
@@ -496,6 +485,15 @@
     for (uint32_t b = 0; b < nblocks; b++) {
         const uint32_t t0 = b * btok, t1 = (b + 1 == nblocks) ? ntok : t0 + btok, nt = t1 - t0;
         const uint32_t eof = (final_chunk_here && b + 1 == nblocks) ? 1u : 0u;
+        uint32_t stored_len;
+        if (counted) {
+            const uint32_t *rec = crec + b * (kCntBlockBytes / 4);
+            if (tid < kCntStoredWord / 2) {
+                const uint2 v = reinterpret_cast<const uint2 *>(rec)[tid];
+                *reinterpret_cast<uint4 *>(&hist[4 * tid]) = make_uint4(v.x & 0xffffu, v.x >> 16, v.y & 0xffffu, v.y >> 16);
+            }
+            stored_len = rec[kCntStoredWord];
+        } else {
         for (uint32_t i = tid; i < kLCodes + kDCodes + 2; i += kThreads) hist[i] = 0;
         __syncthreads();
         uint32_t bytes = 0;
@@ -511,7 +509,9 @@
                 else { uint32_t c, xl, dc, xd; len_code_of(lc, c, xl); dist_code_bits(dist - 1, dc, xd); atomicAdd(&hist[257 + c], 1u); atomicAdd(&hist[kLCodes + dc], 1u); bytes += lc + 3; }
             }
         }
-        const uint32_t stored_len = block_reduce_add(bytes, tmp);
+        stored_len = block_reduce_add(bytes, tmp);
+        }
+        if (!CONT && path_stat && tid == 0) atomicAdd(&path_stat[counted ? 0 : 1], 1ull);
         __syncthreads();
         if (tid == 0) hist[kEndBlock] = 1;
         __syncthreads();
@@ -690,18 +690,18 @@
     HUF_TEND();
 }
 
-void launch_huffman(const ChunkGeom &g, const uint32_t *tokens, ChunkMeta *meta, uint8_t *slots, hipStream_t st, bool fixed_trees)
-{
-    hipLaunchKernelGGL(huffman_kernel<false>, dim3(g.nchunks), dim3(kThreads), 0, st, g, tokens, meta, slots, fixed_trees ? 1u : 0u, nullptr, nullptr, nullptr);
+void launch_huffman(const ChunkGeom &g, const uint32_t *tokens, ChunkMeta *meta, uint8_t *slots, hipStream_t st, bool fixed_trees, const uint32_t *counts, unsigned long long *path_stat)
+{
+    hipLaunchKernelGGL(huffman_kernel<false>, dim3(g.nchunks), dim3(kThreads), 0, st, g, tokens, meta, slots, fixed_trees ? 1u : 0u, nullptr, nullptr, nullptr, counts, path_stat);
 }
 void launch_huffman_cont(const ChunkGeom &g, const uint32_t *compact_tokens, uint32_t nblk, ContBlk *blk, ContState *cst, uint8_t *slots, hipStream_t st, bool fixed_trees)
 {
-    if (nblk) hipLaunchKernelGGL(huffman_kernel<true>, dim3(nblk), dim3(kThreads), 0, st, g, compact_tokens, nullptr, slots, fixed_trees ? 1u : 0u, blk, cst, nullptr);
+    if (nblk) hipLaunchKernelGGL(huffman_kernel<true>, dim3(nblk), dim3(kThreads), 0, st, g, compact_tokens, nullptr, slots, fixed_trees ? 1u : 0u, blk, cst, nullptr, nullptr, nullptr);
 }
 void launch_huffman_streams(const ChunkGeom &g, const uint32_t *batch_tokens, uint32_t nslots, ContBlk *blk, ContState *states, const uint32_t *blk_item, uint8_t *slots, hipStream_t st,
                             bool fixed_trees)
 {
-    if (nslots) hipLaunchKernelGGL((huffman_kernel<true, true>), dim3(nslots), dim3(kThreads), 0, st, g, batch_tokens, nullptr, slots, fixed_trees ? 1u : 0u, blk, states, blk_item);
-}
-
-}
+    if (nslots) hipLaunchKernelGGL((huffman_kernel<true, true>), dim3(nslots), dim3(kThreads), 0, st, g, batch_tokens, nullptr, slots, fixed_trees ? 1u : 0u, blk, states, blk_item, nullptr, nullptr);
+}
+
+}
diff --git a/zlib_amd/csrc/zgpu_lz_parse.h b/zlib_amd/csrc/zgpu_lz_parse.h
--- a/zlib_amd/csrc/zgpu_lz_parse.h
+++ b/zlib_amd/csrc/zgpu_lz_parse.h
@@ -53,10 +53,11 @@
     return (w << 5) + (uint32_t)__builtin_ctz(v);
 }
 
-__device__ inline void parse_block_cuts(int slide_at, uint32_t base, const uint32_t *TOK, const uint32_t *MAT, const uint32_t *wbase, uint32_t n, uint32_t nwords, uint32_t nw_done,
-                                        uint32_t ntok, ChunkMeta &out)
+__device__ inline uint32_t parse_block_cuts(int slide_at, uint32_t base, const uint32_t *TOK, const uint32_t *MAT, const uint32_t *wbase, uint32_t n, uint32_t nwords, uint32_t nw_done,
+                                        uint32_t ntok, ChunkMeta &out, uint32_t *starts = nullptr, uint32_t flags = 0)
 {
-    uint32_t nostore = 0, nblk = 0, block_start = 0;
+    uint32_t nostore = flags, nblk = 0, block_start = 0;
+    if (starts) starts[0] = 0;
     for (uint32_t b = 0;; b++) {
         const uint32_t e = (b + 1) * kBlockTokens - 1;
         if (e >= ntok) break;
@@ -71,9 +72,12 @@
         if (is_mat) { ns = next_bit(TOK, pe + 1, nwords); if (ns == kNone) ns = n; }
         if ((int)(pe + 1) >= slide_at && block_start + base < kWSize) nostore |= 1u << nblk;
         nblk++; block_start = ns;
+        if (starts) starts[nblk] = ns;
     }
+    if (starts) starts[nblk + 1] = n;
     if ((int)n >= (int)(kWSize + kMaxDist) - (int)base && block_start + base < kWSize) nostore |= 1u << nblk;
     out.ntok = ntok; out.nostore = nostore; out.in_bytes = n;
+    return nblk;
 }
 
 #ifdef ZGPU_P2_TIME
diff --git a/zlib_amd/csrc/zgpu_lz_sorted.h b/zlib_amd/csrc/zgpu_lz_sorted.h
--- a/zlib_amd/csrc/zgpu_lz_sorted.h
+++ b/zlib_amd/csrc/zgpu_lz_sorted.h
@@ -2,6 +2,7 @@
 #include "zgpu_common.h"
 #include "zgpu_engine.h"
 #include "zgpu_deflate_batch_plan.h"
+#include "zgpu_codes.h"
 
 namespace zgpu {
 
@@ -35,6 +36,7 @@
     uint16_t *lpos() const { return reinterpret_cast<uint16_t *>(lrec() + nch * kChunkMax); }
     uint8_t *G() const { return reinterpret_cast<uint8_t *>(recs); }
 };
+static_assert(SortedWs::kIrBytes == kTailCountsStride * 4 && kCntChunkBytes <= SortedWs::kIrBytes, "a chunk's counts record lies in its ir");
 
 static_assert(SortedWs::kHeaderBytes == kDwsSortedHeader && SortedWs::kSlack == kDwsSortedSlack && SortedWs::bytes(1) == kDwsSortedHeader + kDwsSortedChunk + kDwsSortedSlack &&
               SortedWs::bytes(3) - SortedWs::bytes(2) == kDwsSortedChunk, "zgpu_deflate_batch_plan.h states the workspace of a chunk as numbers");
diff --git a/zlib_amd/csrc/zgpu_lz_sorted.hip b/zlib_amd/csrc/zgpu_lz_sorted.hip
--- a/zlib_amd/csrc/zgpu_lz_sorted.hip
+++ b/zlib_amd/csrc/zgpu_lz_sorted.hip
@@ -4,6 +4,7 @@
 
 size_t lz_sorted_workspace_bytes(uint32_t batch) { return SortedWs::bytes(batch); }
 uint32_t *lz_sorted_fault_word(void *workspace) { return SortedWs(workspace, 0).fault; }
+const uint32_t *lz_sorted_tail_counts(void *workspace, uint32_t nchunks, int impl) { return impl == ZGPU_LZ_WALK ? SortedWs(workspace, nchunks).ir : nullptr; }
 
 bool launch_lz_sorted(const ChunkGeom &g, LevelCfg cfg, void *workspace, uint32_t *tokens, ChunkMeta *meta, hipStream_t st, zgpu_engine *prof, int exact_sort, int impl)
 {
diff --git a/zlib_amd/csrc/zgpu_lz_tail.h b/zlib_amd/csrc/zgpu_lz_tail.h
--- a/zlib_amd/csrc/zgpu_lz_tail.h
+++ b/zlib_amd/csrc/zgpu_lz_tail.h
@@ -1,6 +1,9 @@
 #pragma once
+#include "zgpu_codes.h"
 
 namespace zgpu {
+
+static_assert((kChunkMax + kBlockTokens - 1) / kBlockTokens <= kCntBlocks && kBlockTokens < 65536, "a chunk's tokens lie in kCntBlocks blocks; a count fits 16 bits");
 
 constexpr uint32_t kWtRounds = 24, kWtBlk = 64, kWtNone = 0xffffu;
 template <uint32_t T> struct TailLds {
@@ -8,7 +11,11 @@
     static constexpr uint32_t kBlocks = kCap / kWtBlk;
     static constexpr uint32_t kHAS = 0, kCOV = kHAS + kP2Words * 4, kMAT = kCOV + kP2Words * 4, kWbase = kMAT + kP2Words * 4, kRC = kWbase + (kP2Words + 4) * 4,
                               kN = kRC + kP2Words * 2, kMARK = kN + kCap * 2, kEX = kMARK + kCap / 8, kENT = kEX + kBlocks * 2, kWtot = kENT + kBlocks * 2,
-                              kFlag = kWtot + 64, kBytes = kFlag + 16;
+                              kFlag = kWtot + 64,
+                              kCNT = kFlag + 16,
+                              kStarts = kCNT + kCntBlocks * kCntSyms * 4,
+                              kBytes = kStarts + 32;
+    static_assert(kCNT % 16 == 0, "the counts are zeroed sixteen bytes a lane");
     static_assert(kCap < kWtNone && kCap % kWtBlk == 0 && kBlocks % 64 == 0 && kBlocks <= T && kP2Words % T == 0 && T % 64 == 0 && T / 64 <= 16, "workgroup size");
 };
 
@@ -46,14 +53,14 @@
 
 template <uint32_t T>
 __device__ __forceinline__ bool tail_chunk(uint8_t *pl, const uint32_t *lcnt, const uint16_t *lpos, const uint32_t *lrec, const uint8_t *src, uint32_t n, uint32_t base,
-                                           int slide_at, uint32_t *tok, ChunkMeta &out, uint32_t tid_all)
+                                           int slide_at, uint32_t *tok, ChunkMeta &out, uint32_t tid_all, uint32_t *cnt_out)
 {
     using L = TailLds<T>;
     constexpr uint32_t kOwn = kP2Batch, kRun = 4 * kOwn * T;
     static_assert(kWtRounds % kP2Batch == 0 && kP2Wins == 8, "whole batches");
     uint32_t *const HAS = reinterpret_cast<uint32_t *>(pl + L::kHAS), *const COV = reinterpret_cast<uint32_t *>(pl + L::kCOV), *const MAT = reinterpret_cast<uint32_t *>(pl + L::kMAT),
              *const wbase = reinterpret_cast<uint32_t *>(pl + L::kWbase), *const MARK = reinterpret_cast<uint32_t *>(pl + L::kMARK), *const wtot = reinterpret_cast<uint32_t *>(pl + L::kWtot),
-             *const flag = reinterpret_cast<uint32_t *>(pl + L::kFlag);
+             *const flag = reinterpret_cast<uint32_t *>(pl + L::kFlag), *const CNT = reinterpret_cast<uint32_t *>(pl + L::kCNT), *const starts = reinterpret_cast<uint32_t *>(pl + L::kStarts);
     uint16_t *const RC = reinterpret_cast<uint16_t *>(pl + L::kRC), *const N = reinterpret_cast<uint16_t *>(pl + L::kN), *const EX = reinterpret_cast<uint16_t *>(pl + L::kEX),
              *const ENT = reinterpret_cast<uint16_t *>(pl + L::kENT);
     uint32_t tid = tid_all;
@@ -195,6 +202,8 @@
     if (!ok) { WT_TEND(1); __syncthreads(); return false; }
 
     WT_TID();
+    if (cnt_out && tid < kCntBlocks * kCntSyms / 4) reinterpret_cast<uint4 *>(CNT)[tid] = make_uint4(0, 0, 0, 0);
+    static_assert(kCntBlocks * kCntSyms / 4 <= T, "one store a lane");
     uint32_t onp = 0;
 #pragma unroll
     for (uint32_t i = 0; i < kWtRounds; i++) {
@@ -235,6 +244,12 @@
     WT_T(7);
 
     auto tok_put = [&](uint32_t idx, uint32_t v) { *reinterpret_cast<uint32_t *>(reinterpret_cast<uint8_t *>(tok) + (idx << 2)) = v; };
+    auto cnt_add = [&](uint32_t idx, uint32_t sym) { __hip_atomic_fetch_add(&CNT[(idx / kBlockTokens) * kCntSyms + sym], 1u, __ATOMIC_RELAXED, __HIP_MEMORY_SCOPE_WORKGROUP); };
+    auto cnt_match = [&](uint32_t idx, uint32_t v) {
+        uint32_t lc, xl, dc, xd;
+        len_code_of(v & 255u, lc, xl); dist_code_bits((v >> 8) - 1u, dc, xd);
+        cnt_add(idx, 257u + lc); cnt_add(idx, kCntDist + dc);
+    };
     WT_TID();
 #pragma unroll
     for (uint32_t ib = 0; ib < kWtRounds; ib += kP2Batch) {
@@ -249,7 +264,7 @@
 #pragma unroll
             for (uint32_t u = 0; u < kP2Batch; u++) asm volatile("" : "+v"(mx[u]), "+v"(mt[u]));
 #pragma unroll
-            for (uint32_t u = 0; u < kP2Batch; u++) if (mx[u] != kNone) tok_put(mx[u], mt[u]);
+            for (uint32_t u = 0; u < kP2Batch; u++) if (mx[u] != kNone) { tok_put(mx[u], mt[u]); if (cnt_out) cnt_match(mx[u], mt[u]); }
         }
     }
     const uint32_t sa = (uint32_t)(reinterpret_cast<uintptr_t>(src) & 3u), dlast = (sa + n - 1) >> 2;
@@ -274,7 +289,7 @@
             asm volatile("" : "+v"(lit[i]), "+v"(ix));
 #pragma unroll
             for (uint32_t j = 0; j < 4; j++) {
-                if ((lw >> j) & 1u) tok_put(ix, tok_lit((lit[i] >> (8 * j)) & 255u));
+                if ((lw >> j) & 1u) { tok_put(ix, tok_lit((lit[i] >> (8 * j)) & 255u)); if (cnt_out) cnt_add(ix, (lit[i] >> (8 * j)) & 255u); }
                 ix += (tw >> (sh + j)) & 1u;
             }
         }
@@ -292,7 +307,21 @@
     WT_T(8);
 
     WT_TID();
-    if (tid == 0) parse_block_cuts(slide_at, base, TOK, MAT, wbase, n, nwords, kP2Words, ntok, out);
+    if (tid == 0) {
+        const uint32_t nb = parse_block_cuts(slide_at, base, TOK, MAT, wbase, n, nwords, kP2Words, ntok, out, cnt_out ? starts : nullptr, cnt_out ? kTailCounts : 0u) + 1;
+        if (cnt_out) starts[7] = nb < kCntBlocks ? nb : kCntBlocks;
+    }
+    if (cnt_out) {
+        __syncthreads();
+        const uint32_t nw = starts[7] * (kCntBlockBytes / 4);
+        for (uint32_t w = tid; w < nw; w += T) {
+            const uint32_t b = w / (kCntBlockBytes / 4), k = w % (kCntBlockBytes / 4);
+            uint32_t v = 0;
+            if (k < kCntStoredWord) { const uint2 c2 = *reinterpret_cast<const uint2 *>(&CNT[b * kCntSyms + 2 * k]); v = c2.x | (c2.y << 16); }
+            else if (k == kCntStoredWord) v = starts[b + 1] - starts[b];
+            cnt_out[w] = v;
+        }
+    }
     WT_T(9);
     WT_TEND(0);
 #undef WT_TID
diff --git a/zlib_amd/csrc/zgpu_lz_walk.hip b/zlib_amd/csrc/zgpu_lz_walk.hip
--- a/zlib_amd/csrc/zgpu_lz_walk.hip
+++ b/zlib_amd/csrc/zgpu_lz_walk.hip
@@ -211,7 +211,7 @@
 static_assert(TailLds<kWThreads>::kBytes <= kWOffLcnt && kWTailCap >= 12288, "the whole-chunk tail works in the same memory; every chunk of the bench corpora at levels 4-9 fits it (profiles/r07_walk_log_summary.txt)");
 template <int MODE>
 __global__ void __launch_bounds__(kWThreads, kWThreads / 128) walk_kernel(ChunkGeom g, LevelCfg cfg, const uint16_t *__restrict__ S_all, const uint32_t *__restrict__ ir_all,
-                                                            uint32_t *__restrict__ gm_all, uint32_t *__restrict__ gs_all, uint32_t *__restrict__ tokens, ChunkMeta *meta, TileGeom tg, uint32_t tail_cap)
+                                                            uint32_t *__restrict__ gm_all, uint32_t *__restrict__ gs_all, uint32_t *__restrict__ tokens, ChunkMeta *meta, TileGeom tg, uint32_t tail_cap, uint32_t tail_counts)
 {
     static_assert(MODE == 1 || MODE == 2 || MODE == 3, "a chunk, a tile, a tile of a launch over many streams");
     constexpr bool FUSE = MODE == 1, TILE = MODE >= 2, ROWS = MODE == 3;
@@ -558,7 +558,8 @@
         for (uint32_t a = 0; a < kP2Wins; a++) nlog += (uint32_t)__builtin_amdgcn_readfirstlane((int)lcnt[a]);
         const bool whole = tail_cap != 0 && nlog <= tail_cap;
         bool done = false;
-        if (whole) done = tail_chunk<kWThreads>(reinterpret_cast<uint8_t *>(lds), lcnt, lpos, lrec, src, n, base, slide_at, tokens + (size_t)c * kChunkMax, meta[c], tid);
+        if (whole) done = tail_chunk<kWThreads>(reinterpret_cast<uint8_t *>(lds), lcnt, lpos, lrec, src, n, base, slide_at, tokens + (size_t)c * kChunkMax, meta[c], tid,
+                                                   tail_counts ? const_cast<uint32_t *>(ir) : nullptr);
 #ifdef ZGPU_WALK_STATS
         if (tid == 0) atomicAdd(&walk_log_stats[done ? 2 : whole ? 4 : 3], 1ull);
 #endif
@@ -586,7 +587,9 @@
     uint32_t *games = MODE == 1 ? ws.lrec() : ws.gm(), *starts = MODE == 1 ? reinterpret_cast<uint32_t *>(ws.lpos()) : ws.gs();
     uint32_t tail_cap = kWTailCap;
     if (MODE == 1) { const char *v = getenv("ZGPU_WALK_TAIL_CAP"); char *end = nullptr; const unsigned long x = v ? strtoul(v, &end, 10) : 0; if (v && end != v) tail_cap = x < kWTailCap ? (uint32_t)x : kWTailCap; }
-    hipLaunchKernelGGL(walk_kernel<MODE>, dim3(g.nchunks), dim3(kWThreads), kWLds, st, g, cfg, ws.S, ws.ir, games, starts, tokens, meta, tg, tail_cap);
+    uint32_t tail_counts = 0;
+    if (MODE == 1) { const char *v = getenv("ZGPU_TAIL_COUNTS"); tail_counts = (v && v[0] == '0' && v[1] == 0) ? 0u : 1u; }
+    hipLaunchKernelGGL(walk_kernel<MODE>, dim3(g.nchunks), dim3(kWThreads), kWLds, st, g, cfg, ws.S, ws.ir, games, starts, tokens, meta, tg, tail_cap, tail_counts);
 }
 void launch_walk_chunks(const ChunkGeom &g, LevelCfg cfg, const SortedWs &ws, uint32_t *tokens, ChunkMeta *meta, hipStream_t st) { launch_walk<1>(g, cfg, ws, tokens, meta, TileGeom{}, st); }
 void launch_walk_tiles(const ChunkGeom &g, const TileGeom &tg, LevelCfg cfg, const SortedWs &ws, ChunkMeta *meta, hipStream_t st)
diff --git a/zlib_amd/gpu.py b/zlib_amd/gpu.py
--- a/zlib_amd/gpu.py
+++ b/zlib_amd/gpu.py
@@ -189,6 +189,9 @@
     L.zgpu_stage_name.restype = C.c_char_p
     L.zgpu_deflate_fast_count.argtypes = [vp, C.c_int]
     L.zgpu_deflate_fast_count.restype = u64
+    if hasattr(L, "zgpu_deflate_tail_count"):
+        L.zgpu_deflate_tail_count.argtypes = [vp, C.c_int]
+        L.zgpu_deflate_tail_count.restype = u64
     L.zgpu_corpus_fill_device.argtypes = [vp, u32, u64, u64, u64, vp, vp]
     _lib = L
     return L
@@ -286,6 +289,11 @@
 
     def fast_round_counts(self):
         return {k: int(self.L.zgpu_deflate_fast_count(self.h, i)) for i, k in enumerate(self.FAST_COUNTS)}
+
+    TAIL_COUNTS = ("from_counts", "from_tokens")
+
+    def tail_block_counts(self):
+        return {k: int(self.L.zgpu_deflate_tail_count(self.h, i)) for i, k in enumerate(self.TAIL_COUNTS)}
 
     def set_tuning(self, tune=None):
         g, l, n, c = tune if tune else (0, 0, 0, 0)
```
